# flybirdxx/ComfyUI-SDMatte

Measured on AMD Instinct MI355X. Metric: alpha mattes/sec at 1024x1024, higher is better.
Workload: dtype f16x3

## Files before the change

comfyui-sdmatte_amd/csrc/k_attn.h:

```cpp
#pragma once
#include "sdm_common.h"
#include "k_gemm.h"

struct AttnParams {
  const half_t* q; long q_bs; int ldq;
  const half_t* k; long k_bs; int ldk;
  int k_hs;
  const half_t* vt; long vt_bs; long vt_hs; int ldvt;
  const float* bias; long bias_bs;
  half_t* o; long o_bs; int ldo;
  int o_f32;
  int o_p3; long o_xl_off;
  long q_lo, k_lo, vt_lo;
  int Lq, Lk;
  float scale_log2e;
  const int* tiles; int tiles_bs;
  int nsplit; long part_stride; float* part_ml;
  int batch, heads, nq_blocks, q_chunks;
  int pp_flags;
  int ablate;
};

#define SDM_NEG_BIG (-1.0e30f)
#define SDM_ATTN_SKIP_MARGIN 2000.0f
// ... 385 lines not shown
      for (int dt = 0; dt < 2; ++dt)
#pragma unroll
        for (int g = 0; g < 4; ++g) {
          f32x4 h;
#pragma unroll
          for (int e = 0; e < 4; ++e) h[e] = o[qt][dt][4 * g + e] * inv;
          *(f32x4*)(stf + l31 * PS + (dt * 32 + 8 * g + 4 * hi) * 4) = h;
        }
      SDM_WAVE_SYNC();
      if (p.o_p3 && p.nsplit <= 1) {
        attn_store_p3(p, stf, PS, b, q0 + qt * 32, head, lane);
      } else {
#pragma unroll
      for (int pass = 0; pass < 8; ++pass) {
        const int row = pass * 4 + (lane >> 4), part = lane & 15;
        const int qg = q0 + qt * 32 + row;
        if (qg < p.Lq)
          *(f32x4*)(obase + (size_t)qg * p.ldo + head * 64 + part * 4) = *(const f32x4*)(stf + row * PS + part * 16);
      }
      }
      SDM_WAVE_SYNC();
    }
    return;
  }
#pragma unroll
  for (int qt = 0; qt < QT; ++qt) {
    const float l = PVS ? (lsum + __shfl_xor(lsum, 32)) : ls[qt][0];
    const float inv = 1.0f / l;
#pragma unroll
    for (int dt = 0; dt < 2; ++dt)
#pragma unroll
      for (int g = 0; g < 4; ++g) {
        f16x4 h;
#pragma unroll
        for (int e = 0; e < 4; ++e) h[e] = (half_t)(o[qt][dt][4 * g + e] * inv);
        *(f16x4*)(stg + l31 * PK + (dt * 32 + 8 * g + 4 * hi) * 2) = h;
      }
    SDM_WAVE_SYNC();
#pragma unroll
    for (int pass = 0; pass < 4; ++pass) {
      const int row = pass * 8 + (lane >> 3), part = lane & 7;
      const int qg = q0 + qt * 32 + row;
      if (qg < p.Lq)
        *(f16x8*)(p.o + (size_t)b * p.o_bs + (size_t)qg * p.ldo + head * 64 + part * 8) = *(const f16x8*)(stg + row * PK + part * 16);
    }
    SDM_WAVE_SYNC();
  }
}

#define ATTN64PIPE_SMEM (3 * ATTN64P_BUF)
#define ATTN64PIPE4_KB (2 * 64 * ATTN64_PK + 256)
#define ATTN64PIPE4_VB (64 * ATTN64_PV)
#define ATTN64PIPE4_SMEM (2 * ATTN64PIPE4_KB + 3 * ATTN64PIPE4_VB)
template <int NW>
__global__ void __launch_bounds__(64 * NW, 2) attn_d64_pipe_kernel(AttnParams p) {
  constexpr int NTH = 64 * NW, VPT = 512 / NTH;
  constexpr bool SPLITBUF = NW == 4;
  SDM_DYN_SMEM(smem);
  constexpr int PK = ATTN64_PK, PV = ATTN64_PV, BUF = ATTN64P_BUF;
  constexpr int KLO = 64 * PK, VOFF = 2 * 64 * PK, BOFF = VOFF + 64 * PV;
  auto k_of = [&](int b3, int b2) { return SPLITBUF ? smem + b2 * ATTN64PIPE4_KB : smem + b3 * BUF; };
  auto v_of = [&](int b3) { return SPLITBUF ? smem + 2 * ATTN64PIPE4_KB + b3 * ATTN64PIPE4_VB : smem + b3 * BUF + VOFF; };
  auto bias_of = [&](int b3, int b2) { return (float*)(SPLITBUF ? smem + b2 * ATTN64PIPE4_KB + 2 * 64 * PK : smem + b3 * BUF + BOFF); };
  const int tid = threadIdx.x, lane = tid & 63, wave = tid >> 6;
  const int hi = lane >> 5, l31 = lane & 31;
  int b, head, qblk;
  if (!attn_block_coords(p, blockIdx.x, b, head, qblk)) return;
  const int q0 = qblk * (32 * NW) + wave * 32;

  f16x8 qf[4];
  i32x8 q8p[2];
  {
    int qrow = q0 + l31;
    if (qrow > p.Lq - 1) qrow = p.Lq - 1;
    const half_t* qp = p.q + (size_t)b * p.q_bs + (size_t)qrow * p.ldq + head * 64 + hi * 8;
#pragma unroll
    for (int ks = 0; ks < 4; ++ks) qf[ks] = *(const f16x8*)(qp + ks * 16);
    const half_t* qb = p.q + (size_t)b * p.q_bs + p.q_lo + (size_t)qrow * p.ldq + head * 64 + hi * 16;
#pragma unroll
    for (int m = 0; m < 2; ++m) {
      const i32x4 r0 = *(const i32x4*)(qb + m * 32), r1 = *(const i32x4*)(qb + m * 32 + 8);
      q8p[m] = i32x8{r0[1], r0[0], r0[3], r0[2], r1[1], r1[0], r1[3], r1[2]};
    }
  }
  f32x16 o[2], ls;
  float m_i = SDM_NEG_BIG;
#pragma unroll
  for (int r = 0; r < 16; ++r) { ls[r] = 0.0f; o[0][r] = 0.0f; o[1][r] = 0.0f; }
  f16x8 ones;
#pragma unroll
  for (int j = 0; j < 8; ++j) ones[j] = (half_t)1.0f;

  const half_t* kbase = p.k + (size_t)b * p.k_bs + head * p.k_hs;
  const half_t* vbase = p.vt + (size_t)b * p.vt_bs + (size_t)head * p.vt_hs;
  const float* bbase = p.bias ? p.bias + (size_t)b * p.bias_bs : nullptr;
  const float* bsrc = bbase ? bbase : (const float*)(p.k + (size_t)b * p.k_bs);
  const int ntiles = (p.Lk + 63) / 64;
  const int* tl = p.tiles ? p.tiles + (size_t)b * p.tiles_bs : nullptr;
  const int sp = p.nsplit > 1 ? (int)blockIdx.y : 0;
  int i0, nwalk;
  attn_split_range(p, tl, ntiles, tl ? tl[0] : ntiles, sp, i0, nwalk);
  if (nwalk <= 0) { attn_write_empty_part(p, sp, b, head, q0, lane); return; }
  auto tile_at = [&](int i) { return tl ? tl[1 + i0 + i] : i0 + i; };

  f16x8 rk[VPT], rkl[VPT], rv[VPT];
  float rb = 0.0f;
  bool rin = true;
  auto prefetch = [&](int t) {
    const int k0 = t * 64;
#pragma unroll
    for (int i = 0; i < VPT; ++i) {
      const int v = tid + i * NTH, srow = v >> 3, spart = v & 7;
      int kr = k0 + srow;
      if (kr > p.Lk - 1) kr = p.Lk - 1;
      rk[i] = *(const f16x8*)(kbase + (size_t)kr * p.ldk + spart * 8);
      rv[i] = *(const f16x8*)(vbase + (size_t)srow * p.ldvt + k0 + spart * 8);
      rkl[i] = *(const f16x8*)(kbase + p.k_lo + (size_t)kr * p.ldk + spart * 8);
    }
    int kb = k0 + (tid & 63);
    rin = kb < p.Lk;
    if (!rin) kb = p.Lk - 1;
    rb = bsrc[kb];
  };
  auto stage = [&](int b3, int b2) {
    unsigned char* kb_ = k_of(b3, b2);
    unsigned char* vb_ = v_of(b3);
#pragma unroll
    for (int i = 0; i < VPT; ++i) {
      const int v = tid + i * NTH, srow = v >> 3, spart = v & 7;
      *(f16x8*)(kb_ + srow * PK + spart * 16) = rk[i];
      f16x4 lo, hi4;
#pragma unroll
      for (int e = 0; e < 4; ++e) { lo[e] = rv[i][e]; hi4[e] = rv[i][4 + e]; }
      *(f16x4*)(vb_ + srow * PV + spart * 16) = lo;
      *(f16x4*)(vb_ + srow * PV + spart * 16 + 8) = hi4;
      *(f16x8*)(kb_ + KLO + srow * PK + spart * 16) = rkl[i];
    }
    if (tid < 64) bias_of(b3, b2)[tid] = rin ? (bbase ? rb : 0.0f) : SDM_NEG_BIG;
  };
  auto qk = [&](int b3, int b2, f32x16 (&s)[2]) {
    const unsigned char* Ks = k_of(b3, b2);
    const float* Bs = bias_of(b3, b2);
#pragma unroll
    for (int kt = 0; kt < 2; ++kt)
#pragma unroll
      for (int g = 0; g < 4; ++g) {
        const f32x4 b4 = *(const f32x4*)(Bs + kt * 32 + 8 * g + 4 * hi);
#pragma unroll
        for (int e = 0; e < 4; ++e) s[kt][4 * g + e] = b4[e];
      }
#pragma unroll
    for (int kt = 0; kt < 2; ++kt) {
#pragma unroll
      for (int ks = 0; ks < 4; ++ks) {
        const f16x8 a = *(const f16x8*)(Ks + (kt * 32 + l31) * PK + ks * 32 + hi * 16);
        s[kt] = SDM_MFMA_32x32x16_F16(a, qf[ks], s[kt]);
      }
#pragma unroll
      for (int m = 0; m < 2; ++m) {
        const unsigned char* kp = Ks + KLO + (kt * 32 + l31) * PK + m * 64 + hi * 32;
        const i32x4 a0 = *(const i32x4*)kp, a1 = *(const i32x4*)(kp + 16);
        const i32x8 a8 = i32x8{a0[0], a0[1], a0[2], a0[3], a1[0], a1[1], a1[2], a1[3]};
        s[kt] = SDM_MFMA_32x32x64_BF8_BF8(a8, q8p[m], s[kt], 127 - 11, 127);
      }
    }
  };
  auto lds_barrier = [&]() { SDM_WAIT_LGKMCNT0(); SDM_RAW_BARRIER(); };

  prefetch(tile_at(0));
  stage(0, 0);
  if (1 < nwalk) prefetch(tile_at(1));
  lds_barrier();
  if (1 < nwalk) stage(1, 1);
  if (2 < nwalk) prefetch(tile_at(2));
  f32x16 sa[2], sb[2];
  qk(0, 0, sa);
  lds_barrier();

  int bt = 0;
  auto iter = [&](const int t, f32x16 (&sc)[2], f32x16 (&sn)[2]) {
    const int b1 = bt == 2 ? 0 : bt + 1, b2 = b1 == 2 ? 0 : b1 + 1;
    qk(b1, (t + 1) & 1, sn);
    float mx = SDM_NEG_BIG;
#pragma unroll
    for (int kt = 0; kt < 2; ++kt)
#pragma unroll
      for (int r = 0; r < 16; r += 2) mx = fmaxf(fmaxf(mx, sc[kt][r]), sc[kt][r + 1]);
    mx = fmaxf(mx, __shfl_xor(mx, 32));
    const float mnew = fmaxf(m_i, mx);
    const float alpha = sdm_exp2(m_i - mnew);
    m_i = mnew;
#pragma unroll
    for (int kt = 0; kt < 2; ++kt)
#pragma unroll
      for (int r = 0; r < 16; ++r) sc[kt][r] = sdm_exp2(sc[kt][r] - mnew);
    if (__any(alpha != 1.0f)) {
#pragma unroll
      for (int r = 0; r < 16; ++r) ls[r] *= alpha;
#pragma unroll
      for (int dt = 0; dt < 2; ++dt)
#pragma unroll
        for (int r = 0; r < 16; ++r) o[dt][r] *= alpha;
    }
    if (t + 2 < nwalk) stage(b2, t & 1);
    if (t + 3 < nwalk) prefetch(tile_at(t + 3));
    const unsigned char* Vs = v_of(bt);
#pragma unroll
    for (int kt = 0; kt < 2; ++kt)
#pragma unroll
      for (int u = 0; u < 2; ++u) {
        f16x8 pf;
#pragma unroll
        for (int j = 0; j < 8; ++j) pf[j] = (half_t)sc[kt][8 * u + j];
        ls = SDM_MFMA_32x32x16_F16(ones, pf, ls);
#pragma unroll
        for (int dt = 0; dt < 2; ++dt) {
          const unsigned char* vp = Vs + (dt * 32 + l31) * PV + (kt * 32 + 16 * u + 4 * hi) * 2;
          const f16x4 v0 = *(const f16x4*)vp, v1 = *(const f16x4*)(vp + 16);
          f16x8 vf;
#pragma unroll
          for (int e = 0; e < 4; ++e) { vf[e] = v0[e]; vf[4 + e] = v1[e]; }
          o[dt] = SDM_MFMA_32x32x16_F16(vf, pf, o[dt]);
        }
      }
    lds_barrier();
    bt = b1;
  };
  for (int t = 0; t < nwalk; t += 2) {
    iter(t, sa, sb);
    if (t + 1 < nwalk) iter(t + 1, sb, sa);
  }

  constexpr int PS = 272;
  unsigned char* stf = smem + wave * (32 * PS);
  const float inv = p.nsplit > 1 ? 1.0f : 1.0f / ls[0];
  float* obase = (float*)p.o + (p.nsplit > 1 ? (size_t)sp * p.part_stride : (size_t)0) + (size_t)b * p.o_bs;
  if (p.nsplit > 1 && hi == 0 && q0 + l31 < p.Lq) {
    float* ml = p.part_ml + ((((size_t)sp * p.batch + b) * p.heads + head) * p.Lq + q0 + l31) * 2;
    ml[0] = m_i; ml[1] = ls[0];
  }
#pragma unroll
  for (int dt = 0; dt < 2; ++dt)
#pragma unroll
    for (int g = 0; g < 4; ++g) {
      f32x4 h;
#pragma unroll
      for (int e = 0; e < 4; ++e) h[e] = o[dt][4 * g + e] * inv;
      *(f32x4*)(stf + l31 * PS + (dt * 32 + 8 * g + 4 * hi) * 4) = h;
    }
  SDM_WAVE_SYNC();
  if (p.o_p3 && p.nsplit <= 1) { attn_store_p3(p, stf, PS, b, q0, head, lane); return; }
#pragma unroll
  for (int pass = 0; pass < 8; ++pass) {
    const int row = pass * 4 + (lane >> 4), part = lane & 15;
    const int qg = q0 + row;
    if (qg < p.Lq)
      *(f32x4*)(obase + (size_t)qg * p.ldo + head * 64 + part * 4) = *(const f32x4*)(stf + row * PS + part * 16);
  }
}

#define ATTN64PP_SLOT (3 * 8192 + 256)
#define ATTN64PP_SMEM (6 * ATTN64PP_SLOT)
template <int ABL = 0, int BIAS = 1, int LIST = 1, int KE = 0, int DS = 1, int OB = 1>
__global__ void __launch_bounds__(512, 2) attn_d64_pp_kernel(AttnParams p) {
  SDM_DYN_SMEM(smem);
  constexpr int SLOT = ATTN64PP_SLOT, KLO = 8192, VOFF = 16384, BOFF = 24576;
  constexpr int R = KE < 0 ? 4 : 6, D = KE < 0 ? 3 : 4;
  constexpr int NDMA = BIAS ? 4 : 3;
  const int tid = threadIdx.x, lane = tid & 63, wave = SDM_UNIFORM_I(tid >> 6);
  const int grp = wave >> 2;
  const int hi = lane >> 5, l31 = lane & 31;
  int b, head, qblk;
  if (!attn_block_coords(p, blockIdx.x, b, head, qblk)) return;
  const int q0 = qblk * 256 + wave * 32;

  f16x8 qf[4];
  i32x8 q8p[2];
  {
    int qrow = q0 + l31;
    if (qrow > p.Lq - 1) qrow = p.Lq - 1;
    const half_t* qp = p.q + (size_t)b * p.q_bs + (size_t)qrow * p.ldq + head * 64 + hi * 8;
#pragma unroll
    for (int ks = 0; ks < 4; ++ks) qf[ks] = *(const f16x8*)(qp + ks * 16);
    const half_t* qb = p.q + (size_t)b * p.q_bs + p.q_lo + (size_t)qrow * p.ldq + head * 64 + hi * 16;
#pragma unroll
    for (int m = 0; m < 2; ++m) {
      const i32x4 r0 = *(const i32x4*)(qb + m * 32), r1 = *(const i32x4*)(qb + m * 32 + 8);
      q8p[m] = i32x8{r0[1], r0[0], r0[3], r0[2], r1[1], r1[0], r1[3], r1[2]};
    }
  }
  f32x16 o[2], ls;
  float m_i = SDM_NEG_BIG;
#pragma unroll
  for (int r = 0; r < 16; ++r) { ls[r] = 0.0f; o[0][r] = 0.0f; o[1][r] = 0.0f; }
  f16x8 ones;
#pragma unroll
  for (int j = 0; j < 8; ++j) ones[j] = (half_t)1.0f;

  const half_t* kbase = p.k + (size_t)b * p.k_bs + head * p.k_hs;
  const half_t* vbase = p.vt + (size_t)b * p.vt_bs + (size_t)head * p.vt_hs;
  const int ntiles = p.Lk / 64;
  const int* tl = (LIST && p.tiles) ? p.tiles + (size_t)b * p.tiles_bs : nullptr;
  const int sp = p.nsplit > 1 ? (int)blockIdx.y : 0;
  int i0, nwalk;
  attn_split_range(p, tl, ntiles, tl ? tl[0] : ntiles, sp, i0, nwalk);
  if (nwalk <= 0) { attn_write_empty_part(p, sp, b, head, q0, lane); return; }
  const int* tlp = tl ? tl + 1 + i0 : nullptr;
  auto tile_at = [&](int i) { if (i > nwalk - 1) i = nwalk - 1; return LIST ? tlp[i] : i0 + i; };

  const sdm_rsrc rsK = sdm_make_rsrc(kbase, (unsigned int)(((size_t)(p.Lk - 1) * p.ldk + 64) * 2));
  const sdm_rsrc rsK8 = sdm_make_rsrc(kbase + p.k_lo, (unsigned int)(((size_t)(p.Lk - 1) * p.ldk + 64) * 2));
  const sdm_rsrc rsV = sdm_make_rsrc(vbase, (unsigned int)(((size_t)63 * p.ldvt + p.Lk) * 2));
  const sdm_rsrc rsB = sdm_make_rsrc(BIAS ? p.bias + (size_t)b * p.bias_bs : (const float*)kbase, (unsigned int)p.Lk * 4u);
  const int rho = 8 * wave + (lane >> 3), cpos = lane & 7;
  const int csrc = cpos ^ ((rho >> 1) & 7);
  const int rr = rho & 31;
  const int pir = (rr & 0x13) | (((rr >> 2) & 1) << 3) | (((rr >> 3) & 1) << 2);
  const unsigned int voffK = (unsigned int)(((rho & 32) + pir) * p.ldk * 2 + csrc * 16);
  const unsigned int voffV = (unsigned int)(rho * p.ldvt * 2 + csrc * 16);
  const int lr = lane & 31;
  const unsigned int voffB = (unsigned int)(((lane & 32) + ((lr & 0x13) | (((lr >> 2) & 1) << 3) | (((lr >> 3) & 1) << 2))) * 4);
  auto dma = [&](int tile, int slot, int from = 0, int to = 4) {
    if (ABL & 8) return;
    unsigned char* sb = smem + slot * SLOT + wave * 1024;
    const unsigned int k0 = (unsigned int)tile * 64u;
    int i = 0;
    if (i >= from && i < to) sdm_glds16_buf(rsV, voffV, k0 * 2u, sb + VOFF);
    ++i;
    if (BIAS) { if (i >= from && i < to) sdm_glds4_buf(rsB, voffB, k0 * 4u, smem + slot * SLOT + BOFF); ++i; }
    if (i >= from && i < to) sdm_glds16_buf(rsK8, voffK, k0 * (unsigned int)(p.ldk * 2), sb + KLO);
    ++i;
    if (i >= from && i < to) sdm_glds16_buf(rsK, voffK, k0 * (unsigned int)(p.ldk * 2), sb);
  };
  const int kxor = (l31 >> 1) & 7;
  const int kx = l31 * 128 + ((hi ^ kxor) << 4);
  const int k8x = l31 * 128 + (((2 * hi) ^ kxor) << 4);
  const int vx = l31 * 128 + ((hi ^ kxor) << 4);
  struct KFrag { f16x8 h[4]; i32x8 f8[2]; };
  auto load_bias = [&](int slot, f32x16 (&s)[2]) {
    if (!BIAS) {
#pragma unroll
      for (int kt = 0; kt < 2; ++kt)
#pragma unroll
        for (int r = 0; r < 16; ++r) s[kt][r] = 0.0f;
      return;
    }
    if (ABL & 32) return;
    const float* Bs = (const float*)(smem + slot * SLOT + BOFF);
#pragma unroll
    for (int kt = 0; kt < 2; ++kt)
#pragma unroll
      for (int g = 0; g < 4; ++g) {
        const f32x4 b4 = *(const f32x4*)(Bs + kt * 32 + 8 * g + 4 * hi);
#pragma unroll
        for (int e = 0; e < 4; ++e) s[kt][4 * g + e] = b4[e];
      }
  };
  auto load_k = [&](int slot, int kt, KFrag& f) {
    if (ABL & 32) { SDM_PIN_HERE_V4(f.h[0], f.h[1], f.h[2], f.h[3]); SDM_PIN_HERE_V4(f.f8[0], f.f8[1], f.h[0], f.h[1]); return; }
    const unsigned char* Ks = smem + slot * SLOT + kt * 4096;
#pragma unroll
    for (int ks = 0; ks < 4; ++ks) f.h[ks] = *(const f16x8*)(Ks + (kx ^ (ks * 32)));
#pragma unroll
    for (int m = 0; m < 2; ++m) {
      const i32x4 a0 = *(const i32x4*)(Ks + KLO + (k8x ^ (m * 64))), a1 = *(const i32x4*)(Ks + KLO + ((k8x ^ (m * 64)) ^ 16));
      f.f8[m] = i32x8{a0[0], a0[1], a0[2], a0[3], a1[0], a1[1], a1[2], a1[3]};
    }
  };
  auto mma_k = [&](const KFrag& f, f32x16& sk) {
    if (ABL & 4) return;
#pragma unroll
    for (int ks = 0; ks < 4; ++ks) sk = SDM_MFMA_32x32x16_F16(f.h[ks], qf[ks], sk);
#pragma unroll
    for (int m = 0; m < 2; ++m) sk = SDM_MFMA_32x32x64_BF8_BF8(f.f8[m], q8p[m], sk, 127 - 11, 127);
  };
  struct VFrag { f16x8 v[2][2]; };
  auto load_v = [&](int slot, int kt, VFrag& f) {
    if (ABL & 32) { SDM_PIN_HERE_V4(f.v[0][0], f.v[0][1], f.v[1][0], f.v[1][1]); return; }
    const unsigned char* Vs = smem + slot * SLOT + VOFF;
#pragma unroll
    for (int u = 0; u < 2; ++u)
#pragma unroll
      for (int dt = 0; dt < 2; ++dt) f.v[u][dt] = *(const f16x8*)(Vs + dt * 4096 + (vx ^ ((4 * kt + 2 * u) * 16)));
  };
  auto mma_v = [&](const VFrag& f, const f16x8 (&pk)[2]) {
    if (ABL & 2) return;
#pragma unroll
    for (int u = 0; u < 2; ++u) {
      ls = SDM_MFMA_32x32x16_F16(ones, pk[u], ls);
#pragma unroll
      for (int dt = 0; dt < 2; ++dt) o[dt] = SDM_MFMA_32x32x16_F16(f.v[u][dt], pk[u], o[dt]);
    }
  };
  auto qk = [&](int slot, f32x16 (&s)[2]) {
    KFrag k0, k1;
    load_bias(slot, s);
    load_k(slot, 0, k0);
    load_k(slot, 1, k1);
    mma_k(k0, s[0]);
    mma_k(k1, s[1]);
  };
  auto softmax = [&](f32x16 (&s)[2], f16x8 (&pf)[2][2], auto&& mid0, auto&& mid1, auto&& after_max) {
    if (ABL & 1) {
      mid0(); mid1();
      after_max();
#pragma unroll
      for (int kt = 0; kt < 2; ++kt)
#pragma unroll
        for (int u = 0; u < 2; ++u)
#pragma unroll
          for (int j = 0; j < 8; j += 2) { pf[kt][u][j] = (half_t)s[kt][8 * u + j]; pf[kt][u][j + 1] = pf[kt][u][j]; }
      SDM_PIN_HERE_V4(pf[0][0], pf[0][1], pf[1][0], pf[1][1]);
      return;
    }
    float mx = SDM_NEG_BIG;
#pragma unroll
    for (int r = 0; r < 16; r += 2) mx = fmaxf(fmaxf(mx, s[0][r]), s[0][r + 1]);
#pragma unroll
    for (int r = 0; r < 16; r += 2) mx = fmaxf(fmaxf(mx, s[1][r]), s[1][r + 1]);
    {
      unsigned int xa = __builtin_bit_cast(unsigned int, mx), xb = xa;
      sdm_permlane32_swap(xa, xb);
      mx = fmaxf(__builtin_bit_cast(float, xa), __builtin_bit_cast(float, xb));
    }
    const float mnew = fmaxf(m_i, mx);
    const float alpha = sdm_exp2(m_i - mnew);
    m_i = mnew;
    SDM_SCHED_FENCE();
    mid0();
    SDM_SCHED_FENCE();
    if (__any(alpha != 1.0f)) {
#pragma unroll
      for (int r = 0; r < 16; ++r) ls[r] *= alpha;
#pragma unroll
      for (int dt = 0; dt < 2; ++dt)
#pragma unroll
        for (int r = 0; r < 16; ++r) o[dt][r] *= alpha;
    }
    after_max();
#pragma unroll
    for (int r = 0; r < 16; ++r) s[0][r] = sdm_exp2(s[0][r] - mnew);
    SDM_SCHED_FENCE();
    mid1();
    SDM_SCHED_FENCE();
#pragma unroll
    for (int r = 0; r < 16; ++r) s[1][r] = sdm_exp2(s[1][r] - mnew);
#pragma unroll
    for (int kt = 0; kt < 2; ++kt)
#pragma unroll
      for (int u = 0; u < 2; ++u)
#pragma unroll
        for (int j = 0; j < 8; ++j) pf[kt][u][j] = (half_t)s[kt][8 * u + j];
    SDM_PIN_HERE_V4(pf[0][0], pf[0][1], pf[1][0], pf[1][1]);
  };
  auto lds_barrier = [&]() { SDM_SCHED_FENCE(); SDM_WAIT_LGKMCNT0(); SDM_RAW_BARRIER(); SDM_SCHED_FENCE(); };

#pragma unroll
  for (int i = 0; i < D; ++i) dma(tile_at(i), i);
  int tq = tile_at(D);
  SDM_WAIT_VMCNT0();
  lds_barrier();
  if (!OB) {
    if (grp) {
      if (p.pp_flags & 1) SDM_SETPRIO(1);
      lds_barrier();
    }
  } else if (grp && (p.pp_flags & 1)) SDM_SETPRIO(1);
  f32x16 s[2];
  f16x8 pf[2][2];
  qk(0, s);
  if (!OB || grp) lds_barrier();
  unsigned long long* trc = (unsigned long long*)(smem + R * SLOT) + (wave >> 2) * (8 * 28);
  const bool tracing = (ABL & 64) && blockIdx.x == 0 && (wave & 3) == 0;
  auto stamp = [&](int t, int k) { if ((ABL & 64) && tracing && t < 28 && lane == 0) trc[t * 8 + k] = __builtin_readcyclecounter(); };
  int bt = 0, b1 = 1, bD = D;
  for (int t = 0; t < nwalk; ++t) {
    if (p.pp_flags & 2) SDM_SETPRIO(0);
    constexpr int NE = OB ? NDMA : DS;
    if (KE >= 0) dma(tq, bD, 0, NE >= 2 ? NE - 2 : NE);
    int tqn;
    {
      int in_ = t + D + (KE >= 0 ? 1 : 0); if (in_ > nwalk - 1) in_ = nwalk - 1;
      if (LIST) SDM_SLOAD_I32(tqn, tlp + in_);
      else tqn = i0 + in_;
    }
    if (ABL & 64) stamp(t, 4);
    VFrag v0, v1;
    KFrag k0, k1;
    softmax(s, pf, [&]() { if (KE >= 0 && NE >= 2) dma(tq, bD, NE - 2, NE - 1); }, [&]() { if (KE >= 0 && NE >= 2) dma(tq, bD, NE - 1, NE); },
            [&]() { load_v(bt, 0, v0); load_v(bt, 1, v1); });
    if (ABL & 64) stamp(t, 5);
    if (KE >= 1) { load_bias(b1, s); load_k(b1, 0, k0); }
    if (KE >= 2) load_k(b1, 1, k1);
    if (LIST) SDM_SLOAD_WAIT(tqn);
    if (ABL & 64) { SDM_WAIT_LGKMCNT0(); stamp(t, 0); }
    if (!OB) lds_barrier();
    else if (!grp) { if (!(ABL & 8)) { if (BIAS) SDM_WAIT_VMCNT(8); else SDM_WAIT_VMCNT(6); } lds_barrier(); }
    if (ABL & 64) stamp(t, 1);
    if (p.pp_flags & 2) SDM_SETPRIO(2);
    if (KE < 0) dma(tqn, bD);
    mma_v(v0, pf[0]);
    mma_v(v1, pf[1]);
    if (KE < 1) { load_bias(b1, s); load_k(b1, 0, k0); }
    if (KE < 2) load_k(b1, 1, k1);
    if (KE < 1) {
#pragma unroll
      for (int i = 0; i < 12; ++i) { SDM_SCHED_GROUP(0x008, 1, 0); SDM_SCHED_GROUP(0x100, 2, 0); SDM_SCHED_GROUP(0x002, 1, 0); }
    } else if (KE < 2) {
#pragma unroll
      for (int i = 0; i < 8; ++i) { SDM_SCHED_GROUP(0x008, 1, 0); SDM_SCHED_GROUP(0x100, 1, 0); }
    }
    SDM_SCHED_FENCE();
    mma_k(k0, s[0]);
    mma_k(k1, s[1]);
    SDM_SCHED_FENCE();
    if (!(ABL & 8) && !OB) {
      if (KE < 0) { if (BIAS) SDM_WAIT_VMCNT(4); else SDM_WAIT_VMCNT(3); }
      else if (NDMA + DS == 3) SDM_WAIT_VMCNT(3); else if (NDMA + DS == 4) SDM_WAIT_VMCNT(4); else if (NDMA + DS == 5) SDM_WAIT_VMCNT(5);
      else if (NDMA + DS == 6) SDM_WAIT_VMCNT(6); else if (NDMA + DS == 7) SDM_WAIT_VMCNT(7); else SDM_WAIT_VMCNT(8);
    }
    if (KE >= 0 && !OB) dma(tq, bD, DS, NDMA);
    if (ABL & 64) { asm volatile("s_nop 0" :: "v"(s[0][0]), "v"(s[1][15])); SDM_WAIT_LGKMCNT0(); stamp(t, 2); }
    if (!OB) lds_barrier();
    else if (grp) { if (!(ABL & 8)) { if (BIAS) SDM_WAIT_VMCNT(8); else SDM_WAIT_VMCNT(6); } lds_barrier(); }
    if (ABL & 64) stamp(t, 3);
    tq = tqn;
    bt = b1; b1 = b1 == R - 1 ? 0 : b1 + 1; bD = bD == R - 1 ? 0 : bD + 1;
  }
  if (!grp) lds_barrier();
  SDM_WAIT_VMCNT0();
  lds_barrier();
  if ((ABL & 64) && blockIdx.x == 0) {
    const unsigned long long* tr0 = (const unsigned long long*)(smem + R * SLOT);
    for (int i = tid; i < 2 * 8 * 28; i += 512) ((unsigned long long*)p.part_ml)[i] = tr0[i];
    __syncthreads();
  }

  constexpr int PS = 272;
  unsigned char* stf = smem + wave * (32 * PS);
  const float inv = p.nsplit > 1 ? 1.0f : 1.0f / ls[0];
  float* obase = (float*)p.o + (p.nsplit > 1 ? (size_t)sp * p.part_stride : (size_t)0) + (size_t)b * p.o_bs;
  if (p.nsplit > 1 && hi == 0 && q0 + l31 < p.Lq) {
    float* ml = p.part_ml + ((((size_t)sp * p.batch + b) * p.heads + head) * p.Lq + q0 + l31) * 2;
    ml[0] = m_i; ml[1] = ls[0];
  }
#pragma unroll
  for (int dt = 0; dt < 2; ++dt)
#pragma unroll
    for (int g = 0; g < 4; ++g) {
      f32x4 h;
#pragma unroll
      for (int e = 0; e < 4; ++e) h[e] = o[dt][4 * g + e] * inv;
      *(f32x4*)(stf + l31 * PS + (dt * 32 + 8 * g + 4 * hi) * 4) = h;
    }
  SDM_WAVE_SYNC();
  if (p.o_p3 && p.nsplit <= 1) { attn_store_p3(p, stf, PS, b, q0, head, lane); return; }
#pragma unroll
  for (int pass = 0; pass < 8; ++pass) {
    const int row = pass * 4 + (lane >> 4), part = lane & 15;
    const int qg = q0 + row;
    if (qg < p.Lq)
      *(f32x4*)(obase + (size_t)qg * p.ldo + head * 64 + part * 4) = *(const f32x4*)(stf + row * PS + part * 16);
  }
}

#define ATTN512_X_BYTES (8 * 16 * 64 * 4)

#define ATTN512P_K_BYTES (32 * 1024)
#define ATTN512P_V_BYTES (512 * 64)
#define ATTN512P_X_OFF (2 * ATTN512P_K_BYTES + 2 * ATTN512P_V_BYTES)
#define ATTN512P_SMEM (ATTN512P_X_OFF + ATTN512_X_BYTES)

template <int ABL = 0>
__global__ void __launch_bounds__(512) attn_d512_kernel(AttnParams p) {
  SDM_DYN_SMEM(smem);
  float* Xs = (float*)(smem + ATTN512P_X_OFF);
  const int tid = threadIdx.x, lane = tid & 63, wave = SDM_UNIFORM_I(tid >> 6);
  const int hi = lane >> 5, l31 = lane & 31;
  const int qgp = wave >> 1, dh = wave & 1;
  int b, head_unused, qblk;
  if (!attn_block_coords(p, blockIdx.x, b, head_unused, qblk)) return;
  const int q0 = qblk * 128 + qgp * 32;

  f16x8 qf[16];
  {
    int qrow = q0 + l31;
    if (qrow > p.Lq - 1) qrow = p.Lq - 1;
    const half_t* qp = p.q + (size_t)b * p.q_bs + (size_t)qrow * p.ldq + dh * 256 + hi * 8;
#pragma unroll
    for (int ks = 0; ks < 16; ++ks) qf[ks] = *(const f16x8*)(qp + ks * 16);
  }
  f32x16 o[8];
#pragma unroll
  for (int dt = 0; dt < 8; ++dt)
#pragma unroll
    for (int r = 0; r < 16; ++r) o[dt][r] = 0.0f;
  float m_i = SDM_NEG_BIG, l_i = 0.0f;

  const half_t* kbase = p.k + (size_t)b * p.k_bs;
  const half_t* vbase = p.vt + (size_t)b * p.vt_bs;
  const int ntiles = (p.Lk + 31) / 32;

  const sdm_rsrc rsK = sdm_make_rsrc(kbase, (unsigned int)((size_t)p.Lk * p.ldk * 2));
  const sdm_rsrc rsV = sdm_make_rsrc(vbase, (unsigned int)((size_t)512 * p.ldvt * 2));
  const unsigned int v_voff = (unsigned int)((lane >> 2) * p.ldvt * 2 + (((lane & 3) ^ ((lane >> 4) & 3)) * 16));
  auto issue_tile = [&](int t, int buf) {
    if (ABL & 8) return;
    const int k0 = t * 32;
    unsigned char* Kd = smem + buf * ATTN512P_K_BYTES;
    unsigned char* Vd = smem + 2 * ATTN512P_K_BYTES + buf * ATTN512P_V_BYTES;
#pragma unroll
    for (int i = 0; i < 4; ++i) {
      const int rho = 4 * wave + i;
      const int pi = (rho & 16) | (((rho >> 2) & 1) << 3) | (((rho >> 3) & 1) << 2) | (rho & 3);
      int kr = k0 + pi;
// ... 58 lines not shown
        float x = (s[r] + xpt[r * 64 + lane]) * p.scale_log2e;
        if (key >= p.Lk) x = SDM_NEG_BIG;
        s[r] = x;
        mx = fmaxf(mx, x);
      }
    } else {
#pragma unroll
      for (int r = 0; r < 16; ++r) {
        const float x = (s[r] + xpt[r * 64 + lane]) * p.scale_log2e;
        s[r] = x;
        mx = fmaxf(mx, x);
      }
    }
    mx = fmaxf(mx, __shfl_xor(mx, 32));
    const float mnew = fmaxf(m_i, mx);
    const float alpha = sdm_exp2(m_i - mnew);
    m_i = mnew;
    float rs = 0.0f;
#pragma unroll
    for (int r = 0; r < 16; ++r) {
      const float pv = sdm_exp2(s[r] - mnew);
      s[r] = pv;
      rs += pv;
    }
    l_i = l_i * alpha + rs;
    if (__any(alpha != 1.0f)) {
#pragma unroll
      for (int dt = 0; dt < 8; ++dt)
#pragma unroll
        for (int r = 0; r < 16; ++r) o[dt][r] *= alpha;
    }
    } else l_i = 1.0f;
    f16x8 pf[2];
#pragma unroll
    for (int u = 0; u < 2; ++u)
#pragma unroll
      for (int j = 0; j < 8; ++j) pf[u][j] = (half_t)s[8 * u + j];
    SDM_SCHED_FENCE();
#pragma unroll
    for (int i = 0; i < 16; ++i) {
      if (i + 3 < 16) a[(i + 3) & 3] = rd_v(i + 3);
      if (!(ABL & 2)) o[i & 7] = SDM_MFMA_32x32x16_F16(a[i & 3], pf[i >> 3], o[i & 7]);
    }
    if (!(ABL & 34)) {
#pragma unroll
      for (int i = 0; i < 13; ++i) { SDM_SCHED_GROUP(0x100, 1, 1); SDM_SCHED_GROUP(0x008, 1, 1); }
      SDM_SCHED_GROUP(0x008, 3, 1);
    }
    SDM_SCHED_FENCE();
    SDM_WAIT_VMCNT0();
    SDM_RAW_BARRIER();
  }

  l_i += __shfl_xor(l_i, 32);
  const float inv = 1.0f / l_i;
  if (p.o_f32) {
    constexpr int PF = 528;
    unsigned char* stf = smem + wave * (32 * PF);
#pragma unroll
    for (int half = 0; half < 2; ++half) {
      __syncthreads();
#pragma unroll
      for (int d4 = 0; d4 < 4; ++d4) {
        const int dt = half * 4 + d4;
#pragma unroll
        for (int g = 0; g < 4; ++g) {
          f32x4 h;
#pragma unroll
          for (int e = 0; e < 4; ++e) h[e] = o[dt][4 * g + e] * inv;
          *(f32x4*)(stf + l31 * PF + (d4 * 32 + 8 * g + 4 * hi) * 4) = h;
        }
      }
      __syncthreads();
#pragma unroll
      for (int pass = 0; pass < 16; ++pass) {
        const int row = pass * 2 + (lane >> 5), part = lane & 31;
        const int qg = q0 + row;
        if (qg < p.Lq)
          *(f32x4*)((float*)p.o + (size_t)b * p.o_bs + (size_t)qg * p.ldo + dh * 256 + half * 128 + part * 4) =
              *(const f32x4*)(stf + row * PF + part * 16);
      }
    }
    return;
  }
  constexpr int PS = 272;
  unsigned char* stg = smem + wave * (32 * PS);
#pragma unroll
  for (int half = 0; half < 2; ++half) {
    __syncthreads();
#pragma unroll
    for (int d4 = 0; d4 < 4; ++d4) {
      const int dt = half * 4 + d4;
#pragma unroll
      for (int g = 0; g < 4; ++g) {
        f16x4 h;
#pragma unroll
        for (int e = 0; e < 4; ++e) h[e] = (half_t)(o[dt][4 * g + e] * inv);
        *(f16x4*)(stg + l31 * PS + (d4 * 32 + 8 * g + 4 * hi) * 2) = h;
      }
    }
    __syncthreads();
#pragma unroll
    for (int pass = 0; pass < 8; ++pass) {
      const int row = pass * 4 + (lane >> 4), part = lane & 15;
      const int qg = q0 + row;
      if (qg < p.Lq)
        *(f16x8*)(p.o + (size_t)b * p.o_bs + (size_t)qg * p.ldo + dh * 256 + half * 128 + part * 8) =
            *(const f16x8*)(stg + row * PS + part * 16);
    }
  }
}

__global__ void __launch_bounds__(256) attn_combine_kernel(const float* __restrict__ part_o, const float* __restrict__ part_ml, float* __restrict__ out,
                                                           int nsplit, long part_stride, int batch, int heads, int Lq, long o_bs, int ldo) {
  const long t = (long)blockIdx.x * blockDim.x + threadIdx.x;
  const int part = (int)(t & 15);
  const long rh = t >> 4;
  if (rh >= (long)batch * Lq * heads) return;
  const int head = (int)(rh % heads);
  const long br = rh / heads;
  const int row = (int)(br % Lq), b = (int)(br / Lq);
  float M = SDM_NEG_BIG;
  for (int s = 0; s < nsplit; ++s) M = fmaxf(M, part_ml[((((size_t)s * batch + b) * heads + head) * Lq + row) * 2]);
  f32x4 acc = {0.f, 0.f, 0.f, 0.f};
  float L = 0.0f;
  for (int s = 0; s < nsplit; ++s) {
    const float* ml = part_ml + ((((size_t)s * batch + b) * heads + head) * Lq + row) * 2;
    const float w = sdm_exp2(ml[0] - M);
    L += ml[1] * w;
    const f32x4 v = *(const f32x4*)(part_o + (size_t)s * part_stride + (size_t)b * o_bs + (size_t)row * ldo + head * 64 + part * 4);
#pragma unroll
    for (int e = 0; e < 4; ++e) acc[e] += v[e] * w;
  }
  const float inv = 1.0f / L;
#pragma unroll
  for (int e = 0; e < 4; ++e) acc[e] *= inv;
  *(f32x4*)(out + (size_t)b * o_bs + (size_t)row * ldo + head * 64 + part * 4) = acc;
}

__global__ void __launch_bounds__(256) attn_combine_p3_kernel(const float* __restrict__ part_o, const float* __restrict__ part_ml, unsigned char* __restrict__ out,
                                                              long xl_off, int nsplit, long part_stride, int batch, int heads, int Lq, long o_bs, int ldo) {
  const long t = (long)blockIdx.x * blockDim.x + threadIdx.x;
  const int part = (int)(t & 7);
  const long rh = t >> 3;
  if (rh >= (long)batch * Lq * heads) return;
  const int head = (int)(rh % heads);
  const long br = rh / heads;
  const int row = (int)(br % Lq), b = (int)(br / Lq);
  float M = SDM_NEG_BIG;
  for (int s = 0; s < nsplit; ++s) M = fmaxf(M, part_ml[((((size_t)s * batch + b) * heads + head) * Lq + row) * 2]);
  float acc[8] = {0.f, 0.f, 0.f, 0.f, 0.f, 0.f, 0.f, 0.f};
  float L = 0.0f;
  for (int s = 0; s < nsplit; ++s) {
    const float* ml = part_ml + ((((size_t)s * batch + b) * heads + head) * Lq + row) * 2;
    const float w = sdm_exp2(ml[0] - M);
    L += ml[1] * w;
    const float* src = part_o + (size_t)s * part_stride + (size_t)b * o_bs + (size_t)row * ldo + head * 64 + part * 8;
    const f32x4 v0 = *(const f32x4*)src, v1 = *(const f32x4*)(src + 4);
#pragma unroll
    for (int e = 0; e < 4; ++e) { acc[e] += v0[e] * w; acc[4 + e] += v1[e] * w; }
  }
  const float inv = 1.0f / L;
#pragma unroll
// ... 70 lines not shown
```

comfyui-sdmatte_amd/csrc/k_misc.h:

```cpp
#pragma once
#include "sdm_common.h"

template <typename F>
SDM_DEV_INLINE float resize_aa_sample(F fetch, int in_h, int in_w, int out_h, int out_w, int oy, int ox) {
  const float sy = (float)in_h / (float)out_h, sx = (float)in_w / (float)out_w;
  const float supy = sy >= 1.0f ? sy : 1.0f, supx = sx >= 1.0f ? sx : 1.0f;
  const float invy = sy >= 1.0f ? 1.0f / sy : 1.0f, invx = sx >= 1.0f ? 1.0f / sx : 1.0f;
  const float cy = sy * ((float)oy + 0.5f), cx = sx * ((float)ox + 0.5f);
  int ymin = (int)(cy - supy + 0.5f); if (ymin < 0) ymin = 0;
  int ymax = (int)(cy + supy + 0.5f); if (ymax > in_h) ymax = in_h;
  int xmin = (int)(cx - supx + 0.5f); if (xmin < 0) xmin = 0;
  int xmax = (int)(cx + supx + 0.5f); if (xmax > in_w) xmax = in_w;
  float wys = 0.0f, wxs = 0.0f;
  for (int y = ymin; y < ymax; ++y) { float w = 1.0f - fabsf(((float)y - cy + 0.5f) * invy); wys += w > 0.0f ? w : 0.0f; }
  for (int x = xmin; x < xmax; ++x) { float w = 1.0f - fabsf(((float)x - cx + 0.5f) * invx); wxs += w > 0.0f ? w : 0.0f; }
  float acc = 0.0f;
  for (int y = ymin; y < ymax; ++y) {
    float wy = 1.0f - fabsf(((float)y - cy + 0.5f) * invy); wy = wy > 0.0f ? wy / wys : 0.0f;
    float row = 0.0f;
    for (int x = xmin; x < xmax; ++x) {
      float wx = 1.0f - fabsf(((float)x - cx + 0.5f) * invx); wx = wx > 0.0f ? wx / wxs : 0.0f;
      row += wx * fetch(y, x);
    }
    acc += wy * row;
// ... 106 lines not shown
  const float r = img[i * 3 + 0], g = img[i * 3 + 1], b = img[i * 3 + 2];
  if (mode == 1) {
    f32x4 o = {r, g, b, a};
    *(f32x4*)(matted + i * 4) = o;
  } else if (mode == 2) {
    const float gate = (t > 0.2f && a > 0.1f) ? 1.0f : 0.0f;
    matted[i * 3 + 0] = r * gate; matted[i * 3 + 1] = g * gate; matted[i * 3 + 2] = b * gate;
  } else {
    matted[i * 3 + 0] = 0.0f; matted[i * 3 + 1] = 0.0f; matted[i * 3 + 2] = 0.0f;
  }
}

SDM_DEV_INLINE u32x2 sdm_pair_plane4(const float (&x)[4], f16x4& oh) {
  float xx[4], xl[4];
#pragma unroll
  for (int e = 0; e < 4; ++e) {
    const float y = fminf(fmaxf(x[e], -57344.0f), 57344.0f);
    oh[e] = (half_t)y; xx[e] = y; xl[e] = (y - (float)oh[e]) * 2048.0f;
  }
  int a = SDM_CVT_PK_BF8(xx[0], xx[1], 0, false), b = SDM_CVT_PK_BF8(xl[0], xl[1], 0, false);
  a = SDM_CVT_PK_BF8(xx[2], xx[3], a, true); b = SDM_CVT_PK_BF8(xl[2], xl[3], b, true);
  u32x2 pr;
  pr[0] = (unsigned int)a; pr[1] = (unsigned int)b;
  return pr;
}

__global__ void split_planes_kernel(const float* __restrict__ x, half_t* __restrict__ hi, half_t* __restrict__ lo, long n, float mult, int mode) {
  const long i4 = ((long)blockIdx.x * blockDim.x + threadIdx.x) * 4;
  if (i4 >= n) return;
  float y[4];
#pragma unroll
  for (int e = 0; e < 4; ++e) y[e] = (i4 + e < n) ? x[i4 + e] * mult : 0.0f;
  f16x4 oh, ol;
  if (mode == 3) {
    const u32x2 pr = sdm_pair_plane4(y, oh);
    *(f16x4*)(hi + i4) = oh;
    *(u32x2*)(lo + i4) = pr;
  } else {
#pragma unroll
    for (int e = 0; e < 4; ++e) { oh[e] = (half_t)y[e]; ol[e] = (half_t)(y[e] - (float)oh[e]); }
    *(f16x4*)(hi + i4) = oh;
    *(f16x4*)(lo + i4) = ol;
  }
}

SDM_DEV_INLINE float cross_patch_value(const float* __restrict__ uin, int H, int W, long b, int key, int j) {
  if (j >= 36 || key >= H * W) return 0.0f;
  const int ci = j / 9, tap = j - ci * 9, ky = tap / 3, kx = tap - ky * 3;
  const int y = key / W + ky - 1, x = key - (key / W) * W + kx - 1;
  if ((unsigned)y >= (unsigned)H || (unsigned)x >= (unsigned)W) return 0.0f;
  return uin[((size_t)b * H * W + (size_t)y * W + x) * 16 + 4 + ci];
}
__global__ void __launch_bounds__(256) cross_patch_planes_kernel(const float* __restrict__ uin, int B, int H, int W, half_t* __restrict__ k_hi,
                                                                 half_t* __restrict__ k_pair, half_t* __restrict__ vt, int ldvt) {
  const long t = (long)blockIdx.x * blockDim.x + threadIdx.x;
  const int Lk = H * W;
  if (blockIdx.y == 0) {
    if (t >= (long)B * Lk * 8) return;
    const int oct = (int)(t & 7), key = (int)((t >> 3) % Lk);
    const long b = (t >> 3) / Lk;
    u32x4 hv, pv;
#pragma unroll
    for (int g = 0; g < 2; ++g) {
      float x[4];
#pragma unroll
      for (int e = 0; e < 4; ++e) x[e] = cross_patch_value(uin, H, W, b, key, oct * 8 + g * 4 + e);
      f16x4 oh;
      const u32x2 pr = sdm_pair_plane4(x, oh);
      const u32x2 hw = __builtin_bit_cast(u32x2, oh);
      hv[2 * g] = hw[0]; hv[2 * g + 1] = hw[1]; pv[2 * g] = pr[0]; pv[2 * g + 1] = pr[1];
    }
    const size_t o = ((size_t)b * Lk + key) * 64 + oct * 8;
    *(u32x4*)(k_hi + o) = hv;
    *(u32x4*)(k_pair + o) = pv;
  } else {
    const int cpr = ldvt / 8;
    if (t >= (long)B * 64 * cpr) return;
    const int chunk = (int)(t % cpr), j = (int)((t / cpr) & 63);
    const long b = t / cpr / 64;
    u32x4 hv;
#pragma unroll
    for (int g = 0; g < 2; ++g) {
      f16x4 oh;
#pragma unroll
      for (int e = 0; e < 4; ++e) oh[e] = (half_t)fminf(fmaxf(cross_patch_value(uin, H, W, b, chunk * 8 + g * 4 + e, j), -57344.0f), 57344.0f);
      const u32x2 hw = __builtin_bit_cast(u32x2, oh);
      hv[2 * g] = hw[0]; hv[2 * g + 1] = hw[1];
    }
    *(u32x4*)(vt + ((size_t)b * 64 + j) * ldvt + chunk * 8) = hv;
  }
}

__global__ void scale_copy_kernel(const float* __restrict__ in, float* __restrict__ out, long n, float mult) {
  const long i = (long)blockIdx.x * blockDim.x + threadIdx.x;
  if (i < n) out[i] = in[i] * mult;
}

__global__ void fill_random_f16_kernel(half_t* __restrict__ p, long n, unsigned int seed, float amp) {
  for (long i = (long)blockIdx.x * blockDim.x + threadIdx.x; i < n; i += (long)gridDim.x * blockDim.x) {
    unsigned int h = (unsigned int)i * 2654435761u + seed;
    h ^= h >> 15; h *= 2246822519u; h ^= h >> 13; h *= 3266489917u; h ^= h >> 16;
    p[i] = (half_t)(((float)(h & 0xFFFF) * (1.0f / 32768.0f) - 1.0f) * amp);
  }
}
__global__ void fill_random_f32_kernel(float* __restrict__ p, long n, unsigned int seed, float amp) {
  for (long i = (long)blockIdx.x * blockDim.x + threadIdx.x; i < n; i += (long)gridDim.x * blockDim.x) {
    unsigned int h = (unsigned int)i * 2654435761u + seed;
    h ^= h >> 15; h *= 2246822519u; h ^= h >> 13; h *= 3266489917u; h ^= h >> 16;
    p[i] = ((float)(h & 0xFFFF) * (1.0f / 32768.0f) - 1.0f) * amp;
  }
}

#define SDM_CMASK_EMPTY 0xFFFFFFFFu

__global__ __launch_bounds__(256) void cmask_table_kernel(const float* __restrict__ plane, unsigned int* __restrict__ table, int n0, int H, int W) {
  SDM_SHARED unsigned int tb[4];
  const int b = blockIdx.x, tid = threadIdx.x;
  if (tid < 4) tb[tid] = SDM_CMASK_EMPTY;
  __syncthreads();
  const float* pl = plane + (size_t)b * H * W;
  for (int i = tid; i < 64 * 64; i += 256) {
    const int y = (int)(((long)(i >> 6) * H) >> 6), x = (int)(((long)(i & 63) * W) >> 6);
    const unsigned int bits = __builtin_bit_cast(unsigned int, pl[(size_t)y * W + x]);
    for (int k = 0; k < 4; ++k) {
      unsigned int cur = tb[k];
      if (cur == SDM_CMASK_EMPTY) cur = atomicCAS(&tb[k], SDM_CMASK_EMPTY, bits);
      if (cur == SDM_CMASK_EMPTY || cur == bits) break;
    }
  }
  __syncthreads();
  if (tid < 4) table[(size_t)(n0 + b) * 4 + tid] = tb[tid];
}

__global__ void cmask_init_kernel(const float* __restrict__ plane, unsigned char* __restrict__ mask, const unsigned int* __restrict__ table, int n0, int B, long HW) {
  const long i = (long)blockIdx.x * blockDim.x + threadIdx.x;
  if (i >= (long)B * HW) return;
  const int b = (int)(i / HW);
  const unsigned int bits = __builtin_bit_cast(unsigned int, plane[i]);
// ... 65 lines not shown
```

comfyui-sdmatte_amd/csrc/sdm_common.h:

```cpp
#pragma once
#include <stdint.h>
#include <stddef.h>
#ifdef SDM_EMU
#include "hip_emu.h"
#else
#include <hip/hip_runtime.h>
#endif

typedef _Float16 half_t;
typedef half_t f16x8 __attribute__((ext_vector_type(8)));
typedef half_t f16x4 __attribute__((ext_vector_type(4)));
typedef half_t f16x2 __attribute__((ext_vector_type(2)));
typedef float f32x2 __attribute__((ext_vector_type(2)));
typedef float f32x4 __attribute__((ext_vector_type(4)));
typedef float f32x16 __attribute__((ext_vector_type(16)));
typedef int i32x8 __attribute__((ext_vector_type(8)));
typedef int i32x4 __attribute__((ext_vector_type(4)));

#ifdef SDM_EMU
#define SDM_DYN_SMEM(name) unsigned char* name = emu::g_dyn_smem
#define SDM_SHARED static thread_local
#define SDM_MFMA_32x32x16_F16(a, b, c) emu_mfma_f32_32x32x16_f16((a), (b), (c))
#define SDM_MFMA_32x32x64_F8(a, b, c, sa, sb) emu_mfma_scale_f32_32x32x64_fp8((a), (b), (c), (sa), (sb))
#define SDM_CVT_PK_FP8(a, b, old, hi_word) emu_cvt_pk_fp8_f32((a), (b), (old), (hi_word))
// ... 64 lines not shown
#else
typedef __amdgpu_buffer_rsrc_t sdm_rsrc;
__device__ __forceinline__ sdm_rsrc sdm_make_rsrc(const void* p, unsigned int bytes) {
  return __builtin_amdgcn_make_buffer_rsrc((void*)p, 0, (int)bytes, 0x00020000);
}
__device__ __forceinline__ u32x4 sdm_buffer_load16(sdm_rsrc r, unsigned int voff, unsigned int soff) {
  return __builtin_amdgcn_raw_buffer_load_b128(r, (int)voff, (int)soff, 0);
}
__device__ __forceinline__ u32x2 sdm_buffer_load8(sdm_rsrc r, unsigned int voff, unsigned int soff) {
  return __builtin_amdgcn_raw_buffer_load_b64(r, (int)voff, (int)soff, 0);
}
__device__ __forceinline__ void sdm_buffer_store16(u32x4 v, sdm_rsrc r, unsigned int voff, unsigned int soff) {
  __builtin_amdgcn_raw_buffer_store_b128(v, r, (int)voff, (int)soff, 0);
}
#endif

#ifdef SDM_EMU
typedef sdm_rsrc sdm_rsrc_raw;
static inline sdm_rsrc_raw sdm_make_rsrc_raw(const void* p, unsigned int bytes) { return sdm_make_rsrc(p, bytes); }
#define SDM_ASM_BUFFER_LOAD16(dst, voff, rsrc, imm) (dst) = sdm_buffer_load16((rsrc), (voff), (imm))
#define SDM_ASM_BUFFER_LOAD16_FIRST(dst, voff, rsrc, imm) (dst) = sdm_buffer_load16((rsrc), (voff), (imm))
#else
typedef u32x4 sdm_rsrc_raw;
__device__ __forceinline__ sdm_rsrc_raw sdm_make_rsrc_raw(const void* p, unsigned int bytes) {
  const unsigned long long a = (unsigned long long)p;
  sdm_rsrc_raw d;
  d[0] = (unsigned int)__builtin_amdgcn_readfirstlane((int)(unsigned int)a);
  d[1] = (unsigned int)__builtin_amdgcn_readfirstlane((int)((unsigned int)(a >> 32) & 0xFFFFu));
  d[2] = (unsigned int)__builtin_amdgcn_readfirstlane((int)bytes);
  d[3] = 0x00020000u;
  return d;
}
#define SDM_ASM_BUFFER_LOAD16(dst, voff, rsrc, imm) \
  asm volatile("buffer_load_dwordx4 %0, %1, %2, 0 offen offset:" #imm : "=v"(dst) : "v"(voff), "s"(rsrc) : "memory")
#define SDM_ASM_BUFFER_LOAD16_FIRST(dst, voff, rsrc, imm) \
  asm volatile("s_nop 4\n\tbuffer_load_dwordx4 %0, %1, %2, 0 offen offset:" #imm : "=v"(dst) : "v"(voff), "s"(rsrc) : "memory")
#endif

#ifdef SDM_EMU
static inline void sdm_glds16(const void* gsrc, unsigned char* lds_base) { memcpy(lds_base + (threadIdx.x & 63) * 16, gsrc, 16); }
static inline void sdm_glds16_buf(sdm_rsrc r, unsigned int voff, unsigned int soff, unsigned char* lds_base) {
  const u32x4 v = sdm_buffer_load16(r, voff, soff);
  memcpy(lds_base + (threadIdx.x & 63) * 16, &v, 16);
}
static inline void sdm_glds4_buf(sdm_rsrc r, unsigned int voff, unsigned int soff, unsigned char* lds_base) {
  unsigned int v = 0u;
  const unsigned long long o = (unsigned long long)voff + soff;
  if (o + 4 <= r.bytes) memcpy(&v, r.base + o, 4);
  memcpy(lds_base + (threadIdx.x & 63) * 4, &v, 4);
}
#define SDM_UNIFORM_I(x) (x)
#define SDM_OPAQUE_I(x) ((void)0)
#define SDM_PIN_HERE_V4(a, b, c, d) ((void)0)
#define SDM_WAIT_VMCNT0() ((void)0)
#define SDM_WAIT_VMCNT(n) ((void)0)
#define SDM_WAIT_LGKMCNT0() ((void)0)
#define SDM_SLOAD_I32(dst, ptr) (dst) = *(ptr)
#define SDM_SLOAD_WAIT(dst) ((void)0)
#define SDM_RAW_BARRIER() __syncthreads()
#else
__device__ __forceinline__ void sdm_glds16(const void* gsrc, unsigned char* lds_base) {
  __builtin_amdgcn_global_load_lds((const __attribute__((address_space(1))) void*)gsrc,
                                   (__attribute__((address_space(3))) void*)lds_base, 16, 0, 0);
}
__device__ __forceinline__ void sdm_glds16_buf(sdm_rsrc r, unsigned int voff, unsigned int soff, unsigned char* lds_base) {
  __builtin_amdgcn_raw_ptr_buffer_load_lds(r, (__attribute__((address_space(3))) void*)lds_base, 16, (int)voff, (int)soff, 0, 0);
}
__device__ __forceinline__ void sdm_glds4_buf(sdm_rsrc r, unsigned int voff, unsigned int soff, unsigned char* lds_base) {
  __builtin_amdgcn_raw_ptr_buffer_load_lds(r, (__attribute__((address_space(3))) void*)lds_base, 4, (int)voff, (int)soff, 0, 0);
}
#define SDM_UNIFORM_I(x) __builtin_amdgcn_readfirstlane(x)
#define SDM_OPAQUE_I(x) asm volatile("" : "+v"(x))
#define SDM_PIN_HERE_V4(a, b, c, d) asm volatile("" : "+v"(a), "+v"(b), "+v"(c), "+v"(d))
#define SDM_WAIT_VMCNT0() asm volatile("s_waitcnt vmcnt(0)" ::: "memory")
#define SDM_WAIT_VMCNT(n) asm volatile("s_waitcnt vmcnt(" #n ")" ::: "memory")
#define SDM_WAIT_LGKMCNT0() asm volatile("s_waitcnt lgkmcnt(0)" ::: "memory")
#define SDM_SLOAD_I32(dst, ptr) asm volatile("s_load_dword %0, %1, 0x0" : "=s"(dst) : "s"(ptr) : "memory")
#define SDM_SLOAD_WAIT(dst) asm volatile("s_waitcnt lgkmcnt(0)" : "+s"(dst) :: "memory")
#define SDM_RAW_BARRIER() do { asm volatile("" ::: "memory"); __builtin_amdgcn_s_barrier(); asm volatile("" ::: "memory"); } while (0)
#endif

#ifdef SDM_EMU
static inline float sdm_sum_row16(float v) {
  v += __shfl_xor(v, 1); v += __shfl_xor(v, 2); v += __shfl_xor(v, 4); v += __shfl_xor(v, 8);
  return v;
}
#else
#define SDM_DPP_ADD(v, ctrl) ((v) + __builtin_bit_cast(float, __builtin_amdgcn_update_dpp(0, __builtin_bit_cast(int, (v)), (ctrl), 0xF, 0xF, false)))
__device__ __forceinline__ float sdm_sum_row16(float v) {
  v = SDM_DPP_ADD(v, 0xB1);
  v = SDM_DPP_ADD(v, 0x4E);
  v = SDM_DPP_ADD(v, 0x124);
  v = SDM_DPP_ADD(v, 0x128);
  return v;
}
#endif

#ifdef SDM_EMU
static inline unsigned int sdm_perm_b32(unsigned int s0, unsigned int s1, unsigned int sel) {
  const unsigned long long v = ((unsigned long long)s0 << 32) | s1;
  unsigned int r = 0;
  for (int i = 0; i < 4; ++i) r |= (unsigned int)((v >> (8 * ((sel >> (8 * i)) & 7))) & 0xffull) << (8 * i);
  return r;
}
static inline void sdm_permlane32_swap(unsigned int& a, unsigned int& b) {
  auto& w = emu::wave(); const int l = emu::lane_id();
  w.slot[l][0] = a; w.slot[l][1] = b; emu::wave_barrier();
  if (l < 32) b = w.slot[l + 32][0]; else a = w.slot[l - 32][1];
  emu::wave_barrier();
}
#else
__device__ __forceinline__ unsigned int sdm_perm_b32(unsigned int s0, unsigned int s1, unsigned int sel) { return __builtin_amdgcn_perm(s0, s1, sel); }
__device__ __forceinline__ void sdm_permlane32_swap(unsigned int& a, unsigned int& b) {
  const auto r = __builtin_amdgcn_permlane32_swap(a, b, false, false);
  a = r[0]; b = r[1];
}
#endif

#define SDM_LOG2E 1.4426950408889634f

SDM_DEV_INLINE float sdm_silu(float x) {
  return x / (1.0f + sdm_exp2(-x * SDM_LOG2E));
}

SDM_DEV_INLINE float sdm_gelu_erf(float x) {
  return 0.5f * x * (1.0f + erff(x * 0.70710678118654752f));
// ... 28 lines not shown
```

comfyui-sdmatte_amd/csrc/sdm_engine.cpp:

```cpp
#include "sdm_common.h"
#include "k_conv.h"
#include "k_gemm.h"
#include "k_norm.h"
#include "k_attn.h"
#include "k_misc.h"
#include "k_trimap.h"
#include "k_cclabel.h"
#include "k_foreground.h"
#include "k_guided.h"
#include "k_roi.h"
#include "k_canvas.h"
#include "k_boxes.h"
#include "../../include/sdmatte.h"

#include <algorithm>
#include <cmath>
#include <cstdio>
#include <cstdlib>
#include <cstring>
#include <atomic>
#include <map>
#include <mutex>
#include <shared_mutex>
#include <string>
// ... 33 lines not shown
        if (r_ != hipSuccess) fprintf(stderr, "[sdmatte] hipFuncSetAttribute(%d bytes of LDS) failed: %s\n", (int)(bytes), hipGetErrorString(r_)); \
        else done_.fetch_or(bit_, std::memory_order_relaxed);                                                    \
      }                                                                                                          \
    }                                                                                                            \
  } while (0)
#endif

static inline int rup(int a, int b) { return ((a + b - 1) / b) * b; }
#ifdef SDM_EMU
static inline void dev_use(int) {}
#else
static inline void dev_use(int device) {
  const hipError_t r = hipSetDevice(device);
  if (r != hipSuccess) fprintf(stderr, "[sdmatte] hipSetDevice(%d) failed: %s\n", device, hipGetErrorString(r));
}
#endif
static inline size_t rupz(size_t a, size_t b) { return ((a + b - 1) / b) * b; }

struct OptEntry { const char* name; int value; int def; const char* what; };
static OptEntry g_opts[] = {
  {"conv_f8", 1, 1, "residual terms of the wide split-precision 3x3 convs on fp8 MFMAs (read when a model is built)"},
  {"gemm_f8", 1, 1, "the same for Linear / 1x1 layers with K >= gemm_f8_min_k (read when a model is built)"},
  {"gemm_f8_min_k", 1024, 1024, "smallest K of a GEMM that takes the 8-wave fp8-residual kernel"},
  {"gemm_p3", 1, 1, "transformer-block Linear layers on the plane-fed GEMM (k_gemm.h): pre-split operand planes from LayerNorm / GroupNorm / attention / GEGLU, LDS-DMA only (the W3 weight copies are built when a model is built)"},
  {"gemm_p3_tile", 0, 0, "row tile of the plane-fed GEMM: 0 by shape, 256 / 128 / 64 forced"},
  {"gemm_p3_attn", 1, 1, "d=64 attention cores write the operand planes of to_out themselves (0: fp32 result + one conversion pass)"},
  {"gemm_p3_persist", 1, 1, "plane-fed GEMM: persistent blocks that prefetch the next tile's first chunk underneath the epilogue (0: one block per tile, n > 1: a grid of n blocks - tests)"},
  {"gemm_p3_ablate", 0, 0, "bench only: 1 no MFMAs, 2 no DMAs behind the prologue, 4 no epilogue (sdm_bench_gemm_p3)"},
  {"conv_up_phase", 1, 1, "up-sampling 3x3 convs (Upsample2D) as four 2x2-tap phase convs on the plane-fed GEMM (k_gemm.h, UP): 0 off (the 3x3 kernels on the up-sampled image), 1 the launches with at least two 256-row tiles per CU (up_phase_wins: measured), 2 every eligible launch (tests).  0 / non-0 is read when a model is built: the phase matrices are a derived weight layout"},
  {"conv_epi", 4, 4, "F8 kernels' epilogue: 4 register-direct stores + residual as accumulator init, 3 residual init only, 0 LDS-staged"},
  {"conv_xtile", 1, 1, "F8 3x3: cross-tile prefetch by the producer waves"},
  {"conv_f8_tpb", 0, 0, "F8: tiles per block (0 = by queue depth)"},
  {"conv_dma", 1, 1, "3x3 stride-1 256x128 tile: weights by LDS-DMA"},
  {"conv_dma_all", 0, 0, "keep a stage-ordered weight copy for every wide 3x3 layer, not only the split-precision ones (read when a model is built)"},
  {"conv_pc", -1, -1, "producer / consumer form of the split-precision DMA kernel: -1 by channel count, 0 off, 1 on"},
  {"conv_pc_min_cin", 256, 256, "conv_pc = -1: smallest Cin that takes the producer / consumer form"},
  {"conv_db", 0, 0, "512x128 double-buffered tile where the queue is deep"},
  {"trimap_skip", 1, 1, "VAE encoder, trimap images: output tiles inside a constant region of the trimap are not multiplied (k_misc.h cmask_*; exact). 0 = every tile"},
  {"conv_band_rows", 0, 0, "tile rows per XCD band of the convs that leave constant tiles out (0 = by image height)"},
  {"trimap_skip_min_rows", 512, 512, "smallest output height at which constant tiles are left out (measured at 1024^2: the 1024- and 512-row levels gain 3.7 + 1.6 ms, the 256-row level loses 0.7: too few of its 32 x 128-pixel tiles lie inside one region)"},
  {"conv_splitk", -1, -1, "split-K of the register-staged conv / GEMM kernels: -1 by shape (few tiles, long K), 0 off, n >= 2 forced where the shape allows"},
  {"force_cfg0", 0, 0, "always the 256x128 tile for 3x3 stride 1 (tests: fused GroupNorm at tiny sizes)"},
  {"no_gn_fuse", 0, 0, "never fuse the GroupNorm apply into the consuming conv"},
  {"split_lds_pad", 0, 0, "extra dynamic LDS of the register-staged split kernels (forces one block per CU)"},
  {"attn_f8", 1, 1, "Q.K^T residual terms of the d=64 split-precision attention on fp8 MFMAs"},
  {"attn_dense", 0, 0, "walk every key tile of the trimap-biased self-attention"},
  {"attn_pv_split", 0, 0, "residual terms of P.V too (fully split attention; tests)"},
  {"attn_nw", 0, 0, "waves per d=64 attention block: 0 by launch size, 4, 8"},
  {"attn_pipe", 1, 1, "8-wave split-precision d=64 attention: two-tile software pipeline"},
  {"attn_pipe4", 1, 1, "the same pipeline for the 4-wave launches (two K / three V^T buffers)"},
  {"attn_pp", 1, 1, "split-precision d=64 attention with fp32 output as a ping-pong of the block's wave halves (attn_d64_pp_kernel, 256 query rows per block): 0 off, 1 on, 2 on without the static priority of the younger half, 3 on with per-segment priority flips"},
  {"attn_pp_min_blocks", 128, 128, "attn_pp: launches with fewer 256-row blocks than this keep the 4-wave pipelines (0 in tests: the ping-pong kernel at any size)"},
  {"attn_ksplit", 0, 0, "key split of the d=64 split-precision attention: 0 by launch size (blocks that do not fill the chip's block slots a whole number of times), 1 off, 2 / 4 forced, 3 forced on the ping-pong kernel (ignored elsewhere: those launches run unsplit)"},
  {"cross_shared", 1, 1, "cross-attention on ONE key / value operand per forward, the patch matrix of the trimap latent (cross_patch_planes_kernel), with the K|V fold moved into q_shared / out_shared: 0 = every block's own kv_folded conv + transpose.  Read per forward"},
  {"precise_mask", -1, -1, "stages in split precision (-1 = the config's own mask; per-stage attribution experiments; read at sdm_create)"},
#ifdef SDM_EMU
  {"emu_arena_extra", 0, 0, "emulator build only, self-test of the arena check: the launch pass of a stand-alone op allocates one block its sizing pass did not"},
#endif
};
static OptEntry* opt_find(const char* name) {
  for (auto& o : g_opts) if (name && strcmp(o.name, name) == 0) return &o;
  return nullptr;
}
static int opt(const char* name) { OptEntry* o = opt_find(name); return o ? o->value : 0; }
static std::shared_mutex g_opt_mu;
struct OptReadLock { std::shared_lock<std::shared_mutex> l; OptReadLock() : l(g_opt_mu) {} };
static std::mutex g_count_mu;
static std::map<std::string, long> g_kernel_counts;
static void count_kernel(const char* name) { std::lock_guard<std::mutex> g(g_count_mu); g_kernel_counts[name] += 1; }

template <int NTAPS, int STRIDE, int TH, int TW, int BN, int KC, int WM, int WN, int DB = 0, int GNOK = 0>
static void launch_conv_t(const ConvParams& p_in, void* stream) {
  using C = ConvCfg<NTAPS, STRIDE, TH, TW, BN, KC, WM, WN, DB>;
  ConvParams p = p_in;
  p.tiles_m = (NTAPS == 9) ? sdm_cdiv(p.Wout, TW) * sdm_cdiv(p.Hout, TH)
                           : (int)(((p.rows_per_img ? (long)p.rows_per_img : p.M) + C::BM - 1) / C::BM);
  p.tiles_n = sdm_cdiv(p.Cout_pad, BN);
  const long total_m = (long)p.tiles_m * ((NTAPS == 9 || p.rows_per_img) ? p.N : 1);
  p.xcd_chunk = (int)((total_m + 7) / 8);
  const dim3 grid((unsigned)(8L * p.xcd_chunk * p.tiles_n), (unsigned)(p.ksplit > 1 ? p.ksplit : 1), 1);
  const size_t gn_extra = (size_t)(p.C0 + p.C1) * 8;
  if constexpr (!DB) {
    if (p.w_lo) {
      using CS = ConvCfg<NTAPS, STRIDE, TH, TW, BN, KC, WM, WN, 0, 1>;
      const size_t lds_pad = (size_t)opt("split_lds_pad");
      if (GNOK && p.gn_scale) {
        auto k = conv_mfma_kernel<NTAPS, STRIDE, TH, TW, BN, KC, WM, WN, 1, 0, GNOK, 1>;
        SDM_SET_SMEM(k, 160 * 1024);
        SDM_LAUNCH(k, grid, dim3(CS::NTHREADS), (size_t)CS::SMEM + gn_extra + lds_pad, stream, p);
      } else {
        auto k = conv_mfma_kernel<NTAPS, STRIDE, TH, TW, BN, KC, WM, WN, 1, 0, 0, 1>;
        SDM_SET_SMEM(k, 160 * 1024);
        SDM_LAUNCH(k, grid, dim3(CS::NTHREADS), CS::SMEM + lds_pad, stream, p);
      }
      return;
    }
  }
  if (GNOK && p.gn_scale) {
    const size_t smem = (size_t)C::SMEM + gn_extra;
    if (p.in_f32) {
      auto k = conv_mfma_kernel<NTAPS, STRIDE, TH, TW, BN, KC, WM, WN, 1, DB, GNOK>;
      SDM_SET_SMEM(k, C::SMEM + 1024 * 8);
      SDM_LAUNCH(k, grid, dim3(C::NTHREADS), smem, stream, p);
    } else {
      auto k = conv_mfma_kernel<NTAPS, STRIDE, TH, TW, BN, KC, WM, WN, 0, DB, GNOK>;
      SDM_SET_SMEM(k, C::SMEM + 1024 * 8);
// ... 1110 lines not shown
  return 0;
}

static int op_groupnorm_raw(sdm_ctx* e, const void* in0, const void* in1, int C0, int C1, int in_f32, int N, int HW, int groups,
                            const float* gamma, const float* beta, float eps, int silu, void* out, int out_f32, const float* st0 = nullptr,
                            int rows0 = 0, const float* st1 = nullptr, int rows1 = 0, bool have_stats = false) {
  const int C = C0 + C1;
  T scratch; float* scale; float* shift;
  TRY(gn_scale_shift(e, in0, in1, C0, C1, in_f32, N, HW, groups, gamma, beta, eps, st0, rows0, st1, rows1, have_stats, &scratch, &scale, &shift));
  if (!e->dry) {
    GnSrc s; s.in0 = in0; s.in1 = in1; s.C0 = C0; s.C1 = C1; s.in_f32 = in_f32; s.HW = HW;
    const GnGeometry g = gn_geometry(C, N, HW);
    prof_begin(e, "gn_apply", 0, (double)N * HW * C * (in_f32 ? 4 : 2) + (double)N * HW * C * (double)fmt_bytes(out_f32));
    if (out_f32 == kFmtP3)
      SDM_LAUNCH(gn_apply_p3_kernel, dim3((unsigned)(((long)N * HW + 15) / 16)), dim3(256), 0, e->stream, s, (const float*)scale, (const float*)shift, (unsigned char*)out,
                 silu, (long)N * HW);
    else
    SDM_LAUNCH(gn_apply_kernel, dim3(g.nb, N), dim3(g.threads), 0, e->stream, s, (const float*)scale, (const float*)shift, out, out_f32, silu, g.ppb);
    prof_end(e);
  }
  tfree(e, scratch);
  return 0;
}

static int op_gn(sdm_ctx* e, const NormL& n, const T& x, const T* x2, int silu, float eps, T* out, int out_fmt = -1) {
  const int C = x.C + (x2 ? x2->C : 0);
  if (C != n.C) SDM_FAIL(e, SDM_ERR_INVALID, "groupnorm: C %d != %d", C, n.C);
  *out = talloc(e, x.N, x.H, x.W, C, out_fmt >= 0 ? out_fmt : e->act_f32);
  const bool hs = x.sbytes && (!x2 || x2->sbytes);
  return op_groupnorm_raw(e, x.p, x2 ? x2->p : nullptr, x.C, x2 ? x2->C : 0, x.f32, x.N, x.H * x.W, e->cfg.groups, n.g, n.b, eps, silu,
                          out->p, out->f32, x.stats, x.srows, x2 ? x2->stats : nullptr, x2 ? x2->srows : 0, hs);
}

static int op_ln(sdm_ctx* e, const NormL& n, const T& x, float eps, T* out, int out_fmt = -1) {
  if (x.C != n.C || x.C % 64 || x.C > 64 * SDM_LN_MAXV) SDM_FAIL(e, SDM_ERR_INVALID, "layernorm: unsupported C %d", x.C);
  *out = talloc(e, x.N, x.H, x.W, x.C, out_fmt >= 0 ? out_fmt : e->act_f32);
  if (e->dry) return 0;
  const long rows = x.rows();
  if (out->f32 == kFmtP3) {
    if (x.f32 != 1 || x.C > 128 * SDM_LNP_MAXI) SDM_FAIL(e, SDM_ERR_INVALID, "layernorm (P3): fp32 input, C <= %d expected", 128 * SDM_LNP_MAXI);
    prof_begin(e, "layernorm", 0, (double)rows * x.C * 7);
    SDM_LAUNCH(layernorm_p3_kernel, dim3((unsigned)((rows + 15) / 16)), dim3(256), 0, e->stream, (const float*)x.p, (const float*)n.g, (const float*)n.b,
               (unsigned char*)out->p, rows, x.C, eps);
    prof_end(e);
    return 0;
  }
  prof_begin(e, "layernorm", 0, (double)rows * x.C * ((x.f32 ? 4 : 2) + (out->f32 ? 4 : 2)));
  SDM_LAUNCH(layernorm_kernel, dim3((unsigned)((rows + 3) / 4)), dim3(256), 0, e->stream, (const void*)x.p, x.f32, (const float*)n.g,
             (const float*)n.b, out->p, out->f32, rows, x.C, eps);
  prof_end(e);
  return 0;
}

struct AttnPrec { int prec = 0; long q_lo = 0, k_lo = 0, v_lo = 0; int out_f32 = 0; int out_p3 = 0; bool has_bias = false, has_tiles = false; bool shared_kv = false; };

enum AttnKernel { kAttnPP, kAttnPPBias, kAttnPPTiles, kAttnPipe8, kAttnPipe4, kAttnP3W8, kAttnP3W4, kAttnP1W8, kAttnP1W4, kAttnP2W8, kAttnP2W4,
                  kAttnF16W8, kAttnF16W4, kAttnD512 };
struct AttnPlan {
  AttnKernel kernel;
  const char* spec_counter;
  const char* combine_counter;
  int qrows;
  unsigned nblk;
  int nsplit;
  bool walk_tiles, own_list;
  bool pv_split;
  int pp_flags;
};
struct AttnKernelInfo { const char* counter; int threads; size_t smem; void (*launch)(const AttnKernelInfo&, const AttnPlan&, const AttnParams&, void*); };
template <auto K, int LDS_LIMIT = 160 * 1024>
static void attn_launch_t(const AttnKernelInfo& ki, const AttnPlan& pl, const AttnParams& p, void* stream) {
  if constexpr (LDS_LIMIT > 0) SDM_SET_SMEM(K, LDS_LIMIT);
  SDM_LAUNCH(K, dim3(pl.nblk, (unsigned)pl.nsplit, 1), dim3(ki.threads), ki.smem, stream, p);
}
static const AttnKernelInfo kAttnKernels[] = {
  {"attn_d64_pp", 512, ATTN64PP_SMEM, attn_launch_t<attn_d64_pp_kernel<0, 0, 0>>},
  {"attn_d64_pp", 512, ATTN64PP_SMEM, attn_launch_t<attn_d64_pp_kernel<0, 1, 0>>},
  {"attn_d64_pp", 512, ATTN64PP_SMEM, attn_launch_t<attn_d64_pp_kernel<0, 1, 1>>},
  {"attn_d64_pipe<8>", 512, ATTN64PIPE_SMEM, attn_launch_t<attn_d64_pipe_kernel<8>>},
  {"attn_d64_pipe<4>", 256, ATTN64PIPE4_SMEM, attn_launch_t<attn_d64_pipe_kernel<4>>},
  {"attn_d64<prec3,8>", 512, ATTN64P_SMEM, attn_launch_t<attn_d64_kernel<1, 3, 8>>},
  {"attn_d64<prec3,4>", 256, ATTN64P_SMEM, attn_launch_t<attn_d64_kernel<1, 3, 4>>},
  {"attn_d64<prec1,8>", 512, ATTN64P_SMEM, attn_launch_t<attn_d64_kernel<1, 1, 8>>},
  {"attn_d64<prec1,4>", 256, ATTN64P_SMEM, attn_launch_t<attn_d64_kernel<1, 1, 4>>},
  {"attn_d64<prec2,8>", 512, ATTN64P_SMEM, attn_launch_t<attn_d64_kernel<1, 2, 8>>},
  {"attn_d64<prec2,4>", 256, ATTN64P_SMEM, attn_launch_t<attn_d64_kernel<1, 2, 4>>},
  {"attn_d64<fp16,8>", 512, ATTN64P_SMEM, attn_launch_t<attn_d64_kernel<1, 0, 8>>},
  {"attn_d64<fp16,4>", 256, ATTN64_SMEM, attn_launch_t<attn_d64_kernel<1, 0, 4>, 0>},
  {"attn_d512", 512, ATTN512P_SMEM, attn_launch_t<attn_d512_kernel<0>, ATTN512P_SMEM>},
};
static AttnPlan attn_plan(int B, int heads, int Lq, int Lk, int D, int prec, int out_f32, bool has_bias, bool has_tiles, int cus) {
  AttnPlan pl;
  memset(&pl, 0, sizeof(pl));
  pl.nsplit = 1;
  bool nw8 = true, pp = false;
  if (D != 64) {
    pl.kernel = kAttnD512; pl.qrows = 128;
  } else {
    pl.walk_tiles = has_bias && opt("attn_dense") == 0;
    pl.own_list = pl.walk_tiles && !has_tiles;
    pl.pv_split = prec == 1 && opt("attn_pv_split") != 0;
    const int force_nw = opt("attn_nw");
    const long blocks256 = (long)B * heads * sdm_cdiv(Lq, 256);
    pp = prec == 2 && out_f32 && opt("attn_pp") != 0 && !force_nw && Lk % 64 == 0 &&
         blocks256 >= opt("attn_pp_min_blocks");
    nw8 = pp || (force_nw ? (force_nw == 8) : (prec && blocks256 >= 1024));
    pl.qrows = nw8 ? 256 : 128;
    if (prec == 2) {
      const bool pipe = out_f32 && opt(nw8 ? "attn_pipe" : "attn_pipe4") != 0;
      if (pp) pl.kernel = pl.walk_tiles ? kAttnPPTiles : (has_bias ? kAttnPPBias : kAttnPP);
      else if (pipe) pl.kernel = nw8 ? kAttnPipe8 : kAttnPipe4;
      else pl.kernel = nw8 ? kAttnP3W8 : kAttnP3W4;
    } else if (prec) {
      pl.kernel = pl.pv_split ? (nw8 ? kAttnP1W8 : kAttnP1W4) : (nw8 ? kAttnP2W8 : kAttnP2W4);
    } else {
      pl.kernel = nw8 ? kAttnF16W8 : kAttnF16W4;
    }
    if (pp) {
      pl.spec_counter = pl.walk_tiles ? "attn_pp<0,1,1>" : (has_bias ? "attn_pp<0,1,0>" : "attn_pp<0,0,0>");
      pl.pp_flags = opt("attn_pp") == 1 ? 1 : (opt("attn_pp") == 3 ? 2 : 0);
    }
  }
  pl.nblk = (unsigned)(B * heads * 8 * sdm_cdiv(sdm_cdiv(Lq, pl.qrows), 8));
  if (D == 64 && prec && out_f32 && !pl.pv_split) {
    const long blocks = pl.nblk, slots = (long)cus * (nw8 ? 1 : 2);
    const int o = opt("attn_ksplit"), ntiles64 = sdm_cdiv(Lk, 64);
    if (o >= 2) pl.nsplit = (o == 2 || o == 4 || (o == 3 && pp)) ? o : 1;
    else if (o == 0) {
      auto rounds = [&](int s) { return (double)((blocks * s + slots - 1) / slots) / s; };
      for (int s = 2; s <= 4; ++s)
        if ((s != 3 || pp) && ntiles64 / s >= 32 && rounds(s) < 0.85 * rounds(pl.nsplit)) pl.nsplit = s;
    }
    if (pl.nsplit > 1) pl.combine_counter = pl.nsplit == 2 ? "attn_combine/n=2" : (pl.nsplit == 3 ? "attn_combine/n=3" : "attn_combine/n=4");
  }
  return pl;
}

static int op_attention_raw(sdm_ctx* e, const half_t* q, int ldq, const half_t* k, int ldk, const half_t* v, int ldv, const float* bias_l2,
                            int B, int heads, int Lq, int Lk, int D, void* out, int ldo, bool q_prescaled = false, const int* tiles = nullptr,
                            AttnPrec ap = AttnPrec()) {
  if (!(D == 64 || (D == 512 && heads == 1))) SDM_FAIL(e, SDM_ERR_INVALID, "attention: unsupported head dim %d x %d heads", D, heads);
  if ((ldq | ldk | ldv | ldo) % 8) SDM_FAIL(e, SDM_ERR_INVALID, "attention: row strides must be multiples of 8");
  if (ap.prec && D != 64) SDM_FAIL(e, SDM_ERR_INVALID, "attention: the split-precision variant exists for head dim 64 only");
  if (ap.prec == 2 && !q_prescaled) SDM_FAIL(e, SDM_ERR_INVALID, "attention: the fp8-residual form takes pre-scaled queries");
  if (!e->dry && (ap.has_bias != (bias_l2 != nullptr) || ap.has_tiles != (tiles != nullptr)))
    SDM_FAIL(e, SDM_ERR_STATE, "attention: bias / tile list do not match what the sizing pass was told");
  const AttnPlan pl = attn_plan(B, heads, Lq, Lk, D, ap.prec, ap.out_f32, ap.has_bias, ap.has_tiles, device_cus());
  const AttnKernelInfo& ki = kAttnKernels[pl.kernel];
  const int nsplit = pl.nsplit;
  const int ldvt = rup(Lk, 64);
  if (ap.shared_kv && (D != 64 || pl.pv_split || ldk != 64)) SDM_FAIL(e, SDM_ERR_INVALID, "attention: a shared key / value operand is [key][64] at head dim 64, without the residual terms of P.V");
  T vt;
  if (!ap.shared_kv) vt = talloc(e, (ap.prec ? 2 : 1) * B, heads, D, ldvt, 0);
  const int ntiles64 = sdm_cdiv(Lk, 64);
  T tl_own, part_o, part_ml;
  if (pl.own_list) tl_own = talloc(e, B, 1, 1, ntiles64 + 1, 1);
  if (nsplit > 1) {
    part_o = talloc(e, nsplit * B, Lq, 1, ldo, 1);
    part_ml = talloc(e, nsplit * B, heads, Lq, 2, 1);
  }
  if (!e->dry) {
    if (pl.own_list) {
      SDM_LAUNCH(attn_active_tiles_kernel, dim3(B), dim3(256), 0, e->stream, bias_l2, Lk, ntiles64, (int*)tl_own.p, ntiles64 + 1, SDM_ATTN_SKIP_MARGIN);
      tiles = (const int*)tl_own.p;
    }
    if (!pl.walk_tiles) tiles = nullptr;
    const long vt_hs = ap.shared_kv ? 0 : (long)D * ldvt, vt_bs = ap.shared_kv ? (long)D * ldvt : (long)heads * vt_hs;
    if (!ap.shared_kv) {
      prof_begin(e, "transpose_v", 0, (double)B * Lk * heads * D * 4);
      count_kernel("transpose_v");
      SDM_LAUNCH(transpose_v_kernel, dim3(ldvt / 64, heads * (D / 64), B), dim3(256), 0, e->stream, v, (long)Lk * ldv, ldv, (half_t*)vt.p, vt_bs,
                 vt_hs, ldvt, Lk, D);
      if (pl.pv_split)
        SDM_LAUNCH(transpose_v_kernel, dim3(ldvt / 64, heads * (D / 64), B), dim3(256), 0, e->stream, v + ap.v_lo, (long)Lk * ldv, ldv,
                   (half_t*)vt.p + (size_t)B * vt_bs, vt_bs, vt_hs, ldvt, Lk, D);
      prof_end(e);
    }
    AttnParams p;
    memset(&p, 0, sizeof(p));
    p.q = q; p.q_bs = (long)Lq * ldq; p.ldq = ldq;
    p.k = k; p.k_bs = (long)Lk * ldk; p.ldk = ldk; p.k_hs = ap.shared_kv ? 0 : 64;
    p.vt = ap.shared_kv ? v : (const half_t*)vt.p; p.vt_bs = vt_bs; p.vt_hs = vt_hs; p.ldvt = ldvt;
    p.bias = bias_l2; p.bias_bs = Lk;
    p.tiles = tiles; p.tiles_bs = ntiles64 + 1;
    p.o = (half_t*)out; p.o_bs = (long)Lq * ldo; p.ldo = ldo; p.o_f32 = ap.out_f32;
    if (ap.out_p3) {
      if (!ap.out_f32 || Lq % 32 || ldo % 32 || D != 64) SDM_FAIL(e, SDM_ERR_INVALID, "attention: plane output needs d = 64, Lq %% 32 == 0 and C %% 32 == 0");
      p.o_p3 = 1; p.o_xl_off = (long)(p3_rows_pad((size_t)B * Lq) * ldo * 2);
    }
    p.q_lo = ap.q_lo; p.k_lo = ap.k_lo; p.vt_lo = (long)B * vt_bs;
    p.Lq = Lq; p.Lk = Lk;
    p.scale_log2e = q_prescaled ? 1.0f : (1.0f / sqrtf((float)D)) * SDM_LOG2E;
    if (nsplit > 1) { p.nsplit = nsplit; p.o = (half_t*)part_o.p; p.part_stride = (long)B * p.o_bs; p.part_ml = (float*)part_ml.p; }
    p.batch = B; p.heads = heads; p.nq_blocks = sdm_cdiv(Lq, pl.qrows); p.q_chunks = 8;
    p.pp_flags = pl.pp_flags;
    double flops = 4.0 * B * heads * (double)Lq * Lk * D;
    const double bytes = 2.0 * B * heads * D * (2.0 * Lq + 2.0 * Lk);
    std::string adesc = "B=" + std::to_string(B) + " h=" + std::to_string(heads) + " Lq=" + std::to_string(Lq) + " Lk=" + std::to_string(Lk);
    if (e->prof_on && tiles) {
      std::vector<int> hl((size_t)B * (ntiles64 + 1));
      (void)dev_sync(e->stream);
      (void)dev_memcpy_d2h(hl.data(), tiles, hl.size() * sizeof(int), e->stream);
      (void)dev_sync(e->stream);
      long act = 0;
      for (int bi = 0; bi < B; ++bi) act += hl[(size_t)bi * (ntiles64 + 1)];
      const double frac = (double)act / ((double)B * ntiles64);
      flops *= frac;
      char fb[48];
      snprintf(fb, sizeof(fb), " active_key_tiles=%.3f", frac);
      adesc += fb;
    }
    if (D == 64) {
      prof_begin(e, "attn_d64", flops, bytes, adesc);
      count_kernel(ki.counter);
      if (pl.spec_counter) count_kernel(pl.spec_counter);
      ki.launch(ki, pl, p, e->stream);
      if (nsplit > 1) {
        count_kernel("attn_combine");
        count_kernel(pl.combine_counter);
        if (ap.out_p3) count_kernel("attn_combine_p3");
        const long nthr = (long)B * Lq * heads * 16;
        if (ap.out_p3)
          SDM_LAUNCH(attn_combine_p3_kernel, dim3((unsigned)((nthr / 2 + 255) / 256)), dim3(256), 0, e->stream, (const float*)part_o.p, (const float*)part_ml.p,
                     (unsigned char*)out, (long)(p3_rows_pad((size_t)B * Lq) * ldo * 2), nsplit, (long)B * (long)Lq * ldo, B, heads, Lq, (long)Lq * ldo, ldo);
        else
        SDM_LAUNCH(attn_combine_kernel, dim3((unsigned)((nthr + 255) / 256)), dim3(256), 0, e->stream, (const float*)part_o.p, (const float*)part_ml.p, (float*)out,
                   nsplit, (long)B * (long)Lq * ldo, B, heads, Lq, (long)Lq * ldo, ldo);
      }
      prof_end(e);
    } else {
      prof_begin(e, "attn_d512", flops, bytes);
      ki.launch(ki, pl, p, e->stream);
      prof_end(e);
    }
  }
  if (nsplit > 1) { tfree(e, part_ml); tfree(e, part_o); }
  if (pl.own_list) tfree(e, tl_own);
  if (!ap.shared_kv) tfree(e, vt);
  return 0;
}


static int conv_simple(sdm_ctx* e, int layer, const T& in, T* out, int Cout_store, int out_f32, int stride = 1, int pad_mode = 0, int up = 0,
                       const T* res = nullptr, float scale = 1.0f, bool want_stats = false, int lo_cols = -1) {
  const ConvL& L = e->convs[layer];
  int Ho = in.H << up, Wo = in.W << up;
  if (stride == 2) { Ho /= 2; Wo /= 2; }
  *out = talloc(e, in.N, Ho, Wo, Cout_store, out_f32);
  if (want_stats) TRY(tstats(e, *out));
  ConvArgs a; a.in0 = &in; a.out = out; a.stride = stride; a.pad_mode = pad_mode; a.up = up; a.res = res; a.out_scale = scale; a.lo_cols = lo_cols;
  return op_conv(e, L, a);
}

static int gn_conv(sdm_ctx* e, const NormL& n, const ConvL& L, const T& x, const T* x2, int silu, float eps, ConvArgs a) {
  const int C = x.C + (x2 ? x2->C : 0);
  if (C != n.C) SDM_FAIL(e, SDM_ERR_INVALID, "groupnorm: C %d != %d", C, n.C);
  int cfg = -1;
  if (!opt("no_gn_fuse") && L.ntaps == 9 && a.stride == 1 && C <= 1024 && C == L.Cin_pad) {
    ConvParams p;
    memset(&p, 0, sizeof(p));
    conv_shape_params(p, L, x, x2, *a.out, a.stride);
    cfg = conv_pick_cfg(L.ntaps, a.stride, p);
  }
  if (cfg == 0 || cfg == 4 || cfg == 5) {
    const bool hs = x.sbytes && (!x2 || x2->sbytes);
    T scratch; float* scale; float* shift;
    TRY(gn_scale_shift(e, x.p, x2 ? x2->p : nullptr, x.C, x2 ? x2->C : 0, x.f32, x.N, x.H * x.W, e->cfg.groups, n.g, n.b, eps, x.stats, x.srows,
                       x2 ? x2->stats : nullptr, x2 ? x2->srows : 0, hs, &scratch, &scale, &shift));
    a.in0 = &x; a.in1 = x2;
    a.gn_scale = e->dry ? (const float*)16 : scale; a.gn_shift = shift; a.gn_silu = silu;
    a.force_cfg = cfg;
    int rc = op_conv(e, L, a);
    tfree(e, scratch);
    return rc;
  }
  T h;
  TRY(op_gn(e, n, x, x2, silu, eps, &h));
  a.in0 = &h; a.in1 = nullptr;
  int rc = op_conv(e, L, a);
  tfree(e, h);
  return rc;
}

static int resblock(sdm_ctx* e, const ResB& r, const T& x, const T* x2, float eps, T* out) {
// ... 71 lines not shown
  count_kernel("gemm_p3");
  launch_gemm_p3(p, epi, e->stream);
#ifndef SDM_EMU
  { const hipError_t le = hipGetLastError(); if (le != hipSuccess) SDM_FAIL(e, SDM_ERR_HIP, "gemm %s: launch failed: %s", L.name.c_str(), hipGetErrorString(le)); }
#endif
  prof_end(e);
  return 0;
}

static int op_to_p3(sdm_ctx* e, const T& x, T* out) {
  if (x.f32 != 1 || x.C % 32) SDM_FAIL(e, SDM_ERR_INVALID, "to_p3: fp32 input with C %% 32 == 0 expected (C = %d)", x.C);
  *out = talloc(e, x.N, x.H, x.W, x.C, kFmtP3);
  if (e->dry) return 0;
  const long units = ((x.rows() + 31) / 32) * (x.C / 32);
  prof_begin(e, "to_p3", 0, (double)x.rows() * x.C * 7);
  SDM_LAUNCH(to_p3_kernel, dim3((unsigned)std::min<long>((units + 3) / 4, 1 << 20)), dim3(256), 0, e->stream, (const float*)x.p, (unsigned char*)out->p, x.rows(), x.C);
  prof_end(e);
  return 0;
}

static int linear(sdm_ctx* e, int layer, const T& in, T* out, int Cout, int out_f32, const T* res = nullptr, bool want_stats = false, int lo_cols = -1) {
  *out = talloc(e, in.N, in.H, in.W, Cout, out_f32);
  if (want_stats) TRY(tstats(e, *out));
  if (in.f32 == kFmtP3) return op_gemm_p3(e, e->convs[layer], in, out, res, lo_cols);
  ConvArgs a; a.in0 = &in; a.out = out; a.res = res; a.lo_cols = lo_cols;
  return op_conv(e, e->convs[layer], a);
}

static int vae_attention(sdm_ctx* e, const VaeAttnB& a, const T& x, T* out) {
  T hn, qkv, ao;
  const int pa = ((e->cfg.precise_mask & SDM_PRECISE_UNET_ATTN) && a.C == 64) ? 1 : 0;
  const int pf = pa ? 2 : 0;
  const bool need_vlo = pf == 2 && opt("attn_pv_split") != 0;
  const int L = x.H * x.W;
  const bool p3 = pf == 0 && e->cfg.stream_f32 == 1 && L % 32 == 0 && a.C % 32 == 0 && p3_ok(e, e->convs[a.qkv]) && p3_ok(e, e->convs[a.out]);
  TRY(op_gn(e, e->norms[a.gn], x, nullptr, 0, e->cfg.vae_eps, &hn, p3 ? kFmtP3 : -1));
  TRY(linear(e, a.qkv, hn, &qkv, 3 * a.C, pf, nullptr, false, need_vlo ? -1 : 2 * a.C));
  tfree(e, hn);
  ao = talloc(e, x.N, x.H, x.W, a.C, e->act_f32);
  const half_t* q = (const half_t*)qkv.p;
  AttnPrec ap; ap.out_f32 = ao.f32; ap.prec = pa ? pf - 1 : 0;
  ap.q_lo = ap.k_lo = ap.v_lo = (long)qkv.rows() * qkv.C;
  TRY(op_attention_raw(e, q, 3 * a.C, q ? q + a.C : nullptr, 3 * a.C, q ? q + 2 * a.C : nullptr, 3 * a.C, nullptr, x.N, 1, L, L, a.C,
                       ao.p, a.C, false, nullptr, ap));
  tfree(e, qkv);
  if (p3) { T ap3; TRY(op_to_p3(e, ao, &ap3)); tfree(e, ao); ao = ap3; }
  TRY(linear(e, a.out, ao, out, a.C, e->cfg.stream_f32, &x, true));
  tfree(e, ao);
  return 0;
}

static int unet_attn_plane_fmt(const sdm_ctx* e) { return (e->cfg.precise_mask & SDM_PRECISE_UNET_ATTN) ? (attn_f8_enabled() ? 3 : 2) : 0; }

struct CrossPlanes { bool on = false; T k, vt; };
static int cross_planes_build(sdm_ctx* e, const T& uin, CrossPlanes* cp) {
  cp->on = opt("cross_shared") != 0 && unet_attn_plane_fmt(e) == 3 && uin.f32 == 1 && uin.C == 16;
  if (!cp->on) return 0;
  const int B = uin.N, Lk = uin.H * uin.W, ldvt = rup(Lk, 64);
  cp->k = talloc(e, 2 * B, 1, Lk, 64, 0);
  cp->vt = talloc(e, B, 1, 64, ldvt, 0);
  if (e->dry) return 0;
  prof_begin(e, "cross_patch_planes", 0, (double)B * Lk * (16.0 + 64 * 6));
  count_kernel("cross_patch_planes");
  const long nthr = std::max((long)B * Lk * 8, (long)B * 64 * (ldvt / 8));
  SDM_LAUNCH(cross_patch_planes_kernel, dim3((unsigned)((nthr + 255) / 256), 2, 1), dim3(256), 0, e->stream, (const float*)uin.p, B, uin.H, uin.W,
             (half_t*)cp->k.p, (half_t*)cp->k.p + (size_t)B * Lk * 64, (half_t*)cp->vt.p, ldvt);
  prof_end(e);
  return 0;
}
static void cross_planes_free(sdm_ctx* e, CrossPlanes* cp) {
  if (!cp->on) return;
  tfree(e, cp->vt); tfree(e, cp->k);
}

static bool transformer_p3(sdm_ctx* e, const TfB& t, int pf) {
  bool p3 = e->cfg.stream_f32 == 1 && pf == 3 && t.C % 32 == 0;
  for (int l : {t.proj_in, t.qkv1, t.o1, t.q2, t.o2, t.q2s, t.o2s, t.ff1, t.ff2, t.proj_out}) p3 = p3 && p3_ok(e, e->convs[l]);
  return p3;
}

static int cross_attention(sdm_ctx* e, const TfB& t, T& n, const T& uin, const CrossPlanes& cp, int pf, bool p3, bool p3a, const T* res, T* out) {
  const int C = t.C, N = n.N, H = n.H, W = n.W, L = H * W, L0 = uin.H * uin.W, sf = e->cfg.stream_f32;
  const int pa = pf ? 1 : 0;
  const bool need_vlo = pf == 2 && opt("attn_pv_split") != 0;
  T q2, kv, ao;
  TRY(linear(e, cp.on ? t.q2s : t.q2, n, &q2, C, pf));
  tfree(e, n);
  if (!cp.on) TRY(conv_simple(e, t.kv2, uin, &kv, 2 * C, pf, 1, 0, 0, nullptr, 1.0f, false, need_vlo ? -1 : C));
  ao = talloc(e, N, H, W, C, p3a ? kFmtP3 : e->act_f32);
  {
    AttnPrec ap; ap.prec = pa ? pf - 1 : 0; ap.out_f32 = p3a ? 1 : ao.f32; ap.out_p3 = p3a ? 1 : 0;
    ap.q_lo = (long)q2.rows() * q2.C;
    if (cp.on) {
      const half_t* kk = (const half_t*)cp.k.p;
      ap.shared_kv = true; ap.k_lo = (long)N * L0 * 64;
      TRY(op_attention_raw(e, (const half_t*)q2.p, C, kk, 64, (const half_t*)cp.vt.p, 64, nullptr, N, t.heads, L, L0, 64, ao.p, C, true, nullptr, ap));
    } else {
      const half_t* kk = (const half_t*)kv.p;
      ap.k_lo = ap.v_lo = (long)kv.rows() * kv.C;
      TRY(op_attention_raw(e, (const half_t*)q2.p, C, kk, 2 * C, kk ? kk + C : nullptr, 2 * C, nullptr, N, t.heads, L, L0, 64, ao.p, C, true, nullptr, ap));
    }
  }
  tfree(e, q2);
  if (!cp.on) tfree(e, kv);
  if (p3 && !p3a) {
    T ap3;
    TRY(op_to_p3(e, ao, &ap3));
    tfree(e, ao);
    ao = ap3;
  }
  TRY(linear(e, cp.on ? t.o2s : t.o2, ao, out, C, sf, res));
  tfree(e, ao);
  return 0;
}

static int transformer(sdm_ctx* e, const TfB& t, const T& x, const T& uin, const CrossPlanes& cp, bool masked, const float* bias, const int* tiles, T* out) {
  const int sf = e->cfg.stream_f32;
  const int C = t.C, L = x.H * x.W;
  T hn, h, n, qkv, ao, h2, f;
  const int pf = unet_attn_plane_fmt(e);
  const int pa = pf ? 1 : 0;
  const bool need_vlo = pf == 2 && opt("attn_pv_split") != 0;
  const bool p3 = transformer_p3(e, t, pf);
  const int nf = p3 ? kFmtP3 : -1;
  const bool p3a = p3 && L % 32 == 0 && opt("gemm_p3_attn") != 0;
  auto attn_out = [&](T& a) -> int {
    if (!p3 || p3a) return 0;
    T ap;
    TRY(op_to_p3(e, a, &ap));
    tfree(e, a);
    a = ap;
    return 0;
  };
  TRY(op_gn(e, e->norms[t.gn], x, nullptr, 0, e->cfg.unet_tf_gn_eps, &hn, nf));
  TRY(linear(e, t.proj_in, hn, &h, C, sf));
  tfree(e, hn);
  TRY(op_ln(e, e->norms[t.ln1], h, e->cfg.unet_ln_eps, &n, nf));
  TRY(linear(e, t.qkv1, n, &qkv, 3 * C, pf, nullptr, false, need_vlo ? -1 : 2 * C));
  tfree(e, n);
  ao = talloc(e, x.N, x.H, x.W, C, p3a ? kFmtP3 : e->act_f32);
  {
    const half_t* q = (const half_t*)qkv.p;
    AttnPrec ap; ap.prec = pa ? pf - 1 : 0; ap.out_f32 = p3a ? 1 : ao.f32; ap.out_p3 = p3a ? 1 : 0; ap.has_bias = ap.has_tiles = masked;
    ap.q_lo = ap.k_lo = ap.v_lo = (long)qkv.rows() * qkv.C;
    TRY(op_attention_raw(e, q, 3 * C, q ? q + C : nullptr, 3 * C, q ? q + 2 * C : nullptr, 3 * C, bias, x.N, t.heads, L, L, 64, ao.p, C, true, tiles, ap));
  }
  tfree(e, qkv);
  TRY(attn_out(ao));
// ... 1553 lines not shown
```

comfyui-sdmatte_amd/csrc/sdm_hooks.h:

```cpp
#pragma once

struct DevBuf {
  void* p = nullptr;
  DevBuf() = default;
  DevBuf(DevBuf&& o) noexcept : p(o.p) { o.p = nullptr; }
  ~DevBuf() { if (p) dev_free(p); }
  int alloc(size_t n) { return dev_malloc(&p, n); }
  int alloc0(size_t n, void* stream) { const int rc = alloc(n); return rc ? rc : dev_memset(p, 0, n, stream); }
};

struct RestoreInt { int& s; int v; ~RestoreInt() { s = v; } };

struct TempLayer {
  enum { kDma = 1, kW3 = 2, kUp = 4 };
  sdm_ctx* e;
  ConvL L;
  DevBuf w, w_lo, b, w_dma, w3, wup;
  explicit TempLayer(sdm_ctx* c) : e(c) {}
  ~TempLayer() { dev_sync(e->stream); }
  int init(const char* name, int ntaps, int I, int O, int geglu, int split, int layouts, const float* wsrc, const float* bias) {
    L = make_layer(name, ntaps, I, O, geglu, split);
    layer_choose_layouts(L, layouts & kDma, layouts & kDma, layouts & kW3, layouts & kUp);
    SDM_CHECK_DEV(e, w.alloc0(L.w_bytes(), e->stream));
    SDM_CHECK_DEV(e, b.alloc0(L.b_bytes(), e->stream));
// ... 278 lines not shown
  if (gnf) { p.gn_scale = (const float*)gnt.p; p.gn_shift = (const float*)gnt.p + (size_t)N * L.Cin_pad; p.gn_silu = 1; }
  int cfg = tile_cfg >= 0 ? tile_cfg : conv_pick_cfg(ntaps, stride, p);
  int ksplit = 1;
  if (!(p.w_dma && ((ntaps == 9 && stride == 1 && cfg == 0) || (ntaps == 1 && cfg == 4)))) ksplit = conv_pick_ksplit(ntaps, stride, cfg, p);
  if (ksplit > 1 && wsb.alloc((size_t)ksplit * p.M * p.Cout_pad * 4)) return -2.f;
  if (ksplit > 1) fprintf(stderr, "[bench_conv] split-K %d\n", ksplit);
  auto run = [&](const ConvParams& pp) { if (ksplit > 1) launch_conv_splitk(ntaps, stride, cfg, pp, ksplit, (float*)wsb.p, e->stream); else launch_conv(ntaps, stride, cfg, pp, e->stream); };
  if (ablate & 256) {
    DevBuf tr;
    const size_t tb = (size_t)16 * 2 * 384 * 4;
    if (tr.alloc(tb) == 0) {
      dev_memset(tr.p, 0, tb, e->stream);
      ConvParams pt = p; pt.trace = (unsigned int*)tr.p; pt.ablate = ablate & 255; pt.trace_skip = (ablate >> 9) & 7; pt.trace_b0 = ((ablate >> 12) & 0xFF) * 256;
      launch_conv(ntaps, stride, cfg, pt, e->stream);
      std::vector<unsigned int> h(tb / 4);
      (void)dev_memcpy_d2h(h.data(), tr.p, tb, e->stream);
      (void)dev_sync(e->stream);
      for (int b = 0; b < 16; ++b)
        for (int r = 0; r < 2; ++r) {
          const unsigned int* ev = &h[((size_t)b * 2 + r) * 384];
          const int n = (int)ev[383] < 383 ? (int)ev[383] : 383;
          if (!n) continue;
          fprintf(stderr, "[trace] block %d %s n=%d:", pt.trace_b0 + b, r ? "producer" : "consumer", n);
          for (int i = 0; i < n; ++i) fprintf(stderr, " %u", ev[i]);
          fprintf(stderr, "\n");
        }
    }
    p.ablate = ablate & 255;
  }
  return time_launches(e, iters, [&]() { run(p); });
#endif
}

float sdm_bench_attn(sdm_ctx* e, int B, int heads, int Lq, int Lk, int qt, int ablate, int iters) {
  if (e) dev_use(e->device);
  if (!e) return -1.f;
#ifdef SDM_EMU
  return -1.f;
#else
  if (qt & 64) {
    const int ldvt5 = rup(Lk, 64);
    DevBuf q5, k5, v5, o5;
    if (q5.alloc((size_t)B * Lq * 512 * 2) || k5.alloc((size_t)B * Lk * 512 * 2) || v5.alloc((size_t)B * 512 * ldvt5 * 2) || o5.alloc((size_t)B * Lq * 512 * 4)) return -2.f;
    SDM_LAUNCH(fill_random_f16_kernel, dim3(4096), dim3(256), 0, e->stream, (half_t*)q5.p, (long)B * Lq * 512, 3u, 0.3f);
    SDM_LAUNCH(fill_random_f16_kernel, dim3(4096), dim3(256), 0, e->stream, (half_t*)k5.p, (long)B * Lk * 512, 7u, 0.3f);
    SDM_LAUNCH(fill_random_f16_kernel, dim3(4096), dim3(256), 0, e->stream, (half_t*)v5.p, (long)B * 512 * ldvt5, 11u, 1.0f);
    AttnParams p5;
    memset(&p5, 0, sizeof(p5));
    p5.q = (const half_t*)q5.p; p5.q_bs = (long)Lq * 512; p5.ldq = 512; p5.k = (const half_t*)k5.p; p5.k_bs = (long)Lk * 512; p5.ldk = 512;
    p5.vt = (const half_t*)v5.p; p5.vt_hs = (long)512 * ldvt5; p5.vt_bs = p5.vt_hs; p5.ldvt = ldvt5; p5.o = (half_t*)o5.p; p5.o_bs = (long)Lq * 512; p5.ldo = 512; p5.o_f32 = 1;
    p5.Lq = Lq; p5.Lk = Lk; p5.scale_log2e = 0.0441941738f * SDM_LOG2E;
    p5.batch = B; p5.heads = 1; p5.nq_blocks = sdm_cdiv(Lq, 128); p5.q_chunks = 8;
    const unsigned nb5 = (unsigned)(B * p5.q_chunks * sdm_cdiv(p5.nq_blocks, p5.q_chunks));
    return time_launches(e, iters, [&]() {
#define SDM_D512_ABL(A) case A: { auto kp = attn_d512_kernel<A>; SDM_SET_SMEM(kp, ATTN512P_SMEM); SDM_LAUNCH(kp, dim3(nb5), dim3(512), ATTN512P_SMEM, e->stream, p5); } break;
      switch (ablate) { SDM_D512_ABL(0) SDM_D512_ABL(1) SDM_D512_ABL(6) SDM_D512_ABL(7) SDM_D512_ABL(8) SDM_D512_ABL(32) SDM_D512_ABL(40) SDM_D512_ABL(41) default: break; }
#undef SDM_D512_ABL
    });
  }
  const int C = heads * 64, ldvt = rup(Lk, 64);
  const int prec = (qt & 2) ? 1 : 0, nw8 = (qt & 4) ? 1 : 0;
  DevBuf q, k, vt, o;
  if (q.alloc((size_t)B * Lq * C * 2 * (1 + prec)) || k.alloc((size_t)B * Lk * C * 2 * (1 + prec)) ||
      vt.alloc((size_t)B * heads * 64 * ldvt * 2 * (1 + prec)) || o.alloc((size_t)B * Lq * C * (prec ? 4 : 2) + 4096)) return -2.f;
  if (prec) {
    SDM_LAUNCH(fill_random_f16_kernel, dim3(4096), dim3(256), 0, e->stream, (half_t*)q.p + (size_t)B * Lq * C, (long)B * Lq * C, 13u, 0.0003f);
    SDM_LAUNCH(fill_random_f16_kernel, dim3(4096), dim3(256), 0, e->stream, (half_t*)k.p + (size_t)B * Lk * C, (long)B * Lk * C, 17u, 0.0003f);
    SDM_LAUNCH(fill_random_f16_kernel, dim3(4096), dim3(256), 0, e->stream, (half_t*)vt.p + (size_t)B * heads * 64 * ldvt, (long)B * heads * 64 * ldvt, 19u, 0.0003f);
  }
  if (prec && (qt & 16)) {
    (void)hipMemsetAsync((half_t*)q.p + (size_t)B * Lq * C, 0, (size_t)B * Lq * C * 2, (hipStream_t)e->stream);
    (void)hipMemsetAsync((half_t*)k.p + (size_t)B * Lk * C, 0, (size_t)B * Lk * C * 2, (hipStream_t)e->stream);
  }
  SDM_LAUNCH(fill_random_f16_kernel, dim3(4096), dim3(256), 0, e->stream, (half_t*)q.p, (long)B * Lq * C, 3u, 1.0f);
  SDM_LAUNCH(fill_random_f16_kernel, dim3(4096), dim3(256), 0, e->stream, (half_t*)k.p, (long)B * Lk * C, 7u, 1.0f);
  SDM_LAUNCH(fill_random_f16_kernel, dim3(4096), dim3(256), 0, e->stream, (half_t*)vt.p, (long)B * heads * 64 * ldvt, 11u, 1.0f);
  AttnParams p;
  memset(&p, 0, sizeof(p));
  p.q = (const half_t*)q.p; p.q_bs = (long)Lq * C; p.ldq = C; p.k = (const half_t*)k.p; p.k_bs = (long)Lk * C; p.ldk = C;
  p.k_hs = 64;
  p.vt = (const half_t*)vt.p; p.vt_hs = (long)64 * ldvt; p.vt_bs = heads * p.vt_hs; p.ldvt = ldvt; p.o = (half_t*)o.p; p.o_bs = (long)Lq * C; p.ldo = C;
  p.Lq = Lq; p.Lk = Lk; p.scale_log2e = 0.125f * SDM_LOG2E; p.ablate = ablate;
  if (prec) { p.q_lo = (long)B * Lq * C; p.k_lo = (long)B * Lk * C; p.vt_lo = (long)B * p.vt_bs; p.o_f32 = 1; }
  p.batch = B; p.heads = heads; p.nq_blocks = sdm_cdiv(Lq, nw8 ? 256 : 128); p.q_chunks = 8;
  const unsigned nblk = (unsigned)(B * heads * p.q_chunks * sdm_cdiv(p.nq_blocks, p.q_chunks));
  const float ms = time_launches(e, iters, [&]() {
    if (qt & 16) {
      p.pp_flags = (qt & 32) ? 0 : 1;
      p.part_ml = (float*)((unsigned char*)o.p + (size_t)B * Lq * C * 4);
      if (qt & 128) p.pp_flags |= 2;
#define SDM_PP_ABL(A) case A: { auto kp = attn_d64_pp_kernel<A, 0, 0>; SDM_SET_SMEM(kp, 160 * 1024); SDM_LAUNCH(kp, dim3(nblk), dim3(512), ATTN64PP_SMEM + 4096, e->stream, p); } break;
#define SDM_PP_DS(A, S, V) case V: { auto kp = attn_d64_pp_kernel<A, 0, 0, 0, S, 0>; SDM_SET_SMEM(kp, 160 * 1024); SDM_LAUNCH(kp, dim3(nblk), dim3(512), ATTN64PP_SMEM + 4096, e->stream, p); } break;
#define SDM_PP_KE(K, V) case V: { auto kp = attn_d64_pp_kernel<0, 0, 0, K, 1, 0>; SDM_SET_SMEM(kp, 160 * 1024); SDM_LAUNCH(kp, dim3(nblk), dim3(512), ATTN64PP_SMEM, e->stream, p); } break;
      switch (ablate) { SDM_PP_ABL(0) SDM_PP_ABL(1) SDM_PP_ABL(6) SDM_PP_ABL(7) SDM_PP_ABL(8) SDM_PP_ABL(32) SDM_PP_ABL(56) SDM_PP_ABL(63)
                        SDM_PP_KE(-1, 100) SDM_PP_KE(2, 101) SDM_PP_KE(1, 102) SDM_PP_ABL(64)
                        SDM_PP_DS(0, 0, 110) SDM_PP_DS(0, 1, 111) SDM_PP_DS(0, 2, 112) SDM_PP_DS(0, 3, 113) SDM_PP_DS(64, 0, 114) SDM_PP_DS(64, 2, 116) SDM_PP_DS(64, 3, 117) default: break; }
#undef SDM_PP_ABL
#undef SDM_PP_KE
#undef SDM_PP_DS
    }
    else if (prec && (qt & 8) && nw8) { auto kp = attn_d64_kernel<1, 2, 8>; SDM_SET_SMEM(kp, 160 * 1024); SDM_LAUNCH(kp, dim3(nblk), dim3(512), ATTN64P_SMEM, e->stream, p); }
    else if (prec && (qt & 8)) { auto kp = attn_d64_kernel<1, 2, 4>; SDM_SET_SMEM(kp, 160 * 1024); SDM_LAUNCH(kp, dim3(nblk), dim3(256), ATTN64P_SMEM, e->stream, p); }
    else if (prec && nw8) { auto kp = attn_d64_kernel<1, 1, 8>; SDM_SET_SMEM(kp, 160 * 1024); SDM_LAUNCH(kp, dim3(nblk), dim3(512), ATTN64P_SMEM, e->stream, p); }
    else if (prec) { auto kp = attn_d64_kernel<1, 1, 4>; SDM_SET_SMEM(kp, 160 * 1024); SDM_LAUNCH(kp, dim3(nblk), dim3(256), ATTN64P_SMEM, e->stream, p); }
    else if (nw8) { auto kf = attn_d64_kernel<1, 0, 8>; SDM_SET_SMEM(kf, 160 * 1024); SDM_LAUNCH(kf, dim3(nblk), dim3(512), ATTN64P_SMEM, e->stream, p); }
    else { SDM_LAUNCH((attn_d64_kernel<1, 0, 4>), dim3(nblk), dim3(256), ATTN64_SMEM, e->stream, p); }
  });
  if ((qt & 16) && (ablate == 64 || (ablate >= 114 && ablate <= 117))) {
    std::vector<unsigned long long> tr(2 * 8 * 28);
    (void)hipMemcpy(tr.data(), (unsigned char*)o.p + (size_t)B * Lq * C * 4, tr.size() * 8, hipMemcpyDeviceToHost);
    for (int g = 0; g < 2; ++g) {
      double dm = 0, sm = 0, vr = 0, wa = 0, mx = 0, wb = 0; int n = 0;
      for (int t = 5; t < 27; ++t) {
        const unsigned long long* c = &tr[(size_t)g * 224 + (size_t)t * 8];
        const unsigned long long prev3 = tr[(size_t)g * 224 + (size_t)(t - 1) * 8 + 3];
        dm += (double)(c[4] - prev3); sm += (double)(c[5] - c[4]); vr += (double)(c[0] - c[5]); wa += (double)(c[1] - c[0]); mx += (double)(c[2] - c[1]); wb += (double)(c[3] - c[2]); ++n;
      }
      fprintf(stderr, "[attn_pp trace] wave %d: DMA issue %.0f | softmax VALU %.0f | V^T reads + lgkmcnt(0) %.0f | wait at barrier %.0f | matrix segment %.0f | wait at barrier %.0f  (cycles per tile, mean of %d tiles; each stamp costs an s_memtime round trip)\n",
              g * 4, dm / n, sm / n, vr / n, wa / n, mx / n, wb / n, n);
    }
  }
  return ms;
#endif
}

int sdm_op_groupnorm(sdm_ctx* e, const void* in0, const void* in1, int C0, int C1, int in_f32, int N, int HW, int groups, const float* gamma,
                     const float* beta, float eps, int silu, void* out) {
  if (e) dev_use(e->device);
  if (!e || !in0 || !out) return SDM_ERR_INVALID;
  return run_two_pass(e, [&]() { return op_groupnorm_raw(e, in0, in1, C0, C1, in_f32, N, HW, groups, gamma, beta, eps, silu, out, 0); });
}

int sdm_op_layernorm(sdm_ctx* e, const void* x, int in_f32, long rows, int C, const float* gamma, const float* beta, float eps, void* out) {
  if (e) dev_use(e->device);
  if (!e || !x || !out) return SDM_ERR_INVALID;
  if (C % 64 || C > 64 * SDM_LN_MAXV) SDM_FAIL(e, SDM_ERR_INVALID, "layernorm: unsupported C %d", C);
  SDM_LAUNCH(layernorm_kernel, dim3((unsigned)((rows + 3) / 4)), dim3(256), 0, e->stream, x, in_f32, gamma, beta, out, 0, rows, C, eps);
  SDM_CHECK_DEV(e, dev_sync(e->stream));
  return 0;
}

int sdm_op_attention(sdm_ctx* e, const void* q, int ldq, const void* k, int ldk, const void* v, int ldv, const float* bias, int B, int heads,
                     int Lq, int Lk, int D, void* out, int ldo) {
  if (e) dev_use(e->device);
  if (!e || !q || !k || !v || !out) return SDM_ERR_INVALID;
  return run_two_pass(e, [&]() {
    T b2 = talloc(e, B, 1, 1, Lk, 1);
    AttnPrec ap; ap.has_bias = bias != nullptr;
    if (bias && !e->dry) {
      SDM_LAUNCH(scale_copy_kernel, dim3(sdm_cdiv(B * Lk, 256)), dim3(256), 0, e->stream, bias, (float*)b2.p, (long)B * Lk, SDM_LOG2E);
    }
    int rc = op_attention_raw(e, (const half_t*)q, ldq, (const half_t*)k, ldk, (const half_t*)v, ldv, bias ? (const float*)b2.p : nullptr,
                              B, heads, Lq, Lk, D, (half_t*)out, ldo, false, nullptr, ap);
    tfree(e, b2);
    return rc;
  });
}

int sdm_op_attention_split(sdm_ctx* e, const float* q, const float* k, const float* v, const float* bias, int B, int heads, int Lq, int Lk, float* out) {
  return sdm_op_attention_split_ex(e, q, k, v, bias, nullptr, B, heads, Lq, Lk, 0, out, nullptr);
}

int sdm_op_attention_split_ex(sdm_ctx* e, const float* q, const float* k, const float* v, const float* bias, const int* tiles, int B, int heads, int Lq,
                              int Lk, int out_p3, float* out, void* planes) {
  if (e) dev_use(e->device);
  if (!e || !q || !k || !v || !out) return SDM_ERR_INVALID;
  if (out_p3 < 0 || out_p3 > 2 || (tiles && !bias)) SDM_FAIL(e, SDM_ERR_INVALID, "sdm_op_attention_split_ex: out_p3 0..2; a tile list needs the bias");
  const int C = heads * 64;
  const int mode = (attn_f8_enabled() && !opt("attn_pv_split")) ? 3 : 2;
  return run_two_pass(e, [&]() -> int {
    T b2 = talloc(e, B, 1, 1, Lk, 1);
    T qp = talloc(e, B, 1, Lq, C, mode), kp = talloc(e, B, 1, Lk, C, mode), vp = talloc(e, B, 1, Lk, C, mode);
    const long nq = (long)B * Lq * C, nk = (long)B * Lk * C;
    if (!e->dry) {
      if (bias) SDM_LAUNCH(scale_copy_kernel, dim3(sdm_cdiv(B * Lk, 256)), dim3(256), 0, e->stream, bias, (float*)b2.p, (long)B * Lk, SDM_LOG2E);
      SDM_LAUNCH(split_planes_kernel, dim3((unsigned)((nq / 4 + 255) / 256)), dim3(256), 0, e->stream, q, (half_t*)qp.p, (half_t*)qp.p + nq, nq, 0.125f * SDM_LOG2E, mode);
      SDM_LAUNCH(split_planes_kernel, dim3((unsigned)((nk / 4 + 255) / 256)), dim3(256), 0, e->stream, k, (half_t*)kp.p, (half_t*)kp.p + nk, nk, 1.0f, mode);
      SDM_LAUNCH(split_planes_kernel, dim3((unsigned)((nk / 4 + 255) / 256)), dim3(256), 0, e->stream, v, (half_t*)vp.p, (half_t*)vp.p + nk, nk, 1.0f, 2);
    }
    T to, pl;
    if (out_p3) to = talloc(e, B, 1, Lq, C, out_p3 == 1 ? kFmtP3 : 1);
    AttnPrec ap; ap.prec = mode - 1; ap.q_lo = nq; ap.k_lo = nk; ap.v_lo = nk; ap.out_f32 = 1; ap.out_p3 = out_p3 == 1;
    ap.has_bias = bias != nullptr; ap.has_tiles = tiles != nullptr;
    TRY(op_attention_raw(e, (const half_t*)qp.p, C, (const half_t*)kp.p, C, (const half_t*)vp.p, C, bias ? (const float*)b2.p : nullptr, B, heads, Lq, Lk, 64,
                         out_p3 ? to.p : (void*)out, C, true, tiles, ap));
    if (out_p3 == 2) TRY(op_to_p3(e, to, &pl));
    const T& p3 = out_p3 == 2 ? pl : to;
    if (out_p3 && !e->dry) {
      SDM_LAUNCH(from_p3_kernel, dim3((unsigned)std::min<long>(((long)B * Lq * C + 255) / 256, 1 << 20)), dim3(256), 0, e->stream, (const unsigned char*)p3.p, out,
                 (long)B * Lq, C);
      if (planes) SDM_CHECK_DEV(e, dev_memcpy_d2d(planes, p3.p, p3_rows_pad((size_t)B * Lq) * C * 3, e->stream));
    }
    if (out_p3 == 2) tfree(e, pl);
    if (out_p3) tfree(e, to);
    tfree(e, vp); tfree(e, kp); tfree(e, qp); tfree(e, b2);
    return 0;
  });
}

int sdm_op_cross_patch_planes(sdm_ctx* e, const float* uin, int B, int H, int W, void* k_hi, void* k_pair, void* vt) {
  if (e) dev_use(e->device);
  if (!e || !uin || !k_hi || !k_pair || !vt || B < 1 || H < 1 || W < 1) return SDM_ERR_INVALID;
  const int Lk = H * W, ldvt = rup(Lk, 64);
  const long nthr = std::max((long)B * Lk * 8, (long)B * 64 * (ldvt / 8));
  count_kernel("cross_patch_planes");
  SDM_LAUNCH(cross_patch_planes_kernel, dim3((unsigned)((nthr + 255) / 256), 2, 1), dim3(256), 0, e->stream, uin, B, H, W, (half_t*)k_hi, (half_t*)k_pair, (half_t*)vt, ldvt);
  SDM_CHECK_DEV(e, dev_sync(e->stream));
  return 0;
}

int sdm_op_attention_shared(sdm_ctx* e, const float* q, const float* ks, const float* vs, int B, int heads, int Lq, int Lk, int q_prescaled, float* out) {
  if (e) dev_use(e->device);
  if (!e || !q || !ks || !vs || !out) return SDM_ERR_INVALID;
  if (!attn_f8_enabled() || opt("attn_pv_split")) SDM_FAIL(e, SDM_ERR_INVALID, "sdm_op_attention_shared: the fp8-pair plane format only");
  const int C = heads * 64, ldvt = rup(Lk, 64);
  return run_two_pass(e, [&]() -> int {
    T qp = talloc(e, B, 1, Lq, C, 3), kp = talloc(e, B, 1, Lk, 64, 3), vp = talloc(e, B, 1, Lk, 64, 2), vt = talloc(e, B, 1, 64, ldvt, 0);
    const long nq = (long)B * Lq * C, nk = (long)B * Lk * 64;
    if (!e->dry) {
      SDM_LAUNCH(split_planes_kernel, dim3((unsigned)((nq / 4 + 255) / 256)), dim3(256), 0, e->stream, q, (half_t*)qp.p, (half_t*)qp.p + nq, nq,
                 q_prescaled ? 1.0f : 0.125f * SDM_LOG2E, 3);
      SDM_LAUNCH(split_planes_kernel, dim3((unsigned)((nk / 4 + 255) / 256)), dim3(256), 0, e->stream, ks, (half_t*)kp.p, (half_t*)kp.p + nk, nk, 1.0f, 3);
      SDM_LAUNCH(split_planes_kernel, dim3((unsigned)((nk / 4 + 255) / 256)), dim3(256), 0, e->stream, vs, (half_t*)vp.p, (half_t*)vp.p + nk, nk, 1.0f, 2);
      SDM_LAUNCH(transpose_v_kernel, dim3(ldvt / 64, 1, B), dim3(256), 0, e->stream, (const half_t*)vp.p, (long)Lk * 64, 64, (half_t*)vt.p, (long)64 * ldvt,
                 (long)64 * ldvt, ldvt, Lk, 64);
    }
    AttnPrec ap; ap.prec = 2; ap.q_lo = nq; ap.k_lo = nk; ap.out_f32 = 1; ap.shared_kv = true;
    TRY(op_attention_raw(e, (const half_t*)qp.p, C, (const half_t*)kp.p, 64, (const half_t*)vt.p, 64, nullptr, B, heads, Lq, Lk, 64, (void*)out, C, true, nullptr, ap));
    tfree(e, vt); tfree(e, vp); tfree(e, kp); tfree(e, qp);
    return 0;
  });
}

int sdm_debug_cross_attention(sdm_ctx* e, const char* block, const float* x, int B, int H, int W, const float* uin, int h, int w, float* out) {
  if (e) dev_use(e->device);
  if (!e || !block || !x || !uin || !out) return SDM_ERR_INVALID;
  if (!e->finalized) SDM_FAIL(e, SDM_ERR_STATE, "weights not finalised");
  if (!e->act_f32 || e->cfg.stream_f32 != 1) SDM_FAIL(e, SDM_ERR_INVALID, "sdm_debug_cross_attention: fp32 activations and stream expected");
  std::vector<const TfB*> blocks;
  for (auto& v : e->u_down_tf) for (auto& t : v) blocks.push_back(&t);
  blocks.push_back(&e->u_midtf);
  for (auto& v : e->u_up_tf) for (auto& t : v) blocks.push_back(&t);
  const TfB* tb = nullptr;
  for (const TfB* t : blocks) if (e->convs[t->q2].name == std::string(block) + ".transformer_blocks.0.attn2.to_q") tb = t;
  if (!tb) SDM_FAIL(e, SDM_ERR_INVALID, "no transformer block named %s", block);
  const int C = tb->C;
  return run_two_pass(e, [&]() -> int {
    const int pf = unet_attn_plane_fmt(e);
    const bool p3 = transformer_p3(e, *tb, pf), p3a = p3 && (H * W) % 32 == 0 && opt("gemm_p3_attn") != 0;
    const T tu = view(uin, B, h, w, 16, 1), tx = view(x, B, H, W, C, 1);
    CrossPlanes cp;
    TRY(cross_planes_build(e, tu, &cp));
    T n = tx, o;
    if (p3) TRY(op_to_p3(e, tx, &n));
    TRY(cross_attention(e, *tb, n, tu, cp, pf, p3, p3a, nullptr, &o));
    if (!e->dry) SDM_CHECK_DEV(e, dev_memcpy_d2d(out, o.p, (size_t)B * H * W * C * 4, e->stream));
    tfree(e, o);
    cross_planes_free(e, &cp);
    return 0;
  });
}

int sdm_debug_attn_plan(int B, int heads, int Lq, int Lk, int D, int prec, int out_f32, int has_bias, int has_tiles, int cus, char* kernel, int cap,
                        int* nsplit) {
  if (B < 1 || heads < 1 || Lq < 1 || Lk < 1 || cus < 1 || prec < 0 || prec > 2 || !(D == 64 || (D == 512 && heads == 1 && !prec))) return SDM_ERR_INVALID;
  OptReadLock opt_lock;
  const AttnPlan pl = attn_plan(B, heads, Lq, Lk, D, prec, out_f32, has_bias != 0, has_tiles != 0, cus);
  if (kernel && cap > 0) snprintf(kernel, (size_t)cap, "%s", kAttnKernels[pl.kernel].counter);
  if (nsplit) *nsplit = pl.nsplit;
  return SDM_OK;
}

int sdm_op_resize_aa(sdm_ctx* e, const float* in, int P, int Hin, int Win, float* out, int Hout, int Wout) {
  if (e) dev_use(e->device);
  if (!e || !in || !out) return SDM_ERR_INVALID;
  SDM_LAUNCH(resize_planes_kernel, dim3((unsigned)(((long)P * Hout * Wout + 255) / 256)), dim3(256), 0, e->stream, in, out, P, Hin, Win, Hout, Wout, 0);
  SDM_CHECK_DEV(e, dev_sync(e->stream));
  return 0;
}

int sdm_op_mask_bias(sdm_ctx* e, const float* plane, int B, int S, int level, float* out) {
  if (e) dev_use(e->device);
  if (!e || !plane || !out) return SDM_ERR_INVALID;
  const int lk = (S / 8) >> level;
  SDM_LAUNCH(mask_bias_kernel, dim3(sdm_cdiv(B * lk * lk, 256)), dim3(256), 0, e->stream, plane, out, B, S, S, level, e->cfg.attn_mask_value, 1.0f);
  SDM_CHECK_DEV(e, dev_sync(e->stream));
  return 0;
}

}
```

comfyui-sdmatte_amd/engine.py:

```python
import ctypes as C
import os

import numpy as np
import torch

from .config import SDMatteConfig

_HERE = os.path.dirname(os.path.abspath(__file__))
LIB_PATH = os.path.join(_HERE, "csrc", "libsdmatte_hip.so")

SDM_PTR_HOST, SDM_PTR_DEVICE = 0, 1
SDM_F32, SDM_F16, SDM_BF16 = 0, 1, 2
_DT = {torch.float32: SDM_F32, torch.float16: SDM_F16, torch.bfloat16: SDM_BF16}


class SdmConfig(C.Structure):
    _fields_ = [
        ("vae_channels", C.c_int32 * 4), ("vae_layers_per_block", C.c_int32),
        ("unet_channels", C.c_int32 * 4), ("unet_heads", C.c_int32 * 4), ("unet_layers_per_block", C.c_int32),
        ("cross_attention_dim", C.c_int32), ("unet_in_channels", C.c_int32), ("unet_out_channels", C.c_int32),
        ("bbox_embeddings_input_dim", C.c_int32), ("groups", C.c_int32),
        ("vae_eps", C.c_float), ("unet_res_eps", C.c_float), ("unet_tf_gn_eps", C.c_float), ("unet_ln_eps", C.c_float),
        ("vae_scaling_factor", C.c_float), ("attn_mask_value", C.c_float),
        ("stream_f32", C.c_int32), ("point_embeddings_input_dim", C.c_int32), ("precise_mask", C.c_int32), ("reserved", C.c_int32 * 5),
    ]


PRECISE_VAE_ENC, PRECISE_VAE_DEC, PRECISE_VAE_ATTN_LIN, PRECISE_UNET_RES, PRECISE_UNET_TF, PRECISE_UNET_ATTN = 1, 2, 4, 8, 16, 32
PRECISE_ALL = 63
PRECISIONS = {
    "fp16": 0,
    "fp16x3": PRECISE_ALL,
}
DEFAULT_PRECISION = os.environ.get("SDMATTE_PRECISION", "fp16x3")


def precise_mask_of(precision) -> int:
    if precision is None:
        precision = DEFAULT_PRECISION
    if isinstance(precision, int):
        return precision & PRECISE_ALL
    if precision not in PRECISIONS:
        raise ValueError(f"unknown precision {precision!r}; expected one of {sorted(PRECISIONS)} or a stage bit mask")
    return PRECISIONS[precision]


def to_c_config(cfg: SDMatteConfig, stream_f32: bool = True, precision=None) -> SdmConfig:
    c = SdmConfig()
    for i in range(4):
        c.vae_channels[i] = cfg.vae_channels[i]
        c.unet_channels[i] = cfg.unet_channels[i]
        c.unet_heads[i] = cfg.unet_heads[i]
    c.vae_layers_per_block = cfg.vae_layers_per_block
    c.unet_layers_per_block = cfg.unet_layers_per_block
    c.cross_attention_dim = cfg.cross_attention_dim
    c.unet_in_channels = cfg.unet_in_channels
    c.unet_out_channels = cfg.unet_out_channels
    c.bbox_embeddings_input_dim = cfg.bbox_embeddings_input_dim
    c.groups = cfg.unet_groups
    c.vae_eps, c.unet_res_eps = cfg.vae_eps, cfg.unet_res_eps
    c.unet_tf_gn_eps, c.unet_ln_eps = cfg.unet_tf_gn_eps, cfg.unet_ln_eps
    c.vae_scaling_factor, c.attn_mask_value = cfg.vae_scaling_factor, cfg.attn_mask_value
    c.stream_f32 = 1 if stream_f32 else 0
    c.point_embeddings_input_dim = cfg.point_embeddings_input_dim
    c.precise_mask = precise_mask_of(precision)
    return c


EXPORTS = [
    "sdm_default_config", "sdm_create", "sdm_destroy", "sdm_last_error", "sdm_load_tensor", "sdm_finalize_weights",
    "sdm_weight_stats", "sdm_missing_key", "sdm_weight_blob_bytes", "sdm_export_weight_blob", "sdm_import_weight_blob",
    "sdm_host_blob_bytes", "sdm_export_host_blob", "sdm_import_host_blob", "sdm_forward", "sdm_forward_ex", "sdm_forward_rect", "sdm_apply_matte", "sdm_apply_matte_node",
    "sdm_make_trimap", "sdm_clean_mask", "sdm_apply_matte_mask", "sdm_subject_roi", "sdm_apply_matte_roi", "sdm_subject_boxes", "sdm_apply_matte_boxes", "sdm_estimate_foreground", "sdm_refine_alpha_guided", "sdm_compose_canvas",
    "sdm_synchronize", "sdm_release_memory", "sdm_resident_bytes", "sdm_weight_bytes", "sdm_last_forward_ms", "sdm_profile_enable", "sdm_profile_count", "sdm_profile_get", "sdm_profile_dump",
    "sdm_op_conv", "sdm_op_conv_ex", "sdm_op_conv_up_stats", "sdm_op_gemm_p3", "sdm_debug_run_layer", "sdm_debug_set_input_cmask", "sdm_debug_temb_row", "sdm_conv_num_cfgs", "sdm_bench_conv", "sdm_bench_attn", "sdm_bench_gemm_p3", "sdm_op_groupnorm", "sdm_op_layernorm", "sdm_op_attention", "sdm_op_attention_split", "sdm_op_attention_split_ex", "sdm_debug_attn_plan", "sdm_op_resize_aa",
    "sdm_op_mask_bias", "sdm_op_cross_patch_planes", "sdm_op_attention_shared", "sdm_debug_cross_attention",
    "sdm_set_option", "sdm_get_option", "sdm_reset_options", "sdm_option_name", "sdm_option_help", "sdm_kernel_counts", "sdm_kernel_counts_reset",
]


class Bindings:

    def __init__(self, cdll):
        self.dll = cdll
        vp, i32, i64, f32 = C.c_void_p, C.c_int, C.c_int64, C.c_float
        sig = {
            "sdm_default_config": (None, [C.POINTER(SdmConfig)]),
            "sdm_create": (i32, [C.POINTER(vp), i32, C.POINTER(SdmConfig)]),
            "sdm_destroy": (None, [vp]),
            "sdm_last_error": (C.c_char_p, [vp]),
            "sdm_load_tensor": (i32, [vp, C.c_char_p, i32, i32, C.POINTER(i64), vp]),
            "sdm_finalize_weights": (i32, [vp]),
            "sdm_weight_stats": (i32, [vp, C.POINTER(i64), C.POINTER(i64), C.POINTER(i64)]),
            "sdm_missing_key": (C.c_char_p, [vp, i64]),
            "sdm_weight_blob_bytes": (i64, [vp]),
            "sdm_export_weight_blob": (i32, [vp, vp]),
            "sdm_import_weight_blob": (i32, [vp, vp]),
            "sdm_host_blob_bytes": (i64, [vp]),
            "sdm_export_host_blob": (i32, [vp, vp]),
            "sdm_import_host_blob": (i32, [vp, vp]),
            "sdm_forward": (i32, [vp, vp, vp, i32, i32, vp, vp, vp, i32, vp]),
            "sdm_forward_ex": (i32, [vp, vp, vp, i32, i32, vp, vp, i32, i32, i32, vp, i32, vp]),
            "sdm_forward_rect": (i32, [vp, vp, vp, i32, i32, i32, vp, vp, i32, i32, i32, vp, i32, vp]),
            "sdm_apply_matte": (i32, [vp, vp, vp, i32, i32, i32, i32, i32, vp, i32, vp]),
            "sdm_apply_matte_node": (i32, [vp, vp, vp, i32, i32, i32, i32, i32, i32, i32, i32, i32, C.c_double, vp, vp, i32, vp]),
            "sdm_make_trimap": (i32, [vp, vp, i32, i32, i32, f32, i32, i32, vp, i32, vp]),
            "sdm_clean_mask": (i32, [vp, vp, i32, i32, i32, f32, i32, i32, i32, i32, vp, vp, i32, vp]),
            "sdm_apply_matte_mask": (i32, [vp, vp, vp, i32, i32, i32, i32, i32, i32, i32, f32, i32, i32, i32, i32, C.c_double, vp, vp, vp, i32, vp]),
            "sdm_subject_roi": (i32, [vp, vp, i32, i32, i32, f32, i32, i32, i32, vp, i32, vp]),
            "sdm_apply_matte_roi": (i32, [vp, vp, vp, i32, i32, i32, i32, i32, i32, f32, i32, i32, f32, i32, i32, i32, i32, i32, C.c_double, vp, vp, vp, vp, i32, vp]),
            "sdm_subject_boxes": (i32, [vp, vp, i32, i32, i32, f32, i32, i32, i32, i32, i32, vp, vp, i32, vp]),
            "sdm_apply_matte_boxes": (i32, [vp, vp, vp, i32, i32, i32, i32, i32, vp, i32, i32, i32, C.c_double, vp, vp, i32, vp]),
            "sdm_estimate_foreground": (i32, [vp, vp, vp, i32, i32, i32, f32, f32, i32, i32, vp, i32, vp, i32, vp]),
            "sdm_refine_alpha_guided": (i32, [vp, vp, vp, i32, i32, i32, i32, i32, f32, vp, i32, vp]),
            "sdm_compose_canvas": (i32, [vp, vp, vp, i32, i32, i32, f32, i32, i32, i32, i32, i32, vp, vp, i32, f32, f32, i32, i32, vp, i32, vp, i32, vp]),
            "sdm_synchronize": (i32, [vp]),
            "sdm_release_memory": (i32, [vp]),
            "sdm_resident_bytes": (i64, [vp]),
            "sdm_weight_bytes": (i64, [vp]),
            "sdm_last_forward_ms": (f32, [vp]),
            "sdm_profile_enable": (i32, [vp, i32]),
            "sdm_profile_count": (i32, [vp]),
            "sdm_profile_dump": (C.c_char_p, [vp]),
            "sdm_profile_get": (i32, [vp, i32, C.POINTER(C.c_char_p), C.POINTER(f32), C.POINTER(i64), C.POINTER(C.c_double),
                                      C.POINTER(C.c_double)]),
            "sdm_op_conv": (i32, [vp, vp, vp, i32, i32, i32, i32, i32, i32, i32, i32, i32, i32, vp, vp, i32, vp, i32, vp, i32, i32,
                                  f32, i32]),
            "sdm_op_conv_ex": (i32, [vp, vp, vp, i32, i32, i32, i32, i32, i32, i32, i32, i32, i32, vp, vp, i32, vp, i32, vp, i32, i32,
                                     f32, i32, i32, vp, vp, f32, i32, i32]),
            "sdm_op_gemm_p3": (i32, [vp, vp, i32, i32, i32, i32, vp, vp, i32, i32, vp, vp, vp, f32, i32, vp, vp, C.POINTER(i32)]),
            "sdm_op_conv_up_stats": (i32, [vp, vp, i32, i32, i32, i32, vp, vp, i32, vp, vp, C.POINTER(i32)]),
            "sdm_debug_run_layer": (i32, [vp, C.c_char_p, vp, i32, i32, i32, vp, i32]),
            "sdm_debug_set_input_cmask": (i32, [vp, vp]),
            "sdm_debug_temb_row": (i32, [vp, i32, i32, vp, vp, i32]),
            "sdm_conv_num_cfgs": (i32, [i32, i32]),
            "sdm_bench_conv": (f32, [vp] + [i32] * 11),
            "sdm_bench_attn": (f32, [vp] + [i32] * 7),
            "sdm_bench_gemm_p3": (f32, [vp, C.c_long, i32, i32, i32, i32]),
            "sdm_op_groupnorm": (i32, [vp, vp, vp, i32, i32, i32, i32, i32, i32, vp, vp, f32, i32, vp]),
            "sdm_op_layernorm": (i32, [vp, vp, i32, C.c_long, i32, vp, vp, f32, vp]),
            "sdm_op_attention": (i32, [vp, vp, i32, vp, i32, vp, i32, vp, i32, i32, i32, i32, i32, vp, i32]),
            "sdm_op_attention_split": (i32, [vp, vp, vp, vp, vp, i32, i32, i32, i32, vp]),
            "sdm_op_attention_split_ex": (i32, [vp, vp, vp, vp, vp, vp, i32, i32, i32, i32, i32, vp, vp]),
            "sdm_debug_attn_plan": (i32, [i32] * 10 + [C.c_char_p, i32, C.POINTER(i32)]),
            "sdm_op_resize_aa": (i32, [vp, vp, i32, i32, i32, vp, i32, i32]),
            "sdm_op_mask_bias": (i32, [vp, vp, i32, i32, i32, vp]),
            "sdm_op_cross_patch_planes": (i32, [vp, vp, i32, i32, i32, vp, vp, vp]),
            "sdm_op_attention_shared": (i32, [vp, vp, vp, vp, i32, i32, i32, i32, i32, vp]),
            "sdm_debug_cross_attention": (i32, [vp, C.c_char_p, vp, i32, i32, i32, vp, i32, i32, vp]),
            "sdm_set_option": (i32, [C.c_char_p, i32]),
            "sdm_get_option": (i32, [C.c_char_p, C.POINTER(i32)]),
            "sdm_reset_options": (None, []),
            "sdm_option_name": (C.c_char_p, [i32]),
            "sdm_option_help": (C.c_char_p, [i32]),
            "sdm_kernel_counts": (i32, [C.c_char_p, i32]),
            "sdm_kernel_counts_reset": (None, []),
        }
        for name in EXPORTS:
            fn = getattr(cdll, name)
            fn.restype, fn.argtypes = sig[name]
            setattr(self, name, fn)

    def set_option(self, name, value):
        if self.sdm_set_option(name.encode(), int(value)) != 0:
            raise KeyError(f"unknown engine option {name!r}; known: {', '.join(self.options())}")

    def get_option(self, name):
        v = C.c_int(0)
        if self.sdm_get_option(name.encode(), C.byref(v)) != 0:
            raise KeyError(name)
        return v.value

    def options(self):
        out, i = {}, 0
        while True:
            n = self.sdm_option_name(i)
            if n is None:
                return out
            out[n.decode()] = self.sdm_option_help(i).decode()
            i += 1

    def reset_options(self):
        self.sdm_reset_options()

    def attn_plan(self, B, heads, Lq, Lk, cus, D=64, prec=2, out_f32=True, has_bias=False, has_tiles=False):
        buf, ns = C.create_string_buffer(64), C.c_int(0)
        if self.sdm_debug_attn_plan(B, heads, Lq, Lk, D, prec, int(out_f32), int(has_bias), int(has_tiles), cus, buf, 64, C.byref(ns)) != 0:
            raise ValueError(f"sdm_debug_attn_plan: unsupported attention B={B} heads={heads} Lq={Lq} Lk={Lk} D={D} prec={prec}")
        return buf.value.decode(), ns.value

    def kernel_counts(self, reset=False):
        n = self.sdm_kernel_counts(None, 0)
        buf = C.create_string_buffer(n + 1)
        self.sdm_kernel_counts(buf, n + 1)
        out = {}
        for item in buf.value.decode().split(";"):
            if item:
                k, v = item.rsplit("=", 1)
                out[k] = int(v)
        if reset:
# ... 609 lines not shown
            n = N * H * W_ * O
            return out[:n].view(N, H, W_, O), out[n:].view(torch.uint8).view(N, H, W_, O, 2)
        if mode == 4:
            return out, stats[:N * srows.value * O * 2].view(N, srows.value, O, 2)
        return out

    def debug_run_layer(self, name, x_nhwc, cout):
        N, H, W_, _ = x_nhwc.shape
        x = x_nhwc.float().contiguous()
        out = torch.empty(N, H, W_, cout, dtype=torch.float32, device=x.device)
        self._check(self.lib.sdm_debug_run_layer(self.h, name.encode(), _ptr(x), N, H, W_, _ptr(out), cout), "sdm_debug_run_layer")
        return out

    def debug_temb_row(self, index, is_trans, coords, cout):
        out = np.zeros(cout, np.float32)
        co = None if coords is None else np.ascontiguousarray(np.asarray(coords, np.float32).reshape(4))
        self._check(self.lib.sdm_debug_temb_row(self.h, index, int(is_trans), co.ctypes.data_as(C.c_void_p) if co is not None else None,
                                                out.ctypes.data_as(C.c_void_p), cout), "sdm_debug_temb_row")
        return torch.from_numpy(out)

    def bench_conv(self, N, H, W, Cin, Cout, ntaps=9, stride=1, in_f32=0, tile_cfg=-1, ablate=0, iters=10):
        return float(self.lib.sdm_bench_conv(self.h, N, H, W, Cin, Cout, ntaps, stride, in_f32, tile_cfg, ablate, iters))

    def bench_gemm_p3(self, M, K, O, epi=0, res=False, iters=10):
        return float(self.lib.sdm_bench_gemm_p3(self.h, M, K, O, epi | (256 if res else 0), iters))

    def bench_attn(self, B, heads, Lq, Lk, qt=1, ablate=0, iters=10):
        return float(self.lib.sdm_bench_attn(self.h, B, heads, Lq, Lk, qt, ablate, iters))

    def op_groupnorm(self, x0, gamma, beta, eps, silu, groups=32, x1=None):
        N, H, W_, C0 = x0.shape
        C1 = x1.shape[-1] if x1 is not None else 0
        out = torch.empty(N, H, W_, C0 + C1, dtype=torch.float16, device=x0.device)
        self._check(self.lib.sdm_op_groupnorm(self.h, _ptr(x0), _ptr(x1), C0, C1, int(x0.dtype == torch.float32), N, H * W_, groups,
                                              _ptr(gamma), _ptr(beta), float(eps), int(silu), _ptr(out)), "sdm_op_groupnorm")
        return out

    def op_layernorm(self, x, gamma, beta, eps):
        rows, Cc = x.numel() // x.shape[-1], x.shape[-1]
        out = torch.empty(x.shape, dtype=torch.float16, device=x.device)
        self._check(self.lib.sdm_op_layernorm(self.h, _ptr(x), int(x.dtype == torch.float32), rows, Cc, _ptr(gamma), _ptr(beta),
                                              float(eps), _ptr(out)), "sdm_op_layernorm")
        return out

    def op_attention(self, q, k, v, heads, bias=None):
        B, Lq, HD = q.shape
        Lk = k.shape[1]
        D = HD // heads
        out = torch.empty(B, Lq, HD, dtype=torch.float16, device=q.device)
        self._check(self.lib.sdm_op_attention(self.h, _ptr(q), q.stride(1), _ptr(k), k.stride(1), _ptr(v), v.stride(1), _ptr(bias), B,
                                              heads, Lq, Lk, D, _ptr(out), HD), "sdm_op_attention")
        return out

    def op_attention_split(self, q, k, v, heads, bias=None, out_p3=0, tiles=None, planes=False):
        B, Lq, HD = q.shape
        Lk = k.shape[1]
        qf, kf, vf = q.float().contiguous(), k.float().contiguous(), v.float().contiguous()
        out = torch.empty(B, Lq, HD, dtype=torch.float32, device=q.device)
        if not out_p3 and tiles is None:
            self._check(self.lib.sdm_op_attention_split(self.h, _ptr(qf), _ptr(kf), _ptr(vf), _ptr(bias), B, heads, Lq, Lk, _ptr(out)), "sdm_op_attention_split")
            return out
        tl = tiles.to(torch.int32).contiguous() if tiles is not None else None
        raw = torch.zeros(((B * Lq + 31) // 32) * 32 * HD * 3, dtype=torch.uint8, device=q.device) if (planes and out_p3) else None
        self._check(self.lib.sdm_op_attention_split_ex(self.h, _ptr(qf), _ptr(kf), _ptr(vf), _ptr(bias), _ptr(tl), B, heads, Lq, Lk, int(out_p3),
                                                       _ptr(out), _ptr(raw)), "sdm_op_attention_split_ex")
        return (out, raw) if raw is not None else out

    def op_cross_patch_planes(self, uin):
        B, H, W_, _ = uin.shape
        L = H * W_
        ldvt = (L + 63) // 64 * 64
        x = uin.float().contiguous()
        k_hi = torch.full((B, L, 64), 7.0, dtype=torch.float16, device=x.device)
        k_pair = torch.full((B, L, 64, 2), 7, dtype=torch.uint8, device=x.device)
        vt = torch.full((B, 64, ldvt), 7.0, dtype=torch.float16, device=x.device)
        self._check(self.lib.sdm_op_cross_patch_planes(self.h, _ptr(x), B, H, W_, _ptr(k_hi), _ptr(k_pair), _ptr(vt)), "sdm_op_cross_patch_planes")
        return k_hi, k_pair, vt

    def op_attention_shared(self, q, ks, vs, heads, q_prescaled=False):
        B, Lq, HD = q.shape
        Lk = ks.shape[1]
        qf, kf, vf = q.float().contiguous(), ks.float().contiguous(), vs.float().contiguous()
        out = torch.empty(B, Lq, HD, dtype=torch.float32, device=q.device)
        self._check(self.lib.sdm_op_attention_shared(self.h, _ptr(qf), _ptr(kf), _ptr(vf), B, heads, Lq, Lk, int(q_prescaled), _ptr(out)), "sdm_op_attention_shared")
        return out

    def debug_cross_attention(self, block, x_nhwc, uin):
        B, H, W_, Cc = x_nhwc.shape
        x, u = x_nhwc.float().contiguous(), uin.float().contiguous()
        out = torch.empty(B, H, W_, Cc, dtype=torch.float32, device=x.device)
        self._check(self.lib.sdm_debug_cross_attention(self.h, block.encode(), _ptr(x), B, H, W_, _ptr(u), u.shape[1], u.shape[2], _ptr(out)), "sdm_debug_cross_attention")
        return out

    def op_resize_aa(self, planes, Hout, Wout):
        P, Hin, Win = planes.shape
        out = torch.empty(P, Hout, Wout, dtype=torch.float32, device=planes.device)
        self._check(self.lib.sdm_op_resize_aa(self.h, _ptr(planes), P, Hin, Win, _ptr(out), Hout, Wout), "sdm_op_resize_aa")
        return out

    def op_mask_bias(self, plane_bss, level):
        B, S, _ = plane_bss.shape
        lk = (S // 8) >> level
        out = torch.empty(B, lk * lk, dtype=torch.float32, device=plane_bss.device)
        self._check(self.lib.sdm_op_mask_bias(self.h, _ptr(plane_bss), B, S, level, _ptr(out)), "sdm_op_mask_bias")
        return out
```

include/sdmatte.h:

```cpp
#ifndef SDMATTE_H_
#define SDMATTE_H_

#include <stddef.h>
#include <stdint.h>

#ifdef __cplusplus
extern "C" {
#endif

typedef struct sdm_ctx sdm_ctx;

enum sdm_status {
  SDM_OK = 0,
  SDM_ERR_INVALID = -1,
  SDM_ERR_HIP = -2,
  SDM_ERR_STATE = -3,
  SDM_ERR_NOMEM = -4,
  SDM_ERR_NODEVICE = -5,
  SDM_ERR_ARENA = -6
};

enum sdm_ptr_kind { SDM_PTR_HOST = 0, SDM_PTR_DEVICE = 1 };
enum sdm_dtype { SDM_F32 = 0, SDM_F16 = 1, SDM_BF16 = 2 };

// ... 113 lines not shown
#define SDM_CANVAS_MAX_SHADOW_SIGMA 32
#define SDM_CANVAS_MAX_SHADOW_RADIUS 96
#define SDM_CANVAS_MAX_SHADOW_OFFSET 4096
int sdm_compose_canvas(sdm_ctx* ctx, const float* fg_bhw3, const float* alpha_bhw, int B, int H, int W, float roi_threshold, int canvas_h, int canvas_w,
                       int fill_pct, int valign, int bg_mode, const float* bg_rgb3, const float* bg_image, int bg_batch, float shadow_opacity,
                       float shadow_sigma, int shadow_dy, int shadow_dx, float* out, int out_channels, int32_t* place_out, int ptr_kind, void* stream);

int64_t sdm_resident_bytes(sdm_ctx* ctx);
int64_t sdm_weight_bytes(sdm_ctx* ctx);
int sdm_release_memory(sdm_ctx* ctx);

int sdm_set_option(const char* name, int value);
int sdm_get_option(const char* name, int* value);
void sdm_reset_options(void);
const char* sdm_option_name(int i);
const char* sdm_option_help(int i);
int sdm_kernel_counts(char* buf, int cap);
void sdm_kernel_counts_reset(void);

int sdm_synchronize(sdm_ctx* ctx);

float sdm_last_forward_ms(sdm_ctx* ctx);

int sdm_profile_enable(sdm_ctx* ctx, int on);
int sdm_profile_count(sdm_ctx* ctx);
const char* sdm_profile_dump(sdm_ctx* ctx);
int sdm_profile_get(sdm_ctx* ctx, int i, const char** name, float* ms, int64_t* launches, double* flops, double* bytes);


int sdm_op_conv(sdm_ctx* ctx, const void* in0, const void* in1, int C0, int C1, int in_f32, int N, int Hin, int Win, int up,
                int stride, int pad_mode, int ntaps, const float* w, const float* bias, int O, void* out, int out_f32,
                const void* res, int res_f32, int geglu, float out_scale, int tile_cfg);
int sdm_conv_num_cfgs(int ntaps, int stride);
int sdm_op_conv_ex(sdm_ctx* ctx, const void* in0, const void* in1, int C0, int C1, int in_f32, int N, int Hin, int Win, int up,
                   int stride, int pad_mode, int ntaps, const float* w, const float* bias, int O, void* out, int out_f32,
                   const void* res, int res_f32, int geglu, float out_scale, int tile_cfg, int split, const float* gn_gamma,
                   const float* gn_beta, float gn_eps, int gn_groups, int gn_silu);
float sdm_bench_gemm_p3(sdm_ctx* ctx, long M, int K, int O, int epi_flags, int iters);
int sdm_op_gemm_p3(sdm_ctx* ctx, const float* x, int N, int H, int W, int K, const float* w, const float* bias, int O, int mode, const float* res,
                   const float* ln_gamma, const float* ln_beta, float ln_eps, int lo_cols, void* out, float* stats, int* srows);
int sdm_op_conv_up_stats(sdm_ctx* ctx, const float* x, int N, int H, int W, int C, const float* w, const float* bias, int O, float* out, float* stats,
                         int* srows);
int sdm_debug_set_input_cmask(sdm_ctx* ctx, const unsigned char* mask);
int sdm_debug_run_layer(sdm_ctx* ctx, const char* layer_name, const float* x_nhwc, int N, int H, int W, float* out_nhwc, int Cout);
int sdm_debug_temb_row(sdm_ctx* ctx, int temb_index, int is_trans, const float* coords4, float* out_host, int cout);
float sdm_bench_attn(sdm_ctx* ctx, int B, int heads, int Lq, int Lk, int qt, int ablate, int iters);
float sdm_bench_conv(sdm_ctx* ctx, int N, int H, int W, int Cin, int Cout, int ntaps, int stride, int in_f32, int tile_cfg, int ablate, int iters);
int sdm_op_groupnorm(sdm_ctx* ctx, const void* in0, const void* in1, int C0, int C1, int in_f32, int N, int HW, int groups,
                     const float* gamma, const float* beta, float eps, int silu, void* out_f16);
int sdm_op_layernorm(sdm_ctx* ctx, const void* x, int in_f32, long rows, int C, const float* gamma, const float* beta,
                     float eps, void* out_f16);
int sdm_op_attention(sdm_ctx* ctx, const void* q, int ldq, const void* k, int ldk, const void* v, int ldv, const float* bias,
                     int B, int heads, int Lq, int Lk, int D, void* out, int ldo);
int sdm_op_attention_split(sdm_ctx* ctx, const float* q, const float* k, const float* v, const float* bias, int B, int heads, int Lq, int Lk, float* out);
int sdm_op_attention_split_ex(sdm_ctx* ctx, const float* q, const float* k, const float* v, const float* bias, const int* tiles, int B, int heads, int Lq,
                              int Lk, int out_p3, float* out, void* planes);
int sdm_op_cross_patch_planes(sdm_ctx* ctx, const float* uin, int B, int H, int W, void* k_hi, void* k_pair, void* vt);
int sdm_op_attention_shared(sdm_ctx* ctx, const float* q, const float* ks, const float* vs, int B, int heads, int Lq, int Lk, int q_prescaled, float* out);
int sdm_debug_cross_attention(sdm_ctx* ctx, const char* block, const float* x, int B, int H, int W, const float* uin, int h, int w, float* out);
int sdm_debug_attn_plan(int B, int heads, int Lq, int Lk, int D, int prec, int out_f32, int has_bias, int has_tiles, int cus, char* kernel, int cap,
                        int* nsplit);
int sdm_op_resize_aa(sdm_ctx* ctx, const float* in, int P, int Hin, int Win, float* out, int Hout, int Wout);
int sdm_op_mask_bias(sdm_ctx* ctx, const float* trimap_plane, int B, int S, int level, float* bias_out);

#ifdef __cplusplus
}
#endif
#endif
```

Baseline: 22.25.

## Add narrow cross-attention path folding softmax row-sum into a ones V row

Adds a NARROW template variant of the d64 attention kernels that drops the last fp16 head-dim slice of the QK product. It also drops the separate ones-matrix MFMA used for the softmax denominator and reads the denominator from a V column filled with ones (o[1][15]). This removes one QK MFMA step and one row-sum MFMA per tile for the cross-attentions, at the cost of relying on cross-patch planes built with a ones row and narrower effective head data. It also factors the d512 output store into a helper, adds a new pipelined d512 kernel, and exposes new host entry points.

```diff
diff --git a/comfyui-sdmatte_amd/csrc/k_attn.h b/comfyui-sdmatte_amd/csrc/k_attn.h
--- a/comfyui-sdmatte_amd/csrc/k_attn.h
+++ b/comfyui-sdmatte_amd/csrc/k_attn.h
@@ -461,9 +461,10 @@
 #define ATTN64PIPE4_KB (2 * 64 * ATTN64_PK + 256)
 #define ATTN64PIPE4_VB (64 * ATTN64_PV)
 #define ATTN64PIPE4_SMEM (2 * ATTN64PIPE4_KB + 3 * ATTN64PIPE4_VB)
-template <int NW>
+template <int NW, int NARROW = 0>
 __global__ void __launch_bounds__(64 * NW, 2) attn_d64_pipe_kernel(AttnParams p) {
   constexpr int NTH = 64 * NW, VPT = 512 / NTH;
+  constexpr int NKS = NARROW ? 3 : 4;
   constexpr bool SPLITBUF = NW == 4;
   SDM_DYN_SMEM(smem);
   constexpr int PK = ATTN64_PK, PV = ATTN64_PV, BUF = ATTN64P_BUF;
@@ -484,7 +485,7 @@
     if (qrow > p.Lq - 1) qrow = p.Lq - 1;
     const half_t* qp = p.q + (size_t)b * p.q_bs + (size_t)qrow * p.ldq + head * 64 + hi * 8;
 #pragma unroll
-    for (int ks = 0; ks < 4; ++ks) qf[ks] = *(const f16x8*)(qp + ks * 16);
+    for (int ks = 0; ks < NKS; ++ks) qf[ks] = *(const f16x8*)(qp + ks * 16);
     const half_t* qb = p.q + (size_t)b * p.q_bs + p.q_lo + (size_t)qrow * p.ldq + head * 64 + hi * 16;
 #pragma unroll
     for (int m = 0; m < 2; ++m) {
@@ -561,7 +562,7 @@
 #pragma unroll
     for (int kt = 0; kt < 2; ++kt) {
 #pragma unroll
-      for (int ks = 0; ks < 4; ++ks) {
+      for (int ks = 0; ks < NKS; ++ks) {
         const f16x8 a = *(const f16x8*)(Ks + (kt * 32 + l31) * PK + ks * 32 + hi * 16);
         s[kt] = SDM_MFMA_32x32x16_F16(a, qf[ks], s[kt]);
       }
@@ -604,8 +605,10 @@
 #pragma unroll
       for (int r = 0; r < 16; ++r) sc[kt][r] = sdm_exp2(sc[kt][r] - mnew);
     if (__any(alpha != 1.0f)) {
-#pragma unroll
-      for (int r = 0; r < 16; ++r) ls[r] *= alpha;
+      if (!NARROW) {
+#pragma unroll
+        for (int r = 0; r < 16; ++r) ls[r] *= alpha;
+      }
 #pragma unroll
       for (int dt = 0; dt < 2; ++dt)
 #pragma unroll
@@ -621,7 +624,7 @@
         f16x8 pf;
 #pragma unroll
         for (int j = 0; j < 8; ++j) pf[j] = (half_t)sc[kt][8 * u + j];
-        ls = SDM_MFMA_32x32x16_F16(ones, pf, ls);
+        if (!NARROW) ls = SDM_MFMA_32x32x16_F16(ones, pf, ls);
 #pragma unroll
         for (int dt = 0; dt < 2; ++dt) {
           const unsigned char* vp = Vs + (dt * 32 + l31) * PV + (kt * 32 + 16 * u + 4 * hi) * 2;
@@ -642,11 +645,12 @@
 
   constexpr int PS = 272;
   unsigned char* stf = smem + wave * (32 * PS);
-  const float inv = p.nsplit > 1 ? 1.0f : 1.0f / ls[0];
+  const float den = NARROW ? o[1][15] : ls[0];
+  const float inv = p.nsplit > 1 ? 1.0f : 1.0f / den;
   float* obase = (float*)p.o + (p.nsplit > 1 ? (size_t)sp * p.part_stride : (size_t)0) + (size_t)b * p.o_bs;
   if (p.nsplit > 1 && hi == 0 && q0 + l31 < p.Lq) {
     float* ml = p.part_ml + ((((size_t)sp * p.batch + b) * p.heads + head) * p.Lq + q0 + l31) * 2;
-    ml[0] = m_i; ml[1] = ls[0];
+    ml[0] = m_i; ml[1] = den;
   }
 #pragma unroll
   for (int dt = 0; dt < 2; ++dt)
@@ -670,8 +674,10 @@
 
 #define ATTN64PP_SLOT (3 * 8192 + 256)
 #define ATTN64PP_SMEM (6 * ATTN64PP_SLOT)
-template <int ABL = 0, int BIAS = 1, int LIST = 1, int KE = 0, int DS = 1, int OB = 1>
+template <int ABL = 0, int BIAS = 1, int LIST = 1, int KE = 0, int DS = 1, int OB = 1, int NARROW = 0>
 __global__ void __launch_bounds__(512, 2) attn_d64_pp_kernel(AttnParams p) {
+  static_assert(!NARROW || !BIAS, "the narrow form serves the cross-attentions: no key bias");
+  constexpr int NKS = NARROW ? 3 : 4;
   SDM_DYN_SMEM(smem);
   constexpr int SLOT = ATTN64PP_SLOT, KLO = 8192, VOFF = 16384, BOFF = 24576;
   constexpr int R = KE < 0 ? 4 : 6, D = KE < 0 ? 3 : 4;
@@ -690,7 +696,7 @@
     if (qrow > p.Lq - 1) qrow = p.Lq - 1;
     const half_t* qp = p.q + (size_t)b * p.q_bs + (size_t)qrow * p.ldq + head * 64 + hi * 8;
 #pragma unroll
-    for (int ks = 0; ks < 4; ++ks) qf[ks] = *(const f16x8*)(qp + ks * 16);
+    for (int ks = 0; ks < NKS; ++ks) qf[ks] = *(const f16x8*)(qp + ks * 16);
     const half_t* qb = p.q + (size_t)b * p.q_bs + p.q_lo + (size_t)qrow * p.ldq + head * 64 + hi * 16;
 #pragma unroll
     for (int m = 0; m < 2; ++m) {
@@ -769,7 +775,7 @@
     if (ABL & 32) { SDM_PIN_HERE_V4(f.h[0], f.h[1], f.h[2], f.h[3]); SDM_PIN_HERE_V4(f.f8[0], f.f8[1], f.h[0], f.h[1]); return; }
     const unsigned char* Ks = smem + slot * SLOT + kt * 4096;
 #pragma unroll
-    for (int ks = 0; ks < 4; ++ks) f.h[ks] = *(const f16x8*)(Ks + (kx ^ (ks * 32)));
+    for (int ks = 0; ks < NKS; ++ks) f.h[ks] = *(const f16x8*)(Ks + (kx ^ (ks * 32)));
 #pragma unroll
     for (int m = 0; m < 2; ++m) {
       const i32x4 a0 = *(const i32x4*)(Ks + KLO + (k8x ^ (m * 64))), a1 = *(const i32x4*)(Ks + KLO + ((k8x ^ (m * 64)) ^ 16));
@@ -779,7 +785,7 @@
   auto mma_k = [&](const KFrag& f, f32x16& sk) {
     if (ABL & 4) return;
 #pragma unroll
-    for (int ks = 0; ks < 4; ++ks) sk = SDM_MFMA_32x32x16_F16(f.h[ks], qf[ks], sk);
+    for (int ks = 0; ks < NKS; ++ks) sk = SDM_MFMA_32x32x16_F16(f.h[ks], qf[ks], sk);
 #pragma unroll
     for (int m = 0; m < 2; ++m) sk = SDM_MFMA_32x32x64_BF8_BF8(f.f8[m], q8p[m], sk, 127 - 11, 127);
   };
@@ -796,7 +802,7 @@
     if (ABL & 2) return;
 #pragma unroll
     for (int u = 0; u < 2; ++u) {
-      ls = SDM_MFMA_32x32x16_F16(ones, pk[u], ls);
+      if (!NARROW) ls = SDM_MFMA_32x32x16_F16(ones, pk[u], ls);
 #pragma unroll
       for (int dt = 0; dt < 2; ++dt) o[dt] = SDM_MFMA_32x32x16_F16(f.v[u][dt], pk[u], o[dt]);
     }
@@ -839,8 +845,10 @@
     mid0();
     SDM_SCHED_FENCE();
     if (__any(alpha != 1.0f)) {
-#pragma unroll
-      for (int r = 0; r < 16; ++r) ls[r] *= alpha;
+      if (!NARROW) {
+#pragma unroll
+        for (int r = 0; r < 16; ++r) ls[r] *= alpha;
+      }
 #pragma unroll
       for (int dt = 0; dt < 2; ++dt)
 #pragma unroll
@@ -914,7 +922,7 @@
     if (KE < 2) load_k(b1, 1, k1);
     if (KE < 1) {
 #pragma unroll
-      for (int i = 0; i < 12; ++i) { SDM_SCHED_GROUP(0x008, 1, 0); SDM_SCHED_GROUP(0x100, 2, 0); SDM_SCHED_GROUP(0x002, 1, 0); }
+      for (int i = 0; i < (NARROW ? 8 : 12); ++i) { SDM_SCHED_GROUP(0x008, 1, 0); SDM_SCHED_GROUP(0x100, 2, 0); SDM_SCHED_GROUP(0x002, 1, 0); }
     } else if (KE < 2) {
 #pragma unroll
       for (int i = 0; i < 8; ++i) { SDM_SCHED_GROUP(0x008, 1, 0); SDM_SCHED_GROUP(0x100, 1, 0); }
@@ -947,11 +955,12 @@
 
   constexpr int PS = 272;
   unsigned char* stf = smem + wave * (32 * PS);
-  const float inv = p.nsplit > 1 ? 1.0f : 1.0f / ls[0];
+  const float den = NARROW ? o[1][15] : ls[0];
+  const float inv = p.nsplit > 1 ? 1.0f : 1.0f / den;
   float* obase = (float*)p.o + (p.nsplit > 1 ? (size_t)sp * p.part_stride : (size_t)0) + (size_t)b * p.o_bs;
   if (p.nsplit > 1 && hi == 0 && q0 + l31 < p.Lq) {
     float* ml = p.part_ml + ((((size_t)sp * p.batch + b) * p.heads + head) * p.Lq + q0 + l31) * 2;
-    ml[0] = m_i; ml[1] = ls[0];
+    ml[0] = m_i; ml[1] = den;
   }
 #pragma unroll
   for (int dt = 0; dt < 2; ++dt)
@@ -970,6 +979,67 @@
     const int qg = q0 + row;
     if (qg < p.Lq)
       *(f32x4*)(obase + (size_t)qg * p.ldo + head * 64 + part * 4) = *(const f32x4*)(stf + row * PS + part * 16);
+  }
+}
+
+SDM_DEV_INLINE void attn512_store(const AttnParams& p, unsigned char* smem, f32x16 (&o)[8], float l_i, int b, int q0, int dh, int wave, int lane) {
+  const int hi = lane >> 5, l31 = lane & 31;
+  l_i += __shfl_xor(l_i, 32);
+  const float inv = 1.0f / l_i;
+  if (p.o_f32) {
+    constexpr int PF = 528;
+    unsigned char* stf = smem + wave * (32 * PF);
+#pragma unroll
+    for (int half = 0; half < 2; ++half) {
+      __syncthreads();
+#pragma unroll
+      for (int d4 = 0; d4 < 4; ++d4) {
+        const int dt = half * 4 + d4;
+#pragma unroll
+        for (int g = 0; g < 4; ++g) {
+          f32x4 h;
+#pragma unroll
+          for (int e = 0; e < 4; ++e) h[e] = o[dt][4 * g + e] * inv;
+          *(f32x4*)(stf + l31 * PF + (d4 * 32 + 8 * g + 4 * hi) * 4) = h;
+        }
+      }
+      __syncthreads();
+#pragma unroll
+      for (int pass = 0; pass < 16; ++pass) {
+        const int row = pass * 2 + (lane >> 5), part = lane & 31;
+        const int qg = q0 + row;
+        if (qg < p.Lq)
+          *(f32x4*)((float*)p.o + (size_t)b * p.o_bs + (size_t)qg * p.ldo + dh * 256 + half * 128 + part * 4) =
+              *(const f32x4*)(stf + row * PF + part * 16);
+      }
+    }
+    return;
+  }
+  constexpr int PS = 272;
+  unsigned char* stg = smem + wave * (32 * PS);
+#pragma unroll
+  for (int half = 0; half < 2; ++half) {
+    __syncthreads();
+#pragma unroll
+    for (int d4 = 0; d4 < 4; ++d4) {
+      const int dt = half * 4 + d4;
+#pragma unroll
+      for (int g = 0; g < 4; ++g) {
+        f16x4 h;
+#pragma unroll
+        for (int e = 0; e < 4; ++e) h[e] = (half_t)(o[dt][4 * g + e] * inv);
+        *(f16x4*)(stg + l31 * PS + (d4 * 32 + 8 * g + 4 * hi) * 2) = h;
+      }
+    }
+    __syncthreads();
+#pragma unroll
+    for (int pass = 0; pass < 8; ++pass) {
+      const int row = pass * 4 + (lane >> 4), part = lane & 15;
+      const int qg = q0 + row;
+      if (qg < p.Lq)
+        *(f16x8*)(p.o + (size_t)b * p.o_bs + (size_t)qg * p.ldo + dh * 256 + half * 128 + part * 8) =
+            *(const f16x8*)(stg + row * PS + part * 16);
+    }
   }
 }
 
@@ -1134,63 +1204,185 @@
     SDM_RAW_BARRIER();
   }
 
-  l_i += __shfl_xor(l_i, 32);
-  const float inv = 1.0f / l_i;
-  if (p.o_f32) {
-    constexpr int PF = 528;
-    unsigned char* stf = smem + wave * (32 * PF);
-#pragma unroll
-    for (int half = 0; half < 2; ++half) {
-      __syncthreads();
-#pragma unroll
-      for (int d4 = 0; d4 < 4; ++d4) {
-        const int dt = half * 4 + d4;
-#pragma unroll
-        for (int g = 0; g < 4; ++g) {
-          f32x4 h;
-#pragma unroll
-          for (int e = 0; e < 4; ++e) h[e] = o[dt][4 * g + e] * inv;
-          *(f32x4*)(stf + l31 * PF + (d4 * 32 + 8 * g + 4 * hi) * 4) = h;
+  attn512_store(p, smem, o, l_i, b, q0, dh, wave, lane);
+}
+
+template <int ABL = 0>
+__global__ void __launch_bounds__(512) attn_d512_pp_kernel(AttnParams p) {
+  SDM_DYN_SMEM(smem);
+  float* Xs = (float*)(smem + ATTN512P_X_OFF);
+  const int tid = threadIdx.x, lane = tid & 63, wave = SDM_UNIFORM_I(tid >> 6);
+  const int hi = lane >> 5, l31 = lane & 31;
+  const int qgp = wave >> 1, dh = wave & 1, grp = wave >> 2;
+  int b, head_unused, qblk;
+  if (!attn_block_coords(p, blockIdx.x, b, head_unused, qblk)) return;
+  const int q0 = qblk * 128 + qgp * 32;
+
+  f16x8 qf[16];
+  {
+    int qrow = q0 + l31;
+    if (qrow > p.Lq - 1) qrow = p.Lq - 1;
+    const half_t* qp = p.q + (size_t)b * p.q_bs + (size_t)qrow * p.ldq + dh * 256 + hi * 8;
+#pragma unroll
+    for (int ks = 0; ks < 16; ++ks) qf[ks] = *(const f16x8*)(qp + ks * 16);
+  }
+  f32x16 o[8];
+#pragma unroll
+  for (int dt = 0; dt < 8; ++dt)
+#pragma unroll
+    for (int r = 0; r < 16; ++r) o[dt][r] = 0.0f;
+  float m_i = SDM_NEG_BIG, l_i = 0.0f;
+
+  const half_t* kbase = p.k + (size_t)b * p.k_bs;
+  const half_t* vbase = p.vt + (size_t)b * p.vt_bs;
+  const int ntiles = (p.Lk + 31) / 32;
+
+  const sdm_rsrc rsK = sdm_make_rsrc(kbase, (unsigned int)((size_t)p.Lk * p.ldk * 2));
+  const sdm_rsrc rsV = sdm_make_rsrc(vbase, (unsigned int)((size_t)512 * p.ldvt * 2));
+  const unsigned int v_voff = (unsigned int)((lane >> 2) * p.ldvt * 2 + (((lane & 3) ^ ((lane >> 4) & 3)) * 16));
+  int lane16 = lane * 16;
+  auto issue_k = [&](int t) {
+    if ((ABL & 8) || t >= ntiles) return;
+    const int k0 = t * 32;
+    unsigned char* Kd = smem + (t & 1) * ATTN512P_K_BYTES;
+    SDM_OPAQUE_I(lane16);
+#pragma unroll
+    for (int i = 0; i < 4; ++i) {
+      const int rho = 4 * wave + i;
+      const int pi = (rho & 16) | (((rho >> 2) & 1) << 3) | (((rho >> 3) & 1) << 2) | (rho & 3);
+      int kr = k0 + pi;
+      if (kr > p.Lk - 1) kr = p.Lk - 1;
+      sdm_glds16_buf(rsK, (unsigned int)(lane16 ^ ((rho & 15) * 16)), (unsigned int)kr * (unsigned int)(p.ldk * 2), Kd + rho * 1024);
+    }
+  };
+  auto issue_v = [&](int t) {
+    if ((ABL & 8) || t >= ntiles) return;
+    const int k0 = t * 32;
+    unsigned char* Vd = smem + 2 * ATTN512P_K_BYTES + (t & 1) * ATTN512P_V_BYTES;
+#pragma unroll
+    for (int i = 0; i < 4; ++i) {
+      const int g = 4 * wave + i;
+      sdm_glds16_buf(rsV, v_voff, (unsigned int)((16 * g * p.ldvt + k0) * 2), Vd + g * 1024);
+    }
+  };
+  int kx = (l31 * 1024 + dh * 512) ^ ((hi ^ (l31 & 15)) * 16);
+  int vx = (dh * 256 + l31) * 64 + ((hi ^ ((l31 >> 2) & 3)) * 16);
+  auto lds_barrier = [&]() { SDM_SCHED_FENCE(); SDM_WAIT_LGKMCNT0(); SDM_RAW_BARRIER(); SDM_SCHED_FENCE(); };
+  float* xme = Xs + wave * (16 * 64);
+  const float* xpt = Xs + (wave ^ 1) * (16 * 64);
+
+  f32x16 s;
+  f16x8 pf[2];
+  auto matrix = [&](int tv, bool pv) {
+    const unsigned char* Vs = smem + 2 * ATTN512P_K_BYTES + (tv & 1) * ATTN512P_V_BYTES;
+    const unsigned char* Ks = smem + ((tv + 1) & 1) * ATTN512P_K_BYTES;
+    SDM_OPAQUE_I(kx);
+    SDM_OPAQUE_I(vx);
+    f16x8 a[4];
+    const int i0 = pv ? 0 : 16;
+    auto rd = [&](int i) -> f16x8 {
+      if (ABL & 32) return qf[(i + 1) & 15];
+      if (i < 16) return *(const f16x8*)(Vs + (vx ^ ((i >> 3) * 32)) + (i & 7) * 2048);
+      return *(const f16x8*)(Ks + (kx ^ ((i - 16) * 32)));
+    };
+#pragma unroll
+    for (int i = 0; i < 3; ++i) a[i] = rd(i0 + i);
+#pragma unroll
+    for (int i = 0; i < 32; ++i) {
+      if (i < i0) continue;
+      if (i + 3 < 32) a[(i + 3) & 3] = rd(i + 3);
+      if (i < 16) { if (!(ABL & 2)) o[i & 7] = SDM_MFMA_32x32x16_F16(a[i & 3], pf[i >> 3], o[i & 7]); }
+      else if (i == 16) {
+        const f32x16 z = {0.f, 0.f, 0.f, 0.f, 0.f, 0.f, 0.f, 0.f, 0.f, 0.f, 0.f, 0.f, 0.f, 0.f, 0.f, 0.f};
+        if (!(ABL & 4)) s = SDM_MFMA_32x32x16_F16(a[0], qf[0], z); else s = z;
+      } else if (!(ABL & 4)) s = SDM_MFMA_32x32x16_F16(a[i & 3], qf[i - 16], s);
+    }
+    if (!(ABL & 38)) {
+      SDM_SCHED_GROUP(0x100, 3, 0);
+      if (pv) {
+#pragma unroll
+        for (int i = 0; i < 29; ++i) { SDM_SCHED_GROUP(0x100, 1, 0); SDM_SCHED_GROUP(0x008, 1, 0); }
+      } else {
+#pragma unroll
+        for (int i = 0; i < 13; ++i) { SDM_SCHED_GROUP(0x100, 1, 0); SDM_SCHED_GROUP(0x008, 1, 0); }
+      }
+      SDM_SCHED_GROUP(0x008, 3, 0);
+    }
+    SDM_SCHED_FENCE();
+    if (!(ABL & 1)) {
+#pragma unroll
+      for (int r = 0; r < 16; ++r) xme[r * 64 + lane] = s[r];
+    }
+  };
+
+  issue_k(0); issue_v(0); issue_k(1);
+  SDM_WAIT_VMCNT0();
+  lds_barrier();
+  if (grp) {
+    if (p.pp_flags & 1) SDM_SETPRIO(1);
+    lds_barrier();
+  }
+  matrix(-1, false);
+  lds_barrier();
+  for (int t = 0; t < ntiles; ++t) {
+    const int k0 = t * 32;
+    if (grp) { issue_v(t + 1); issue_k(t + 2); }
+    float mx = SDM_NEG_BIG;
+    if (!(ABL & 1)) {
+      if (k0 + 32 > p.Lk) {
+#pragma unroll
+        for (int r = 0; r < 16; ++r) {
+          const int key = k0 + 16 * (r >> 3) + 8 * hi + (r & 7);
+          float x = (s[r] + xpt[r * 64 + lane]) * p.scale_log2e;
+          if (key >= p.Lk) x = SDM_NEG_BIG;
+          s[r] = x;
+          mx = fmaxf(mx, x);
         }
-      }
-      __syncthreads();
-#pragma unroll
-      for (int pass = 0; pass < 16; ++pass) {
-        const int row = pass * 2 + (lane >> 5), part = lane & 31;
-        const int qg = q0 + row;
-        if (qg < p.Lq)
-          *(f32x4*)((float*)p.o + (size_t)b * p.o_bs + (size_t)qg * p.ldo + dh * 256 + half * 128 + part * 4) =
-              *(const f32x4*)(stf + row * PF + part * 16);
-      }
-    }
-    return;
-  }
-  constexpr int PS = 272;
-  unsigned char* stg = smem + wave * (32 * PS);
-#pragma unroll
-  for (int half = 0; half < 2; ++half) {
-    __syncthreads();
-#pragma unroll
-    for (int d4 = 0; d4 < 4; ++d4) {
-      const int dt = half * 4 + d4;
-#pragma unroll
-      for (int g = 0; g < 4; ++g) {
-        f16x4 h;
-#pragma unroll
-        for (int e = 0; e < 4; ++e) h[e] = (half_t)(o[dt][4 * g + e] * inv);
-        *(f16x4*)(stg + l31 * PS + (d4 * 32 + 8 * g + 4 * hi) * 2) = h;
-      }
-    }
-    __syncthreads();
-#pragma unroll
-    for (int pass = 0; pass < 8; ++pass) {
-      const int row = pass * 4 + (lane >> 4), part = lane & 15;
-      const int qg = q0 + row;
-      if (qg < p.Lq)
-        *(f16x8*)(p.o + (size_t)b * p.o_bs + (size_t)qg * p.ldo + dh * 256 + half * 128 + part * 8) =
-            *(const f16x8*)(stg + row * PS + part * 16);
-    }
-  }
+      } else {
+#pragma unroll
+        for (int r = 0; r < 16; ++r) {
+          const float x = (s[r] + xpt[r * 64 + lane]) * p.scale_log2e;
+          s[r] = x;
+          mx = fmaxf(mx, x);
+        }
+      }
+      mx = fmaxf(mx, __shfl_xor(mx, 32));
+      const float mnew = fmaxf(m_i, mx);
+      const float alpha = sdm_exp2(m_i - mnew);
+      m_i = mnew;
+      float rs = 0.0f;
+#pragma unroll
+      for (int r = 0; r < 16; ++r) {
+        const float pv = sdm_exp2(s[r] - mnew);
+        s[r] = pv;
+        rs += pv;
+      }
+      l_i = l_i * alpha + rs;
+      if (__any(alpha != 1.0f)) {
+#pragma unroll
+        for (int dt = 0; dt < 8; ++dt)
+#pragma unroll
+          for (int r = 0; r < 16; ++r) o[dt][r] *= alpha;
+      }
+    } else l_i = 1.0f;
+#pragma unroll
+    for (int u = 0; u < 2; ++u)
+#pragma unroll
+      for (int j = 0; j < 8; ++j) pf[u][j] = (half_t)s[8 * u + j];
+    SDM_PIN_HERE_V2(pf[0], pf[1]);
+    if (!grp) SDM_WAIT_VMCNT0();
+    lds_barrier();
+    if (!grp) { issue_v(t + 1); issue_k(t + 2); }
+    matrix(t, true);
+    if (grp) SDM_WAIT_VMCNT0();
+    lds_barrier();
+  }
+  if (!grp) lds_barrier();
+  SDM_WAIT_VMCNT0();
+  int tid_e = threadIdx.x;
+  SDM_OPAQUE_I(tid_e);
+  const int wave_e = SDM_UNIFORM_I(tid_e >> 6);
+  attn512_store(p, smem, o, l_i, b, qblk * 128 + (wave_e >> 1) * 32, wave_e & 1, wave_e, tid_e & 63);
 }
 
 __global__ void __launch_bounds__(256) attn_combine_kernel(const float* __restrict__ part_o, const float* __restrict__ part_ml, float* __restrict__ out,
diff --git a/comfyui-sdmatte_amd/csrc/k_misc.h b/comfyui-sdmatte_amd/csrc/k_misc.h
--- a/comfyui-sdmatte_amd/csrc/k_misc.h
+++ b/comfyui-sdmatte_amd/csrc/k_misc.h
@@ -182,7 +182,7 @@
   return uin[((size_t)b * H * W + (size_t)y * W + x) * 16 + 4 + ci];
 }
 __global__ void __launch_bounds__(256) cross_patch_planes_kernel(const float* __restrict__ uin, int B, int H, int W, half_t* __restrict__ k_hi,
-                                                                 half_t* __restrict__ k_pair, half_t* __restrict__ vt, int ldvt) {
+                                                                 half_t* __restrict__ k_pair, half_t* __restrict__ vt, int ldvt, int ones_rows) {
   const long t = (long)blockIdx.x * blockDim.x + threadIdx.x;
   const int Lk = H * W;
   if (blockIdx.y == 0) {
@@ -213,7 +213,11 @@
     for (int g = 0; g < 2; ++g) {
       f16x4 oh;
 #pragma unroll
-      for (int e = 0; e < 4; ++e) oh[e] = (half_t)fminf(fmaxf(cross_patch_value(uin, H, W, b, chunk * 8 + g * 4 + e, j), -57344.0f), 57344.0f);
+      for (int e = 0; e < 4; ++e) {
+        const int key = chunk * 8 + g * 4 + e;
+        const float x = (ones_rows && (j == 59 || j == 63) && key < Lk) ? 1.0f : cross_patch_value(uin, H, W, b, key, j);
+        oh[e] = (half_t)fminf(fmaxf(x, -57344.0f), 57344.0f);
+      }
       const u32x2 hw = __builtin_bit_cast(u32x2, oh);
       hv[2 * g] = hw[0]; hv[2 * g + 1] = hw[1];
     }
diff --git a/comfyui-sdmatte_amd/csrc/sdm_common.h b/comfyui-sdmatte_amd/csrc/sdm_common.h
--- a/comfyui-sdmatte_amd/csrc/sdm_common.h
+++ b/comfyui-sdmatte_amd/csrc/sdm_common.h
@@ -140,6 +140,7 @@
 #define SDM_UNIFORM_I(x) (x)
 #define SDM_OPAQUE_I(x) ((void)0)
 #define SDM_PIN_HERE_V4(a, b, c, d) ((void)0)
+#define SDM_PIN_HERE_V2(a, b) ((void)0)
 #define SDM_WAIT_VMCNT0() ((void)0)
 #define SDM_WAIT_VMCNT(n) ((void)0)
 #define SDM_WAIT_LGKMCNT0() ((void)0)
@@ -160,6 +161,7 @@
 #define SDM_UNIFORM_I(x) __builtin_amdgcn_readfirstlane(x)
 #define SDM_OPAQUE_I(x) asm volatile("" : "+v"(x))
 #define SDM_PIN_HERE_V4(a, b, c, d) asm volatile("" : "+v"(a), "+v"(b), "+v"(c), "+v"(d))
+#define SDM_PIN_HERE_V2(a, b) asm volatile("" : "+v"(a), "+v"(b))
 #define SDM_WAIT_VMCNT0() asm volatile("s_waitcnt vmcnt(0)" ::: "memory")
 #define SDM_WAIT_VMCNT(n) asm volatile("s_waitcnt vmcnt(" #n ")" ::: "memory")
 #define SDM_WAIT_LGKMCNT0() asm volatile("s_waitcnt lgkmcnt(0)" ::: "memory")
diff --git a/comfyui-sdmatte_amd/csrc/sdm_engine.cpp b/comfyui-sdmatte_amd/csrc/sdm_engine.cpp
--- a/comfyui-sdmatte_amd/csrc/sdm_engine.cpp
+++ b/comfyui-sdmatte_amd/csrc/sdm_engine.cpp
@@ -109,6 +109,8 @@
   {"attn_pp", 1, 1, "split-precision d=64 attention with fp32 output as a ping-pong of the block's wave halves (attn_d64_pp_kernel, 256 query rows per block): 0 off, 1 on, 2 on without the static priority of the younger half, 3 on with per-segment priority flips"},
   {"attn_pp_min_blocks", 128, 128, "attn_pp: launches with fewer 256-row blocks than this keep the 4-wave pipelines (0 in tests: the ping-pong kernel at any size)"},
   {"attn_ksplit", 0, 0, "key split of the d=64 split-precision attention: 0 by launch size (blocks that do not fill the chip's block slots a whole number of times), 1 off, 2 / 4 forced, 3 forced on the ping-pong kernel (ignored elsewhere: those launches run unsplit)"},
+  {"attn512_pp", 0, 0, "d=512 attention (VAE mid-block): the ping-pong kernel (the block's two wave halves one phase apart, attn_d512_pp_kernel; bit-identical): 1 with s_setprio 1 for waves 4-7, 2 without (A/B), 0 = attn_d512_kernel.  Off until its step time has been measured against attn_d512_kernel (profiles/NOTES.md)"},
+  {"cross_narrow", 1, 1, "cross_shared: the narrow form of the d = 64 cores on the shared operand (36 live columns: no Q.K^T step over columns 48..63, the softmax denominator from a row of ones in V^T instead of its own MFMAs; bit-identical).  0 = the full d = 64 program on an operand without the ones rows.  Read per forward"},
   {"cross_shared", 1, 1, "cross-attention on ONE key / value operand per forward, the patch matrix of the trimap latent (cross_patch_planes_kernel), with the K|V fold moved into q_shared / out_shared: 0 = every block's own kv_folded conv + transpose.  Read per forward"},
   {"precise_mask", -1, -1, "stages in split precision (-1 = the config's own mask; per-stage attribution experiments; read at sdm_create)"},
 #ifdef SDM_EMU
@@ -1325,10 +1327,10 @@
   return 0;
 }
 
-struct AttnPrec { int prec = 0; long q_lo = 0, k_lo = 0, v_lo = 0; int out_f32 = 0; int out_p3 = 0; bool has_bias = false, has_tiles = false; bool shared_kv = false; };
-
-enum AttnKernel { kAttnPP, kAttnPPBias, kAttnPPTiles, kAttnPipe8, kAttnPipe4, kAttnP3W8, kAttnP3W4, kAttnP1W8, kAttnP1W4, kAttnP2W8, kAttnP2W4,
-                  kAttnF16W8, kAttnF16W4, kAttnD512 };
+struct AttnPrec { int prec = 0; long q_lo = 0, k_lo = 0, v_lo = 0; int out_f32 = 0; int out_p3 = 0; bool has_bias = false, has_tiles = false; bool shared_kv = false; bool narrow36 = false; };
+
+enum AttnKernel { kAttnPP, kAttnPPBias, kAttnPPTiles, kAttnPPNarrow, kAttnPipe8, kAttnPipe4, kAttnPipe4Narrow, kAttnP3W8, kAttnP3W4, kAttnP1W8, kAttnP1W4, kAttnP2W8, kAttnP2W4,
+                  kAttnF16W8, kAttnF16W4, kAttnD512, kAttnD512PP };
 struct AttnPlan {
   AttnKernel kernel;
   const char* spec_counter;
@@ -1339,6 +1341,7 @@
   bool walk_tiles, own_list;
   bool pv_split;
   int pp_flags;
+  bool narrow;
 };
 struct AttnKernelInfo { const char* counter; int threads; size_t smem; void (*launch)(const AttnKernelInfo&, const AttnPlan&, const AttnParams&, void*); };
 template <auto K, int LDS_LIMIT = 160 * 1024>
@@ -1350,8 +1353,10 @@
   {"attn_d64_pp", 512, ATTN64PP_SMEM, attn_launch_t<attn_d64_pp_kernel<0, 0, 0>>},
   {"attn_d64_pp", 512, ATTN64PP_SMEM, attn_launch_t<attn_d64_pp_kernel<0, 1, 0>>},
   {"attn_d64_pp", 512, ATTN64PP_SMEM, attn_launch_t<attn_d64_pp_kernel<0, 1, 1>>},
+  {"attn_d64_pp", 512, ATTN64PP_SMEM, attn_launch_t<attn_d64_pp_kernel<0, 0, 0, 0, 1, 1, 1>>},
   {"attn_d64_pipe<8>", 512, ATTN64PIPE_SMEM, attn_launch_t<attn_d64_pipe_kernel<8>>},
   {"attn_d64_pipe<4>", 256, ATTN64PIPE4_SMEM, attn_launch_t<attn_d64_pipe_kernel<4>>},
+  {"attn_d64_pipe<4>", 256, ATTN64PIPE4_SMEM, attn_launch_t<attn_d64_pipe_kernel<4, 1>>},
   {"attn_d64<prec3,8>", 512, ATTN64P_SMEM, attn_launch_t<attn_d64_kernel<1, 3, 8>>},
   {"attn_d64<prec3,4>", 256, ATTN64P_SMEM, attn_launch_t<attn_d64_kernel<1, 3, 4>>},
   {"attn_d64<prec1,8>", 512, ATTN64P_SMEM, attn_launch_t<attn_d64_kernel<1, 1, 8>>},
@@ -1361,14 +1366,17 @@
   {"attn_d64<fp16,8>", 512, ATTN64P_SMEM, attn_launch_t<attn_d64_kernel<1, 0, 8>>},
   {"attn_d64<fp16,4>", 256, ATTN64_SMEM, attn_launch_t<attn_d64_kernel<1, 0, 4>, 0>},
   {"attn_d512", 512, ATTN512P_SMEM, attn_launch_t<attn_d512_kernel<0>, ATTN512P_SMEM>},
+  {"attn_d512_pp", 512, ATTN512P_SMEM, attn_launch_t<attn_d512_pp_kernel<0>, ATTN512P_SMEM>},
 };
-static AttnPlan attn_plan(int B, int heads, int Lq, int Lk, int D, int prec, int out_f32, bool has_bias, bool has_tiles, int cus) {
+static AttnPlan attn_plan(int B, int heads, int Lq, int Lk, int D, int prec, int out_f32, bool has_bias, bool has_tiles, int cus, bool narrow36 = false) {
   AttnPlan pl;
   memset(&pl, 0, sizeof(pl));
   pl.nsplit = 1;
   bool nw8 = true, pp = false;
   if (D != 64) {
-    pl.kernel = kAttnD512; pl.qrows = 128;
+    const int pp5 = opt("attn512_pp");
+    pl.kernel = pp5 ? kAttnD512PP : kAttnD512; pl.qrows = 128;
+    pl.pp_flags = pp5 == 1 ? 1 : 0;
   } else {
     pl.walk_tiles = has_bias && opt("attn_dense") == 0;
     pl.own_list = pl.walk_tiles && !has_tiles;
@@ -1389,6 +1397,10 @@
     } else {
       pl.kernel = nw8 ? kAttnF16W8 : kAttnF16W4;
     }
+    if (narrow36 && !has_bias && Lk % 64 == 0) {
+      if (pl.kernel == kAttnPP) { pl.kernel = kAttnPPNarrow; pl.narrow = true; }
+      else if (pl.kernel == kAttnPipe4) { pl.kernel = kAttnPipe4Narrow; pl.narrow = true; }
+    }
     if (pp) {
       pl.spec_counter = pl.walk_tiles ? "attn_pp<0,1,1>" : (has_bias ? "attn_pp<0,1,0>" : "attn_pp<0,0,0>");
       pl.pp_flags = opt("attn_pp") == 1 ? 1 : (opt("attn_pp") == 3 ? 2 : 0);
@@ -1418,7 +1430,8 @@
   if (ap.prec == 2 && !q_prescaled) SDM_FAIL(e, SDM_ERR_INVALID, "attention: the fp8-residual form takes pre-scaled queries");
   if (!e->dry && (ap.has_bias != (bias_l2 != nullptr) || ap.has_tiles != (tiles != nullptr)))
     SDM_FAIL(e, SDM_ERR_STATE, "attention: bias / tile list do not match what the sizing pass was told");
-  const AttnPlan pl = attn_plan(B, heads, Lq, Lk, D, ap.prec, ap.out_f32, ap.has_bias, ap.has_tiles, device_cus());
+  if (ap.narrow36 && !ap.shared_kv) SDM_FAIL(e, SDM_ERR_INVALID, "attention: the narrow form exists for the shared key / value operand only");
+  const AttnPlan pl = attn_plan(B, heads, Lq, Lk, D, ap.prec, ap.out_f32, ap.has_bias, ap.has_tiles, device_cus(), ap.narrow36);
   const AttnKernelInfo& ki = kAttnKernels[pl.kernel];
   const int nsplit = pl.nsplit;
   const int ldvt = rup(Lk, 64);
@@ -1487,6 +1500,7 @@
       prof_begin(e, "attn_d64", flops, bytes, adesc);
       count_kernel(ki.counter);
       if (pl.spec_counter) count_kernel(pl.spec_counter);
+      if (pl.narrow) count_kernel("attn_d64_narrow");
       ki.launch(ki, pl, p, e->stream);
       if (nsplit > 1) {
         count_kernel("attn_combine");
@@ -1503,6 +1517,7 @@
       prof_end(e);
     } else {
       prof_begin(e, "attn_d512", flops, bytes);
+      if (pl.kernel == kAttnD512PP) count_kernel(ki.counter);
       ki.launch(ki, pl, p, e->stream);
       prof_end(e);
     }
@@ -1680,10 +1695,11 @@
 
 static int unet_attn_plane_fmt(const sdm_ctx* e) { return (e->cfg.precise_mask & SDM_PRECISE_UNET_ATTN) ? (attn_f8_enabled() ? 3 : 2) : 0; }
 
-struct CrossPlanes { bool on = false; T k, vt; };
+struct CrossPlanes { bool on = false, narrow = false; T k, vt; };
 static int cross_planes_build(sdm_ctx* e, const T& uin, CrossPlanes* cp) {
   cp->on = opt("cross_shared") != 0 && unet_attn_plane_fmt(e) == 3 && uin.f32 == 1 && uin.C == 16;
   if (!cp->on) return 0;
+  cp->narrow = opt("cross_narrow") != 0;
   const int B = uin.N, Lk = uin.H * uin.W, ldvt = rup(Lk, 64);
   cp->k = talloc(e, 2 * B, 1, Lk, 64, 0);
   cp->vt = talloc(e, B, 1, 64, ldvt, 0);
@@ -1692,7 +1708,7 @@
   count_kernel("cross_patch_planes");
   const long nthr = std::max((long)B * Lk * 8, (long)B * 64 * (ldvt / 8));
   SDM_LAUNCH(cross_patch_planes_kernel, dim3((unsigned)((nthr + 255) / 256), 2, 1), dim3(256), 0, e->stream, (const float*)uin.p, B, uin.H, uin.W,
-             (half_t*)cp->k.p, (half_t*)cp->k.p + (size_t)B * Lk * 64, (half_t*)cp->vt.p, ldvt);
+             (half_t*)cp->k.p, (half_t*)cp->k.p + (size_t)B * Lk * 64, (half_t*)cp->vt.p, ldvt, cp->narrow ? 1 : 0);
   prof_end(e);
   return 0;
 }
@@ -1721,7 +1737,7 @@
     ap.q_lo = (long)q2.rows() * q2.C;
     if (cp.on) {
       const half_t* kk = (const half_t*)cp.k.p;
-      ap.shared_kv = true; ap.k_lo = (long)N * L0 * 64;
+      ap.shared_kv = true; ap.narrow36 = cp.narrow; ap.k_lo = (long)N * L0 * 64;
       TRY(op_attention_raw(e, (const half_t*)q2.p, C, kk, 64, (const half_t*)cp.vt.p, 64, nullptr, N, t.heads, L, L0, 64, ao.p, C, true, nullptr, ap));
     } else {
       const half_t* kk = (const half_t*)kv.p;
diff --git a/comfyui-sdmatte_amd/csrc/sdm_hooks.h b/comfyui-sdmatte_amd/csrc/sdm_hooks.h
--- a/comfyui-sdmatte_amd/csrc/sdm_hooks.h
+++ b/comfyui-sdmatte_amd/csrc/sdm_hooks.h
@@ -354,6 +354,14 @@
     p5.Lq = Lq; p5.Lk = Lk; p5.scale_log2e = 0.0441941738f * SDM_LOG2E;
     p5.batch = B; p5.heads = 1; p5.nq_blocks = sdm_cdiv(Lq, 128); p5.q_chunks = 8;
     const unsigned nb5 = (unsigned)(B * p5.q_chunks * sdm_cdiv(p5.nq_blocks, p5.q_chunks));
+    if (qt & 256) {
+      p5.pp_flags = (qt & 32) ? 0 : 1;
+      return time_launches(e, iters, [&]() {
+#define SDM_D512PP_ABL(A) case A: { auto kp = attn_d512_pp_kernel<A>; SDM_SET_SMEM(kp, ATTN512P_SMEM); SDM_LAUNCH(kp, dim3(nb5), dim3(512), ATTN512P_SMEM, e->stream, p5); } break;
+        switch (ablate) { SDM_D512PP_ABL(0) SDM_D512PP_ABL(1) SDM_D512PP_ABL(6) SDM_D512PP_ABL(7) SDM_D512PP_ABL(8) SDM_D512PP_ABL(32) SDM_D512PP_ABL(40) SDM_D512PP_ABL(41) default: break; }
+#undef SDM_D512PP_ABL
+      });
+    }
     return time_launches(e, iters, [&]() {
 #define SDM_D512_ABL(A) case A: { auto kp = attn_d512_kernel<A>; SDM_SET_SMEM(kp, ATTN512P_SMEM); SDM_LAUNCH(kp, dim3(nb5), dim3(512), ATTN512P_SMEM, e->stream, p5); } break;
       switch (ablate) { SDM_D512_ABL(0) SDM_D512_ABL(1) SDM_D512_ABL(6) SDM_D512_ABL(7) SDM_D512_ABL(8) SDM_D512_ABL(32) SDM_D512_ABL(40) SDM_D512_ABL(41) default: break; }
@@ -459,6 +467,17 @@
   });
 }
 
+int sdm_op_attention_ex(sdm_ctx* e, const void* q, int ldq, const void* k, int ldk, const void* v, int ldv, int B, int heads, int Lq, int Lk, int D, int out_f32,
+                        void* out, int ldo) {
+  if (e) dev_use(e->device);
+  if (!e || !q || !k || !v || !out) return SDM_ERR_INVALID;
+  if (out_f32 && D != 512) SDM_FAIL(e, SDM_ERR_INVALID, "sdm_op_attention_ex: fp32 output of fp16 operands exists for head dim 512 only");
+  return run_two_pass(e, [&]() {
+    AttnPrec ap; ap.out_f32 = out_f32 ? 1 : 0;
+    return op_attention_raw(e, (const half_t*)q, ldq, (const half_t*)k, ldk, (const half_t*)v, ldv, nullptr, B, heads, Lq, Lk, D, out, ldo, false, nullptr, ap);
+  });
+}
+
 int sdm_op_attention_split(sdm_ctx* e, const float* q, const float* k, const float* v, const float* bias, int B, int heads, int Lq, int Lk, float* out) {
   return sdm_op_attention_split_ex(e, q, k, v, bias, nullptr, B, heads, Lq, Lk, 0, out, nullptr);
 }
@@ -501,12 +520,15 @@
 }
 
 int sdm_op_cross_patch_planes(sdm_ctx* e, const float* uin, int B, int H, int W, void* k_hi, void* k_pair, void* vt) {
+  return sdm_op_cross_patch_planes_ex(e, uin, B, H, W, k_hi, k_pair, vt, 0);
+}
+int sdm_op_cross_patch_planes_ex(sdm_ctx* e, const float* uin, int B, int H, int W, void* k_hi, void* k_pair, void* vt, int ones_rows) {
   if (e) dev_use(e->device);
   if (!e || !uin || !k_hi || !k_pair || !vt || B < 1 || H < 1 || W < 1) return SDM_ERR_INVALID;
   const int Lk = H * W, ldvt = rup(Lk, 64);
   const long nthr = std::max((long)B * Lk * 8, (long)B * 64 * (ldvt / 8));
   count_kernel("cross_patch_planes");
-  SDM_LAUNCH(cross_patch_planes_kernel, dim3((unsigned)((nthr + 255) / 256), 2, 1), dim3(256), 0, e->stream, uin, B, H, W, (half_t*)k_hi, (half_t*)k_pair, (half_t*)vt, ldvt);
+  SDM_LAUNCH(cross_patch_planes_kernel, dim3((unsigned)((nthr + 255) / 256), 2, 1), dim3(256), 0, e->stream, uin, B, H, W, (half_t*)k_hi, (half_t*)k_pair, (half_t*)vt, ldvt, ones_rows ? 1 : 0);
   SDM_CHECK_DEV(e, dev_sync(e->stream));
   return 0;
 }
@@ -563,6 +585,26 @@
   });
 }
 
+int sdm_op_cross_core(sdm_ctx* e, const float* q, const float* uin, int B, int heads, int Lq, int h, int w, float* out) {
+  if (e) dev_use(e->device);
+  if (!e || !q || !uin || !out || B < 1 || heads < 1 || Lq < 1 || h < 1 || w < 1) return SDM_ERR_INVALID;
+  const int C = heads * 64, Lk = h * w;
+  return run_two_pass(e, [&]() -> int {
+    const T tu = view(uin, B, h, w, 16, 1);
+    CrossPlanes cp;
+    TRY(cross_planes_build(e, tu, &cp));
+    if (!cp.on) SDM_FAIL(e, SDM_ERR_INVALID, "sdm_op_cross_core: the shared operand is off (cross_shared = 0 or another plane format)");
+    T qp = talloc(e, B, 1, Lq, C, 3);
+    const long nq = (long)B * Lq * C;
+    if (!e->dry) SDM_LAUNCH(split_planes_kernel, dim3((unsigned)((nq / 4 + 255) / 256)), dim3(256), 0, e->stream, q, (half_t*)qp.p, (half_t*)qp.p + nq, nq, 1.0f, 3);
+    AttnPrec ap; ap.prec = 2; ap.q_lo = nq; ap.k_lo = (long)B * Lk * 64; ap.out_f32 = 1; ap.shared_kv = true; ap.narrow36 = cp.narrow;
+    TRY(op_attention_raw(e, (const half_t*)qp.p, C, (const half_t*)cp.k.p, 64, (const half_t*)cp.vt.p, 64, nullptr, B, heads, Lq, Lk, 64, (void*)out, C, true, nullptr, ap));
+    tfree(e, qp);
+    cross_planes_free(e, &cp);
+    return 0;
+  });
+}
+
 int sdm_debug_attn_plan(int B, int heads, int Lq, int Lk, int D, int prec, int out_f32, int has_bias, int has_tiles, int cus, char* kernel, int cap,
                         int* nsplit) {
   if (B < 1 || heads < 1 || Lq < 1 || Lk < 1 || cus < 1 || prec < 0 || prec > 2 || !(D == 64 || (D == 512 && heads == 1 && !prec))) return SDM_ERR_INVALID;
diff --git a/comfyui-sdmatte_amd/engine.py b/comfyui-sdmatte_amd/engine.py
--- a/comfyui-sdmatte_amd/engine.py
+++ b/comfyui-sdmatte_amd/engine.py
@@ -73,8 +73,8 @@
     "sdm_host_blob_bytes", "sdm_export_host_blob", "sdm_import_host_blob", "sdm_forward", "sdm_forward_ex", "sdm_forward_rect", "sdm_apply_matte", "sdm_apply_matte_node",
     "sdm_make_trimap", "sdm_clean_mask", "sdm_apply_matte_mask", "sdm_subject_roi", "sdm_apply_matte_roi", "sdm_subject_boxes", "sdm_apply_matte_boxes", "sdm_estimate_foreground", "sdm_refine_alpha_guided", "sdm_compose_canvas",
     "sdm_synchronize", "sdm_release_memory", "sdm_resident_bytes", "sdm_weight_bytes", "sdm_last_forward_ms", "sdm_profile_enable", "sdm_profile_count", "sdm_profile_get", "sdm_profile_dump",
-    "sdm_op_conv", "sdm_op_conv_ex", "sdm_op_conv_up_stats", "sdm_op_gemm_p3", "sdm_debug_run_layer", "sdm_debug_set_input_cmask", "sdm_debug_temb_row", "sdm_conv_num_cfgs", "sdm_bench_conv", "sdm_bench_attn", "sdm_bench_gemm_p3", "sdm_op_groupnorm", "sdm_op_layernorm", "sdm_op_attention", "sdm_op_attention_split", "sdm_op_attention_split_ex", "sdm_debug_attn_plan", "sdm_op_resize_aa",
-    "sdm_op_mask_bias", "sdm_op_cross_patch_planes", "sdm_op_attention_shared", "sdm_debug_cross_attention",
+    "sdm_op_conv", "sdm_op_conv_ex", "sdm_op_conv_up_stats", "sdm_op_gemm_p3", "sdm_debug_run_layer", "sdm_debug_set_input_cmask", "sdm_debug_temb_row", "sdm_conv_num_cfgs", "sdm_bench_conv", "sdm_bench_attn", "sdm_bench_gemm_p3", "sdm_op_groupnorm", "sdm_op_layernorm", "sdm_op_attention", "sdm_op_attention_ex", "sdm_op_attention_split", "sdm_op_attention_split_ex", "sdm_debug_attn_plan", "sdm_op_resize_aa",
+    "sdm_op_mask_bias", "sdm_op_cross_patch_planes", "sdm_op_cross_patch_planes_ex", "sdm_op_attention_shared", "sdm_debug_cross_attention", "sdm_op_cross_core",
     "sdm_set_option", "sdm_get_option", "sdm_reset_options", "sdm_option_name", "sdm_option_help", "sdm_kernel_counts", "sdm_kernel_counts_reset",
 ]
 
@@ -140,12 +140,15 @@
             "sdm_op_groupnorm": (i32, [vp, vp, vp, i32, i32, i32, i32, i32, i32, vp, vp, f32, i32, vp]),
             "sdm_op_layernorm": (i32, [vp, vp, i32, C.c_long, i32, vp, vp, f32, vp]),
             "sdm_op_attention": (i32, [vp, vp, i32, vp, i32, vp, i32, vp, i32, i32, i32, i32, i32, vp, i32]),
+            "sdm_op_attention_ex": (i32, [vp, vp, i32, vp, i32, vp, i32, i32, i32, i32, i32, i32, i32, vp, i32]),
             "sdm_op_attention_split": (i32, [vp, vp, vp, vp, vp, i32, i32, i32, i32, vp]),
             "sdm_op_attention_split_ex": (i32, [vp, vp, vp, vp, vp, vp, i32, i32, i32, i32, i32, vp, vp]),
             "sdm_debug_attn_plan": (i32, [i32] * 10 + [C.c_char_p, i32, C.POINTER(i32)]),
             "sdm_op_resize_aa": (i32, [vp, vp, i32, i32, i32, vp, i32, i32]),
             "sdm_op_mask_bias": (i32, [vp, vp, i32, i32, i32, vp]),
             "sdm_op_cross_patch_planes": (i32, [vp, vp, i32, i32, i32, vp, vp, vp]),
+            "sdm_op_cross_patch_planes_ex": (i32, [vp, vp, i32, i32, i32, vp, vp, vp, i32]),
+            "sdm_op_cross_core": (i32, [vp, vp, vp, i32, i32, i32, i32, i32, vp]),
             "sdm_op_attention_shared": (i32, [vp, vp, vp, vp, i32, i32, i32, i32, i32, vp]),
             "sdm_debug_cross_attention": (i32, [vp, C.c_char_p, vp, i32, i32, i32, vp, i32, i32, vp]),
             "sdm_set_option": (i32, [C.c_char_p, i32]),
@@ -861,6 +864,14 @@
                                               heads, Lq, Lk, D, _ptr(out), HD), "sdm_op_attention")
         return out
 
+    def op_attention_f32(self, q, k, v, heads):
+        B, Lq, HD = q.shape
+        Lk = k.shape[1]
+        out = torch.empty(B, Lq, HD, dtype=torch.float32, device=q.device)
+        self._check(self.lib.sdm_op_attention_ex(self.h, _ptr(q), q.stride(1), _ptr(k), k.stride(1), _ptr(v), v.stride(1), B, heads, Lq, Lk, HD // heads, 1,
+                                                 _ptr(out), HD), "sdm_op_attention_ex")
+        return out
+
     def op_attention_split(self, q, k, v, heads, bias=None, out_p3=0, tiles=None, planes=False):
         B, Lq, HD = q.shape
         Lk = k.shape[1]
@@ -875,7 +886,7 @@
                                                        _ptr(out), _ptr(raw)), "sdm_op_attention_split_ex")
         return (out, raw) if raw is not None else out
 
-    def op_cross_patch_planes(self, uin):
+    def op_cross_patch_planes(self, uin, ones_rows=False):
         B, H, W_, _ = uin.shape
         L = H * W_
         ldvt = (L + 63) // 64 * 64
@@ -883,7 +894,8 @@
         k_hi = torch.full((B, L, 64), 7.0, dtype=torch.float16, device=x.device)
         k_pair = torch.full((B, L, 64, 2), 7, dtype=torch.uint8, device=x.device)
         vt = torch.full((B, 64, ldvt), 7.0, dtype=torch.float16, device=x.device)
-        self._check(self.lib.sdm_op_cross_patch_planes(self.h, _ptr(x), B, H, W_, _ptr(k_hi), _ptr(k_pair), _ptr(vt)), "sdm_op_cross_patch_planes")
+        self._check(self.lib.sdm_op_cross_patch_planes_ex(self.h, _ptr(x), B, H, W_, _ptr(k_hi), _ptr(k_pair), _ptr(vt), int(ones_rows)),
+                    "sdm_op_cross_patch_planes_ex")
         return k_hi, k_pair, vt
 
     def op_attention_shared(self, q, ks, vs, heads, q_prescaled=False):
@@ -901,6 +913,13 @@
         self._check(self.lib.sdm_debug_cross_attention(self.h, block.encode(), _ptr(x), B, H, W_, _ptr(u), u.shape[1], u.shape[2], _ptr(out)), "sdm_debug_cross_attention")
         return out
 
+    def op_cross_core(self, q, uin, heads):
+        B, Lq, HD = q.shape
+        qf, u = q.float().contiguous(), uin.float().contiguous()
+        out = torch.empty(B, Lq, HD, dtype=torch.float32, device=qf.device)
+        self._check(self.lib.sdm_op_cross_core(self.h, _ptr(qf), _ptr(u), B, heads, Lq, u.shape[1], u.shape[2], _ptr(out)), "sdm_op_cross_core")
+        return out
+
     def op_resize_aa(self, planes, Hout, Wout):
         P, Hin, Win = planes.shape
         out = torch.empty(P, Hout, Wout, dtype=torch.float32, device=planes.device)
diff --git a/include/sdmatte.h b/include/sdmatte.h
--- a/include/sdmatte.h
+++ b/include/sdmatte.h
@@ -189,12 +189,16 @@
                      float eps, void* out_f16);
 int sdm_op_attention(sdm_ctx* ctx, const void* q, int ldq, const void* k, int ldk, const void* v, int ldv, const float* bias,
                      int B, int heads, int Lq, int Lk, int D, void* out, int ldo);
+int sdm_op_attention_ex(sdm_ctx* ctx, const void* q, int ldq, const void* k, int ldk, const void* v, int ldv, int B, int heads, int Lq, int Lk, int D, int out_f32,
+                        void* out, int ldo);
 int sdm_op_attention_split(sdm_ctx* ctx, const float* q, const float* k, const float* v, const float* bias, int B, int heads, int Lq, int Lk, float* out);
 int sdm_op_attention_split_ex(sdm_ctx* ctx, const float* q, const float* k, const float* v, const float* bias, const int* tiles, int B, int heads, int Lq,
                               int Lk, int out_p3, float* out, void* planes);
 int sdm_op_cross_patch_planes(sdm_ctx* ctx, const float* uin, int B, int H, int W, void* k_hi, void* k_pair, void* vt);
+int sdm_op_cross_patch_planes_ex(sdm_ctx* ctx, const float* uin, int B, int H, int W, void* k_hi, void* k_pair, void* vt, int ones_rows);
 int sdm_op_attention_shared(sdm_ctx* ctx, const float* q, const float* ks, const float* vs, int B, int heads, int Lq, int Lk, int q_prescaled, float* out);
 int sdm_debug_cross_attention(sdm_ctx* ctx, const char* block, const float* x, int B, int H, int W, const float* uin, int h, int w, float* out);
+int sdm_op_cross_core(sdm_ctx* ctx, const float* q, const float* uin, int B, int heads, int Lq, int h, int w, float* out);
 int sdm_debug_attn_plan(int B, int heads, int Lq, int Lk, int D, int prec, int out_f32, int has_bias, int has_tiles, int cus, char* kernel, int cap,
                         int* nsplit);
 int sdm_op_resize_aa(sdm_ctx* ctx, const float* in, int P, int Hin, int Win, float* out, int Hout, int Wout);
```

Result: faster. 22.52 (median of 6 runs) (+1.2%).
